# ana-kuznetsova/Policy-Gradient-ASR

Hardware: AMD Instinct MI355X
Metric: utterances/sec (B=32,T=1000,F=80) policy-grad step, 1/2/4/8 MI355X (higher is better)
Workload: dtype f32 (fp32-faithful: fp32 storage and accumulate; every big product -- recurrent sweeps, W_ih projections, input and weight gradients -- on the bf16 MFMA as SIX terms of a 3-plane split hi/mid/lo, every term down to 2^-24 of the product; the small products on the exact fp32 MFMA; the faster bf16x3 mo

## Files before the change

include/pgasr_hip.h:

```cpp
#ifndef PGASR_HIP_H
#define PGASR_HIP_H

#include <stddef.h>
#include <stdint.h>

#ifdef __cplusplus
extern "C" {
#endif

typedef enum pgasr_status {
    PGASR_OK = 0,
    PGASR_ERR_INVALID_ARG = 1,
    PGASR_ERR_LAUNCH = 2,
    PGASR_ERR_WORKSPACE = 3,
    PGASR_ERR_UNSUPPORTED = 4,
    PGASR_ERR_TIMEOUT = 5
} pgasr_status;

#define PGASR_ABI_VERSION 7

int pgasr_abi_version(void);
const char* pgasr_status_string(int status);

size_t pgasr_ctc_workspace_bytes(int T, int B, int V, int Lmax);
int pgasr_ctc_loss_grad(const float* log_probs, const int32_t* targets,
                        const int32_t* input_lengths, const int32_t* target_lengths,
                        int T, int B, int V, int Lmax, int blank,
                        const float* utt_scale, const float* pg_coef, const int32_t* pg_path,
                        float* nll, float* grad_logits,
                        void* workspace, size_t workspace_bytes, void* stream);

int pgasr_ctc_grad_from_lattice(const float* log_probs, const int32_t* input_lengths,
                                const int32_t* target_lengths, int T, int B, int V, int Lmax, int blank,
                                const float* utt_scale, const float* pg_coef, const int32_t* pg_path,
                                int pg_coef_per_frame, float* grad_logits, void* workspace, size_t workspace_bytes,
                                void* stream);

int pgasr_pg_rewards(const int32_t* dist, const int32_t* target_lengths, int B, float lam,
                     float inv_global_batch, float* R_greedy, float* R_sample, float* pg_coef,
                     float* utt_scale, void* stream);
int pgasr_pg_loss_value(const float* log_probs, const int32_t* path, const int32_t* input_lengths,
                        const float* nll, const float* utt_scale, const float* pg_coef,
                        int T, int B, int V, int pg_coef_per_frame, float* terms, void* stream);
int pgasr_pg_step_coefs(const int32_t* paths, const int32_t* input_lengths, const int32_t* prefix_dist, int prefix_stride,
                        const int32_t* token_lengths, const int32_t* target_lengths, int T, int B, int blank,
                        float lam, float inv_global_batch, float* coef, void* stream);

#define PGASR_MAX_SAMPLES 16
#define PGASR_BASELINE_HYPOTHESIS 0
#define PGASR_BASELINE_LEAVE_ONE_OUT 1
int pgasr_frame_sample_multi(const float* scores, int T, int B, int V, int K,
                             uint64_t seed, uint32_t offset, int ctr_stride, int ctr_base,
                             int32_t* greedy_path, int32_t* sample_paths, void* stream);
int pgasr_ctc_grad_from_lattice_multi(const float* log_probs, const int32_t* input_lengths,
                                      const int32_t* target_lengths, int T, int B, int V, int Lmax, int blank,
                                      const float* utt_scale, int K, const float* pg_coef, const int32_t* pg_paths,
                                      float* grad_logits, void* workspace, size_t workspace_bytes, void* stream);
int pgasr_pg_rewards_multi(const int32_t* dist, const int32_t* target_lengths, int B, int K, int baseline,
                           float lam, float inv_global_batch, float* R_baseline, float* R_sample, float* pg_coef,
                           float* utt_scale, void* stream);
int pgasr_pg_loss_value_multi(const float* log_probs, const int32_t* paths, int K, const int32_t* input_lengths,
                              const float* nll, const float* utt_scale, const float* pg_coef,
                              int T, int B, int V, float* terms, void* stream);

size_t pgasr_ctc_hyp_workspace_bytes(int T, int B, int V, int K, int Lh);
int pgasr_ctc_hyp_lattice(const float* log_probs, const int32_t* hyp_tokens, int hyp_stride, const int32_t* hyp_len,
                          const int32_t* input_lengths, int T, int B, int V, int K, int Lh, int blank,
                          float* hyp_nll, void* hyp_workspace, size_t hyp_workspace_bytes, void* stream);
int pgasr_ctc_grad_from_lattices_seq(const float* log_probs, const int32_t* input_lengths, const int32_t* target_lengths,
                                     int T, int B, int V, int Lmax, int blank, const float* utt_scale,
                                     int K, const float* pg_coef, const int32_t* pg_paths, const int32_t* hyp_len, int Lh,
                                     float* grad_logits, void* workspace, size_t workspace_bytes,
                                     void* hyp_workspace, size_t hyp_workspace_bytes, void* stream);
int pgasr_pg_loss_value_seq(const float* log_probs, const int32_t* paths, int K, const int32_t* input_lengths,
                            const float* nll, const float* utt_scale, const float* pg_coef,
                            const float* hyp_nll, const int32_t* hyp_len, int Lh,
                            int T, int B, int V, float* terms, void* stream);

int pgasr_frame_entropy(const float* log_probs, const int32_t* input_lengths, int T, int B, int V,
                        float beta, float inv_global_batch, float* ent_mean, float* ent_scale, void* stream);
int pgasr_ctc_grad_from_lattice_ent(const float* log_probs, const int32_t* input_lengths,
                                    const int32_t* target_lengths, int T, int B, int V, int Lmax, int blank,
                                    const float* utt_scale, const float* pg_coef, const int32_t* pg_path,
                                    int pg_coef_per_frame, const float* ent_scale, float* grad_logits,
                                    void* workspace, size_t workspace_bytes, void* stream);
int pgasr_ctc_grad_from_lattice_multi_ent(const float* log_probs, const int32_t* input_lengths,
                                          const int32_t* target_lengths, int T, int B, int V, int Lmax, int blank,
                                          const float* utt_scale, int K, const float* pg_coef, const int32_t* pg_paths,
                                          const float* ent_scale, float* grad_logits, void* workspace, size_t workspace_bytes,
                                          void* stream);
int pgasr_ctc_grad_from_lattices_seq_ent(const float* log_probs, const int32_t* input_lengths, const int32_t* target_lengths,
                                         int T, int B, int V, int Lmax, int blank, const float* utt_scale,
                                         int K, const float* pg_coef, const int32_t* pg_paths, const int32_t* hyp_len, int Lh,
                                         const float* ent_scale, float* grad_logits, void* workspace, size_t workspace_bytes,
                                         void* hyp_workspace, size_t hyp_workspace_bytes, void* stream);

size_t pgasr_ctc_align_workspace_bytes(int T, int B, int Lmax);
int pgasr_ctc_forced_align(const float* log_probs, const int32_t* tokens, const int32_t* input_lengths,
                           const int32_t* token_lengths, int T, int B, int V, int Lmax, int blank,
                           double* score, int32_t* frame_label, int32_t* frame_token,
                           int32_t* token_start, int32_t* token_end, double* token_logp,
                           void* workspace, size_t workspace_bytes, void* stream);

#define PGASR_WORD_MAX_STRIDE 4094
int pgasr_word_ids(const int32_t* ref, const int32_t* ref_len, int ref_stride,
                   const int32_t* hyp, const int32_t* hyp_len, int hyp_stride, int N, int delimiter,
                   int32_t* ref_ids, int32_t* ref_words, int32_t* hyp_ids, int32_t* hyp_words, void* stream);
int pgasr_pg_rewards_multi_ex(const int32_t* dist, const int32_t* reward_lengths, const int32_t* target_lengths, int B, int K,
                              int baseline, float lam, float inv_global_batch, float* R_baseline, float* R_sample,
                              float* pg_coef, float* utt_scale, void* stream);

int pgasr_head_logsoftmax(const float* x, long long rows, int K, int ldx, const float* W, const float* bias, int V,
                          float* logits, float* log_probs, void* stream);

int pgasr_frame_argmax_sample(const float* scores, int T, int B, int V,
                              uint64_t seed, uint32_t offset, int ctr_stride, int ctr_base,
                              int32_t* greedy_path, int32_t* sample_path, void* stream);

int pgasr_frame_argmax_sample_ids(const float* scores, int T, int B, int V, uint64_t seed, uint32_t offset,
                                  int ctr_stride, const int32_t* utt_ids,
                                  int32_t* greedy_path, int32_t* sample_path, void* stream);
int pgasr_frame_sample_multi_ids(const float* scores, int T, int B, int V, int K, uint64_t seed, uint32_t offset,
                                 int ctr_stride, const int32_t* utt_ids,
                                 int32_t* greedy_path, int32_t* sample_paths, void* stream);

int pgasr_batch_prep(const float* fmask, int B, int T, const long long* tmask, const long long* targets, int L,
                     int32_t* in_len, int32_t* tg_len, int32_t* targets32, void* stream);
int pgasr_ctc_collapse(const int32_t* paths, const int32_t* lengths, int P, int T, int B,
                       int blank, int32_t* tokens, int32_t* token_lengths, void* stream);

int pgasr_edit_distance(const int32_t* ref, const int32_t* ref_len, int ref_stride,
                        const int32_t* hyp, const int32_t* hyp_len, int hyp_stride,
                        int N, int32_t* dist, int32_t* prefix_dist, void* stream);

int pgasr_reinforce_grad(const float* scores, const int32_t* path, const float* coef,
                         const int32_t* lengths, int T, int B, int V, int accumulate,
                         float* grad, void* stream);

size_t pgasr_gemm_workspace_bytes(int M, int N, int batch, int splitk, int sum_batches);
int pgasr_gemm_f32(int transA, int transB, int M, int N, int K, float alpha,
                   const float* A, int lda, long long strideA,
                   const float* B, int ldb, long long strideB,
                   float* C, int ldc, long long strideC,
                   int batch, int sum_batches, int splitk,
                   const float* bias, const float* bias2, int act, float slope, int accumulate,
                   const float* dact_y, int norm_operand, const float* shift, const float* scale,
                   int precision, const unsigned* xcc_busy, void* workspace, size_t workspace_bytes, void* stream);

int pgasr_split_bf16_planes(const float* src, int rows, int cols, int ld, int transpose,
                            unsigned short* hi, unsigned short* lo, void* stream);
int pgasr_gemm_x3w_f32(int M, int N, int K, const float* A, int lda, const unsigned short* Whi,
                       const unsigned short* Wlo, float* C, int ldc, const float* bias,
                       const float* dact_y, float slope, void* stream);
size_t pgasr_gemm_x3w_feed_workspace_bytes(void);
int pgasr_gemm_x3w_feed_col_tiles(int N);
int pgasr_gemm_x3w_feed_head_items(int N, int K, int groups);
int pgasr_gemm_x3w_feed_f32(int M, int N, int K, const float* A, int lda, const unsigned short* Whi,
                            const unsigned short* Wlo, float* C, int ldc, const float* bias,
                            const unsigned* xcc_busy, unsigned* tiles_done, int order, int phase, int head_groups,
                            void* workspace, size_t workspace_bytes, void* stream);

size_t pgasr_lstm_wgrads_workspace_bytes(int T, int in_dim);
int pgasr_lstm_wgrads_streamed(const float* dgates, const float* x, const float* out, int T, int B, int in_dim,
                               float* dwih_perm, float* dwhh_perm, const unsigned* xcc_busy,
                               const unsigned* slab_done, int* err_word, int planes,
                               void* workspace, size_t workspace_bytes, void* stream);

int pgasr_pack_x6w_planes(const float* src, int rows, int cols, int ld, int transpose, void* pack, void* stream);
int pgasr_split_bf16_planes3(const float* src, int rows, int cols, int ld, int transpose,
                             unsigned short* hi, unsigned short* mid, unsigned short* lo, void* stream);
int pgasr_gemm_x6w_f32(int M, int N, int K, const float* A, int lda, const unsigned short* Whi,
                       const unsigned short* Wmid, const unsigned short* Wlo, float* C, int ldc, const float* bias,
                       const float* dact_y, float slope, void* stream);
size_t pgasr_gemm_x6w_feed_workspace_bytes(void);
int pgasr_gemm_x6w_feed_col_tiles(int N);
int pgasr_gemm_x6w_feed_f32(int M, int N, int K, const float* A, int lda, const unsigned short* Whi,
                            const unsigned short* Wmid, const unsigned short* Wlo, float* C, int ldc, const float* bias,
                            const unsigned* xcc_busy, unsigned* tiles_done, int order,
                            void* workspace, size_t workspace_bytes, void* stream);
int pgasr_gemm_x6w_feed_head_items(int M, int N, int K);
int pgasr_gemm_x6w_feed_phase_f32(int M, int N, int K, const float* A, int lda, const unsigned short* Whi,
                                  const unsigned short* Wmid, const unsigned short* Wlo, float* C, int ldc, const float* bias,
                                  const unsigned* xcc_busy, unsigned* tiles_done, int order, int phase, unsigned* ctrl,
                                  void* workspace, size_t workspace_bytes, void* stream);

int pgasr_attention_ctx(const float* dec, const float* enc, int NQ, int B, int T, int H, float* ctx, void* stream);

int pgasr_lstm_cell_f32(const float* gh, const float* xp, float* c, float* h, float* h_out, int B, int H, void* stream);

size_t pgasr_colsum_workspace_bytes(int rows, int cols);
int pgasr_colsum_f32(const float* X, int rows, int cols, int ld, float* out, float* out2, int accumulate,
                     void* workspace, size_t workspace_bytes, void* stream);

int pgasr_instnorm_stats(const float* x, int B, int F, int T, float eps, float* mean, float* rstd,
                         void* stream);

int pgasr_log_softmax_rows(const float* logits, long long rows, int V, float* log_probs, void* stream);

size_t pgasr_lstm_pack_bytes(int which, int planes);
int pgasr_lstm_pack_weights(const float* w_ih_f, const float* w_hh_f, const float* b_ih_f, const float* b_hh_f,
                            const float* w_ih_r, const float* w_hh_r, const float* b_ih_r, const float* b_hh_r,
                            int in_dim, float* wih_perm, float* bias_perm,
                            void* whh_pack_fwd, void* whh_pack_bwd, int planes, void* stream);
int pgasr_lstm_unpack_grads(const float* dwih_perm, const float* dbias_perm, const float* dwhh_perm, int in_dim,
                            float* dw_ih_f, float* dw_hh_f, float* db_ih_f, float* db_hh_f,
                            float* dw_ih_r, float* dw_hh_r, float* db_ih_r, float* db_hh_r,
                            int accumulate, void* stream);
size_t pgasr_lstm_workspace_bytes(int T, int B, int backward);
int pgasr_lstm_error_offset(int B, int backward, size_t* offset);
int pgasr_lstm_status(const void* workspace, size_t workspace_bytes, int B, int backward, void* stream);
int pgasr_error_flag(const int32_t* word0, const int32_t* word1, float* out, void* stream);
int pgasr_lstm_busy_offset(int B, int backward, size_t* offset);
int pgasr_stream_gate(const unsigned* words, int count, int timeout_us, void* stream);
int pgasr_stream_gate_sum(const unsigned* words, int count, int need, const unsigned* running, int timeout_us, void* stream);
int pgasr_stream_gate_report(const unsigned* words, int count, int need, const unsigned* running, int timeout_us,
                             unsigned* report, void* stream);
int pgasr_stream_probe(unsigned* words, int timeout_us, void* stream);
int pgasr_lstm_layer_fwd(float* gates, float* out, float* cbuf, const void* whh_pack_fwd,
                         const int32_t* lengths, int T, int B, int flags,
                         float* out_drop, float drop_p, uint64_t drop_seed, uint32_t drop_offset,
                         void* workspace, size_t workspace_bytes, void* stream);
int pgasr_lstm_layer_fwd_fed(float* gates, float* out, float* cbuf, const void* whh_pack_fwd,
                             const int32_t* lengths, int T, int B, int flags, const unsigned* fed, int fed_need,
                             float* out_drop, float drop_p, uint64_t drop_seed, uint32_t drop_offset,
                             void* workspace, size_t workspace_bytes, void* stream);
int pgasr_lstm_fed_ok(int T, int B, int flags);
int pgasr_lstm_layer_bwd_fed(float* gates, const float* out, const float* cbuf, const float* dout,
                             const void* whh_pack_bwd, const int32_t* lengths, int T, int B, int flags,
                             float* dbias_part, const unsigned* fed, int fed_need, float drop_p, uint64_t drop_seed,
                             uint32_t drop_offset, void* workspace, size_t workspace_bytes, void* stream);
int pgasr_lstm_layer_bwd(float* gates, const float* out, const float* cbuf, const float* dout,
                         const void* whh_pack_bwd, const int32_t* lengths, int T, int B, int flags,
                         float* dbias_part, void* workspace, size_t workspace_bytes, void* stream);
int pgasr_lstm_wgrad_slabs(int T, int* edges, int max_edges);
int pgasr_lstm_layer_bwd_streamed(float* gates, const float* out, const float* cbuf, const float* dout,
                                  const void* whh_pack_bwd, const int32_t* lengths, int T, int B, int flags,
                                  float* dbias_part, const unsigned* fed, int fed_need, float drop_p, uint64_t drop_seed,
                                  uint32_t drop_offset, unsigned* slab_done,
                                  void* workspace, size_t workspace_bytes, void* stream);

size_t pgasr_beam_workspace_bytes(int T, int B, int V, int beam);
int pgasr_ctc_beam_search(const void* log_probs, int is_f64, long long stride_t, long long stride_b,
                          const int32_t* lengths, int T, int B, int V, int beam, int blank, int flags,
                          int32_t* out_tokens, int32_t* out_len, double* out_score,
                          void* workspace, size_t workspace_bytes, void* stream);

int pgasr_ctc_beam_search_lm(const void* log_probs, int is_f64, long long stride_t, long long stride_b,
                             const int32_t* lengths, int T, int B, int V, int beam, int blank, int flags,
                             int32_t* out_tokens, int32_t* out_len, double* out_score,
                             void* workspace, size_t workspace_bytes, void* stream,
                             const float* lm_table, int lm_order, double lm_alpha, double lm_beta);

#define PGASR_SPECAUG_FILL_ROW_MEAN 0
#define PGASR_SPECAUG_FILL_ZERO 1
int pgasr_spec_augment(const float* x, const int32_t* lengths, const int32_t* utt_ids ,
                       int batch_offset, int B, int F, int T, int n_freq, int freq_width, int n_time, int time_width,
                       float time_ratio, int fill_mode, unsigned long long seed, unsigned offset,
                       float* out , int32_t* masks ,
                       void* stream);

int pgasr_dropout(const float* x, float* y, unsigned long long n, float p, uint64_t seed, uint32_t offset,
                  const float* dact_y, float slope, void* stream);
int pgasr_stream_copy(const void* src, void* dst, unsigned long long bytes, int workgroups, void* stream);
int pgasr_adam_step(float* param, const float* grad, float* exp_avg, float* exp_avg_sq, unsigned long long n,
                    int step, float lr, float beta1, float beta2, float eps, float weight_decay,
                    const int32_t* guard0, const int32_t* guard1, int32_t* applied, void* stream);
#define PGASR_CLIP_STATE_BYTES 32
size_t pgasr_grad_norm_ws_bytes(unsigned long long n);
int pgasr_grad_norm_clip(const float* grad, unsigned long long n, float max_norm, void* ws, size_t ws_bytes,
                         void* state, void* stream);
int pgasr_adam_step_clipped(float* param, const float* grad, float* exp_avg, float* exp_avg_sq, unsigned long long n,
                            int step, float lr, float beta1, float beta2, float eps, float weight_decay,
                            const int32_t* guard0, const int32_t* guard1, int32_t* applied, const void* clip_state,
                            void* stream);

int pgasr_feat_frames(const float* wave, const int32_t* n_samples, const int32_t* n_frames, int B,
                      long long wave_stride, int Tmax, float* frames, void* stream);
int pgasr_feat_power(const float* spec, long long rows, float* power, void* stream);
int pgasr_feat_db(float* mel, const int32_t* n_frames, int B, int Tmax, int n_mels, float top_db, void* stream);
int pgasr_feat_deltas_stack(const float* mfcc, const int32_t* n_frames, int B, int Tmax, int n_mfcc,
                            float* feat, float* fmask, void* stream);
int pgasr_feat_stack(const float* x, const int32_t* n_frames, int B, int Tmax, int C, float* feat, float* fmask, void* stream);

#ifdef __cplusplus
}
#endif
#endif
```

policy_gradient_asr_amd/_lib.py:

```python
import ctypes as C
import os

import torch

_HERE = os.path.dirname(os.path.abspath(__file__))
LIB_PATH = os.environ.get("PGASR_HIP_LIB", os.path.join(_HERE, "libpgasr_hip.so"))

c_f32p = C.c_void_p
c_i32p = C.c_void_p
c_ptr = C.c_void_p

SIGNATURES = {
    "pgasr_abi_version": (C.c_int, []),
    "pgasr_status_string": (C.c_char_p, [C.c_int]),
    "pgasr_ctc_workspace_bytes": (C.c_size_t, [C.c_int, C.c_int, C.c_int, C.c_int]),
    "pgasr_ctc_loss_grad": (C.c_int, [c_f32p, c_i32p, c_i32p, c_i32p, C.c_int, C.c_int, C.c_int, C.c_int,
                                      C.c_int, c_f32p, c_f32p, c_i32p, c_f32p, c_f32p, c_ptr, C.c_size_t, c_ptr]),
    "pgasr_ctc_grad_from_lattice": (C.c_int, [c_f32p, c_i32p, c_i32p, C.c_int, C.c_int, C.c_int, C.c_int, C.c_int,
                                              c_f32p, c_f32p, c_i32p, C.c_int, c_f32p, c_ptr, C.c_size_t, c_ptr]),
    "pgasr_pg_rewards": (C.c_int, [c_i32p, c_i32p, C.c_int, C.c_float, C.c_float, c_f32p, c_f32p, c_f32p, c_f32p, c_ptr]),
    "pgasr_pg_loss_value": (C.c_int, [c_f32p, c_i32p, c_i32p, c_f32p, c_f32p, c_f32p, C.c_int, C.c_int, C.c_int, C.c_int,
                                      c_f32p, c_ptr]),
    "pgasr_head_logsoftmax": (C.c_int, [c_f32p, C.c_longlong, C.c_int, C.c_int, c_f32p, c_f32p, C.c_int, c_f32p, c_f32p, c_ptr]),
    "pgasr_pg_step_coefs": (C.c_int, [c_i32p, c_i32p, c_i32p, C.c_int, c_i32p, c_i32p, C.c_int, C.c_int, C.c_int,
                                      C.c_float, C.c_float, c_f32p, c_ptr]),
    "pgasr_frame_argmax_sample": (C.c_int, [c_f32p, C.c_int, C.c_int, C.c_int, C.c_uint64, C.c_uint32, C.c_int, C.c_int,
                                            c_i32p, c_i32p, c_ptr]),
    "pgasr_frame_sample_multi": (C.c_int, [c_f32p, C.c_int, C.c_int, C.c_int, C.c_int, C.c_uint64, C.c_uint32, C.c_int, C.c_int,
                                           c_i32p, c_i32p, c_ptr]),
    "pgasr_frame_argmax_sample_ids": (C.c_int, [c_f32p, C.c_int, C.c_int, C.c_int, C.c_uint64, C.c_uint32, C.c_int, c_i32p,
                                                c_i32p, c_i32p, c_ptr]),
    "pgasr_frame_sample_multi_ids": (C.c_int, [c_f32p, C.c_int, C.c_int, C.c_int, C.c_int, C.c_uint64, C.c_uint32, C.c_int, c_i32p,
                                               c_i32p, c_i32p, c_ptr]),
    "pgasr_ctc_grad_from_lattice_multi": (C.c_int, [c_f32p, c_i32p, c_i32p, C.c_int, C.c_int, C.c_int, C.c_int, C.c_int,
                                                    c_f32p, C.c_int, c_f32p, c_i32p, c_f32p, c_ptr, C.c_size_t, c_ptr]),
    "pgasr_pg_rewards_multi": (C.c_int, [c_i32p, c_i32p, C.c_int, C.c_int, C.c_int, C.c_float, C.c_float, c_f32p, c_f32p, c_f32p,
                                         c_f32p, c_ptr]),
    "pgasr_pg_loss_value_multi": (C.c_int, [c_f32p, c_i32p, C.c_int, c_i32p, c_f32p, c_f32p, c_f32p, C.c_int, C.c_int, C.c_int,
                                            c_f32p, c_ptr]),
    "pgasr_ctc_hyp_workspace_bytes": (C.c_size_t, [C.c_int] * 5),
    "pgasr_ctc_hyp_lattice": (C.c_int, [c_f32p, c_i32p, C.c_int, c_i32p, c_i32p, C.c_int, C.c_int, C.c_int, C.c_int, C.c_int, C.c_int,
                                        c_f32p, c_ptr, C.c_size_t, c_ptr]),
    "pgasr_ctc_grad_from_lattices_seq": (C.c_int, [c_f32p, c_i32p, c_i32p, C.c_int, C.c_int, C.c_int, C.c_int, C.c_int, c_f32p,
                                                   C.c_int, c_f32p, c_i32p, c_i32p, C.c_int, c_f32p, c_ptr, C.c_size_t,
                                                   c_ptr, C.c_size_t, c_ptr]),
    "pgasr_pg_loss_value_seq": (C.c_int, [c_f32p, c_i32p, C.c_int, c_i32p, c_f32p, c_f32p, c_f32p, c_f32p, c_i32p, C.c_int,
                                          C.c_int, C.c_int, C.c_int, c_f32p, c_ptr]),
    "pgasr_frame_entropy": (C.c_int, [c_f32p, c_i32p, C.c_int, C.c_int, C.c_int, C.c_float, C.c_float, c_f32p, c_f32p, c_ptr]),
    "pgasr_ctc_grad_from_lattice_ent": (C.c_int, [c_f32p, c_i32p, c_i32p, C.c_int, C.c_int, C.c_int, C.c_int, C.c_int,
                                                  c_f32p, c_f32p, c_i32p, C.c_int, c_f32p, c_f32p, c_ptr, C.c_size_t, c_ptr]),
    "pgasr_ctc_grad_from_lattice_multi_ent": (C.c_int, [c_f32p, c_i32p, c_i32p, C.c_int, C.c_int, C.c_int, C.c_int, C.c_int,
                                                        c_f32p, C.c_int, c_f32p, c_i32p, c_f32p, c_f32p, c_ptr, C.c_size_t, c_ptr]),
    "pgasr_ctc_grad_from_lattices_seq_ent": (C.c_int, [c_f32p, c_i32p, c_i32p, C.c_int, C.c_int, C.c_int, C.c_int, C.c_int, c_f32p,
                                                       C.c_int, c_f32p, c_i32p, c_i32p, C.c_int, c_f32p, c_f32p, c_ptr, C.c_size_t,
                                                       c_ptr, C.c_size_t, c_ptr]),
    "pgasr_ctc_align_workspace_bytes": (C.c_size_t, [C.c_int] * 3),
    "pgasr_ctc_forced_align": (C.c_int, [c_f32p, c_i32p, c_i32p, c_i32p, C.c_int, C.c_int, C.c_int, C.c_int, C.c_int,
                                         c_ptr, c_i32p, c_i32p, c_i32p, c_i32p, c_ptr, c_ptr, C.c_size_t, c_ptr]),
    "pgasr_word_ids": (C.c_int, [c_i32p, c_i32p, C.c_int, c_i32p, c_i32p, C.c_int, C.c_int, C.c_int, c_i32p, c_i32p, c_i32p, c_i32p,
                                 c_ptr]),
    "pgasr_pg_rewards_multi_ex": (C.c_int, [c_i32p, c_i32p, c_i32p, C.c_int, C.c_int, C.c_int, C.c_float, C.c_float, c_f32p, c_f32p,
                                            c_f32p, c_f32p, c_ptr]),
    "pgasr_batch_prep": (C.c_int, [c_f32p, C.c_int, C.c_int, c_ptr, c_ptr, C.c_int, c_i32p, c_i32p, c_i32p, c_ptr]),
    "pgasr_ctc_collapse": (C.c_int, [c_i32p, c_i32p, C.c_int, C.c_int, C.c_int, C.c_int, c_i32p, c_i32p, c_ptr]),
    "pgasr_edit_distance": (C.c_int, [c_i32p, c_i32p, C.c_int, c_i32p, c_i32p, C.c_int, C.c_int,
                                      c_i32p, c_i32p, c_ptr]),
    "pgasr_reinforce_grad": (C.c_int, [c_f32p, c_i32p, c_f32p, c_i32p, C.c_int, C.c_int, C.c_int, C.c_int,
                                       c_f32p, c_ptr]),
    "pgasr_beam_workspace_bytes": (C.c_size_t, [C.c_int] * 4),
    "pgasr_ctc_beam_search": (C.c_int, [c_ptr, C.c_int, C.c_longlong, C.c_longlong, c_i32p, C.c_int, C.c_int, C.c_int,
                                        C.c_int, C.c_int, C.c_int, c_i32p, c_i32p, c_ptr, c_ptr, C.c_size_t, c_ptr]),
    "pgasr_ctc_beam_search_lm": (C.c_int, [c_ptr, C.c_int, C.c_longlong, C.c_longlong, c_i32p, C.c_int, C.c_int, C.c_int,
                                           C.c_int, C.c_int, C.c_int, c_i32p, c_i32p, c_ptr, c_ptr, C.c_size_t, c_ptr,
                                           c_f32p, C.c_int, C.c_double, C.c_double]),
    "pgasr_dropout": (C.c_int, [c_f32p, c_f32p, C.c_ulonglong, C.c_float, C.c_uint64, C.c_uint32, c_f32p, C.c_float, c_ptr]),
    "pgasr_spec_augment": (C.c_int, [c_f32p, c_i32p, c_i32p, C.c_int, C.c_int, C.c_int, C.c_int, C.c_int, C.c_int, C.c_int, C.c_int,
                                     C.c_float, C.c_int, C.c_ulonglong, C.c_uint, c_f32p, c_i32p, c_ptr]),
    "pgasr_stream_copy": (C.c_int, [c_ptr, c_ptr, C.c_ulonglong, C.c_int, c_ptr]),
    "pgasr_adam_step": (C.c_int, [c_f32p, c_f32p, c_f32p, c_f32p, C.c_ulonglong, C.c_int, C.c_float, C.c_float,
                                  C.c_float, C.c_float, C.c_float, c_i32p, c_i32p, c_i32p, c_ptr]),
    "pgasr_adam_step_clipped": (C.c_int, [c_f32p, c_f32p, c_f32p, c_f32p, C.c_ulonglong, C.c_int, C.c_float, C.c_float,
                                          C.c_float, C.c_float, C.c_float, c_i32p, c_i32p, c_i32p, c_ptr, c_ptr]),
    "pgasr_grad_norm_ws_bytes": (C.c_size_t, [C.c_ulonglong]),
    "pgasr_grad_norm_clip": (C.c_int, [c_f32p, C.c_ulonglong, C.c_float, c_ptr, C.c_size_t, c_ptr, c_ptr]),
    "pgasr_gemm_workspace_bytes": (C.c_size_t, [C.c_int] * 5),
    "pgasr_gemm_f32": (C.c_int, [C.c_int, C.c_int, C.c_int, C.c_int, C.c_int, C.c_float,
                                 c_f32p, C.c_int, C.c_longlong, c_f32p, C.c_int, C.c_longlong,
                                 c_f32p, C.c_int, C.c_longlong, C.c_int, C.c_int, C.c_int,
                                 c_f32p, c_f32p, C.c_int, C.c_float, C.c_int,
                                 c_f32p, C.c_int, c_f32p, c_f32p, C.c_int, c_ptr, c_ptr, C.c_size_t, c_ptr]),
    "pgasr_split_bf16_planes": (C.c_int, [c_f32p, C.c_int, C.c_int, C.c_int, C.c_int, c_ptr, c_ptr, c_ptr]),
    "pgasr_gemm_x3w_f32": (C.c_int, [C.c_int, C.c_int, C.c_int, c_f32p, C.c_int, c_ptr, c_ptr, c_f32p, C.c_int,
                                     c_f32p, c_f32p, C.c_float, c_ptr]),
    "pgasr_gemm_x3w_feed_workspace_bytes": (C.c_size_t, []),
    "pgasr_gemm_x3w_feed_col_tiles": (C.c_int, [C.c_int]),
    "pgasr_gemm_x3w_feed_head_items": (C.c_int, [C.c_int, C.c_int, C.c_int]),
    "pgasr_gemm_x3w_feed_f32": (C.c_int, [C.c_int, C.c_int, C.c_int, c_f32p, C.c_int, c_ptr, c_ptr, c_f32p, C.c_int,
                                          c_f32p, c_ptr, c_ptr, C.c_int, C.c_int, C.c_int, c_ptr, C.c_size_t, c_ptr]),
    "pgasr_feat_frames": (C.c_int, [c_f32p, c_i32p, c_i32p, C.c_int, C.c_longlong, C.c_int, c_f32p, c_ptr]),
    "pgasr_feat_power": (C.c_int, [c_f32p, C.c_longlong, c_f32p, c_ptr]),
    "pgasr_feat_db": (C.c_int, [c_f32p, c_i32p, C.c_int, C.c_int, C.c_int, C.c_float, c_ptr]),
    "pgasr_feat_deltas_stack": (C.c_int, [c_f32p, c_i32p, C.c_int, C.c_int, C.c_int, c_f32p, c_f32p, c_ptr]),
    "pgasr_feat_stack": (C.c_int, [c_f32p, c_i32p, C.c_int, C.c_int, C.c_int, c_f32p, c_f32p, c_ptr]),
    "pgasr_colsum_workspace_bytes": (C.c_size_t, [C.c_int, C.c_int]),
    "pgasr_colsum_f32": (C.c_int, [c_f32p, C.c_int, C.c_int, C.c_int, c_f32p, c_f32p, C.c_int,
                                   c_ptr, C.c_size_t, c_ptr]),
    "pgasr_instnorm_stats": (C.c_int, [c_f32p, C.c_int, C.c_int, C.c_int, C.c_float, c_f32p, c_f32p, c_ptr]),
    "pgasr_log_softmax_rows": (C.c_int, [c_f32p, C.c_longlong, C.c_int, c_f32p, c_ptr]),
    "pgasr_lstm_pack_bytes": (C.c_size_t, [C.c_int, C.c_int]),
    "pgasr_lstm_pack_weights": (C.c_int, [c_f32p] * 8 + [C.c_int, c_f32p, c_f32p, c_ptr, c_ptr, C.c_int, c_ptr]),
    "pgasr_lstm_unpack_grads": (C.c_int, [c_f32p, c_f32p, c_f32p, C.c_int] + [c_f32p] * 8 + [C.c_int, c_ptr]),
    "pgasr_lstm_workspace_bytes": (C.c_size_t, [C.c_int, C.c_int, C.c_int]),
    "pgasr_lstm_error_offset": (C.c_int, [C.c_int, C.c_int, C.POINTER(C.c_size_t)]),
    "pgasr_lstm_busy_offset": (C.c_int, [C.c_int, C.c_int, C.POINTER(C.c_size_t)]),
    "pgasr_lstm_status": (C.c_int, [c_ptr, C.c_size_t, C.c_int, C.c_int, c_ptr]),
    "pgasr_stream_gate": (C.c_int, [c_ptr, C.c_int, C.c_int, c_ptr]),
    "pgasr_stream_gate_sum": (C.c_int, [c_ptr, C.c_int, C.c_int, c_ptr, C.c_int, c_ptr]),
    "pgasr_stream_gate_report": (C.c_int, [c_ptr, C.c_int, C.c_int, c_ptr, C.c_int, c_ptr, c_ptr]),
    "pgasr_stream_probe": (C.c_int, [c_ptr, C.c_int, c_ptr]),
    "pgasr_lstm_layer_fwd": (C.c_int, [c_f32p, c_f32p, c_f32p, c_ptr, c_i32p, C.c_int, C.c_int, C.c_int,
                                       c_f32p, C.c_float, C.c_uint64, C.c_uint32, c_ptr, C.c_size_t, c_ptr]),
    "pgasr_lstm_layer_fwd_fed": (C.c_int, [c_f32p, c_f32p, c_f32p, c_ptr, c_i32p, C.c_int, C.c_int, C.c_int, c_ptr, C.c_int,
                                           c_f32p, C.c_float, C.c_uint64, C.c_uint32, c_ptr, C.c_size_t, c_ptr]),
    "pgasr_lstm_fed_ok": (C.c_int, [C.c_int, C.c_int, C.c_int]),
    "pgasr_lstm_layer_bwd_fed": (C.c_int, [c_f32p, c_f32p, c_f32p, c_f32p, c_ptr, c_i32p, C.c_int, C.c_int, C.c_int,
                                           c_f32p, c_ptr, C.c_int, C.c_float, C.c_uint64, C.c_uint32, c_ptr, C.c_size_t, c_ptr]),
    "pgasr_lstm_layer_bwd": (C.c_int, [c_f32p, c_f32p, c_f32p, c_f32p, c_ptr, c_i32p, C.c_int, C.c_int, C.c_int,
                                       c_f32p, c_ptr, C.c_size_t, c_ptr]),
    "pgasr_lstm_wgrad_slabs": (C.c_int, [C.c_int, c_i32p, C.c_int]),
    "pgasr_lstm_layer_bwd_streamed": (C.c_int, [c_f32p, c_f32p, c_f32p, c_f32p, c_ptr, c_i32p, C.c_int, C.c_int, C.c_int,
                                                c_f32p, c_ptr, C.c_int, C.c_float, C.c_uint64, C.c_uint32, c_ptr,
                                                c_ptr, C.c_size_t, c_ptr]),
    "pgasr_lstm_wgrads_workspace_bytes": (C.c_size_t, [C.c_int, C.c_int]),
    "pgasr_lstm_wgrads_streamed": (C.c_int, [c_f32p, c_f32p, c_f32p, C.c_int, C.c_int, C.c_int, c_f32p, c_f32p, c_ptr,
                                             c_ptr, c_ptr, C.c_int, c_ptr, C.c_size_t, c_ptr]),
    "pgasr_error_flag": (C.c_int, [c_i32p, c_i32p, c_f32p, c_ptr]),
    "pgasr_attention_ctx": (C.c_int, [c_f32p, c_f32p, C.c_int, C.c_int, C.c_int, C.c_int, c_f32p, c_ptr]),
    "pgasr_lstm_cell_f32": (C.c_int, [c_f32p, c_f32p, c_f32p, c_f32p, c_f32p, C.c_int, C.c_int, c_ptr]),
    "pgasr_pack_x6w_planes": (C.c_int, [c_f32p, C.c_int, C.c_int, C.c_int, C.c_int, c_ptr, c_ptr]),
    "pgasr_split_bf16_planes3": (C.c_int, [c_f32p, C.c_int, C.c_int, C.c_int, C.c_int, c_ptr, c_ptr, c_ptr, c_ptr]),
    "pgasr_gemm_x6w_f32": (C.c_int, [C.c_int, C.c_int, C.c_int, c_f32p, C.c_int, c_ptr, c_ptr, c_ptr, c_f32p, C.c_int,
                                     c_f32p, c_f32p, C.c_float, c_ptr]),
    "pgasr_gemm_x6w_feed_workspace_bytes": (C.c_size_t, []),
    "pgasr_gemm_x6w_feed_col_tiles": (C.c_int, [C.c_int]),
    "pgasr_gemm_x6w_feed_f32": (C.c_int, [C.c_int, C.c_int, C.c_int, c_f32p, C.c_int, c_ptr, c_ptr, c_ptr, c_f32p, C.c_int,
                                          c_f32p, c_ptr, c_ptr, C.c_int, c_ptr, C.c_size_t, c_ptr]),
    "pgasr_gemm_x6w_feed_head_items": (C.c_int, [C.c_int, C.c_int, C.c_int]),
    "pgasr_gemm_x6w_feed_phase_f32": (C.c_int, [C.c_int, C.c_int, C.c_int, c_f32p, C.c_int, c_ptr, c_ptr, c_ptr, c_f32p, C.c_int,
                                                c_f32p, c_ptr, c_ptr, C.c_int, C.c_int, c_ptr, c_ptr, C.c_size_t, c_ptr]),
}


class PgasrError(RuntimeError):
    pass


TIMEOUT = 5


_lib = None


def load():
    global _lib
    if _lib is not None:
        return _lib
    if not os.path.exists(LIB_PATH):
        raise PgasrError(
            f"{LIB_PATH} is missing: build it with `python -c 'import __graft_entry__ as g; g.build()'` "
            "or `make -C policy_gradient_asr_amd/csrc`.  There is no CPU fallback.")
    lib = C.CDLL(LIB_PATH)
    for name, (res, args) in SIGNATURES.items():
        fn = getattr(lib, name)
        fn.restype = res
        fn.argtypes = args
    if lib.pgasr_abi_version() != 7:
        raise PgasrError("libpgasr_hip.so ABI version mismatch")
    _lib = lib
    return lib


def check(status, what):
    if status != 0:
        msg = load().pgasr_status_string(status).decode()
        raise PgasrError(f"{what} failed: status {status} ({msg})")
```

policy_gradient_asr_amd/csrc/common.h:

```cpp
#pragma once
#include <hip/hip_runtime.h>
#include <stdint.h>
#include <math.h>
#include <stdio.h>
#include <stdlib.h>
#include "pgasr_hip.h"

#define PGASR_WAVE 64

#define PGASR_LAUNCH_KERNEL(...)                               \
    do {                                                       \
        (void)hipGetLastError();                               \
        hipLaunchKernelGGL(__VA_ARGS__);                       \
    } while (0)

#define PGASR_CHECK_LAUNCH()                                                                  \
    do {                                                                                      \
        hipError_t e__ = hipGetLastError();                                                   \
        if (e__ != hipSuccess) {                                                              \
            if (getenv("PGASR_DEBUG"))                                                        \
                fprintf(stderr, "[pgasr] %s:%d launch failed: %s\n", __FILE__, __LINE__,      \
                        hipGetErrorString(e__));                                              \
            return PGASR_ERR_LAUNCH;                                                          \
        }                                                                                     \
    } while (0)

static inline size_t pgasr_align_up(size_t x, size_t a) { return (x + a - 1) / a * a; }

#define PGASR_NEG_INF (-INFINITY)

__device__ __forceinline__ float wave_sum(float v) {
#pragma unroll
    for (int o = 32; o > 0; o >>= 1) v += __shfl_xor(v, o, 64);
    return v;
}
__device__ __forceinline__ float wave_max(float v) {
#pragma unroll
    for (int o = 32; o > 0; o >>= 1) v = fmaxf(v, __shfl_xor(v, o, 64));
    return v;
}

__device__ __forceinline__ float block_path_logprob_sum(const float* __restrict__ lp, const int32_t* __restrict__ path,
                                                        const float* __restrict__ frame_coef, int Tb, int b, int B, int V, float* red) {
    float s = 0.f;
    for (int t = threadIdx.x; t < Tb; t += 256) {
        const float v = lp[((size_t)t * B + b) * V + path[(size_t)t * B + b]];
        s += frame_coef ? frame_coef[(size_t)t * B + b] * v : v;
    }
    red[threadIdx.x] = s;
    __syncthreads();
    for (int o = 128; o > 0; o >>= 1) {
        if (threadIdx.x < o) red[threadIdx.x] += red[threadIdx.x + o];
        __syncthreads();
    }
    const float r = red[0];
    __syncthreads();
    return r;
}

__device__ __forceinline__ void philox4x32_10(uint32_t c0, uint32_t c1, uint32_t c2, uint32_t c3,
                                              uint32_t k0, uint32_t k1, uint32_t out[4]) {
#pragma unroll
    for (int r = 0; r < 10; ++r) {
        const uint64_t p0 = (uint64_t)0xD2511F53u * c0;
        const uint64_t p1 = (uint64_t)0xCD9E8D57u * c2;
        const uint32_t n0 = (uint32_t)(p1 >> 32) ^ c1 ^ k0;
        const uint32_t n1 = (uint32_t)p1;
        const uint32_t n2 = (uint32_t)(p0 >> 32) ^ c3 ^ k1;
        const uint32_t n3 = (uint32_t)p0;
        c0 = n0; c1 = n1; c2 = n2; c3 = n3;
        k0 += 0x9E3779B9u; k1 += 0xBB67AE85u;
    }
    out[0] = c0; out[1] = c1; out[2] = c2; out[3] = c3;
}

#ifndef PGASR_WSLAB_NUM
#define PGASR_WSLAB_NUM 5
#define PGASR_WSLAB_DEN 4
#define PGASR_WSLAB_CAP 128
#endif
__host__ __device__ inline int pgasr_wslab_next(int s) { const int n = ((s * PGASR_WSLAB_NUM) / PGASR_WSLAB_DEN + 4) & ~7; return n > PGASR_WSLAB_CAP ? PGASR_WSLAB_CAP : n; }
__host__ __device__ inline int pgasr_wslab_count(int T) {
    int h = 0, s = 16, n = 1;
    while (T - h > s + s / 2) { h += s; s = pgasr_wslab_next(s); ++n; }
    return n;
}
__host__ __device__ inline int pgasr_wslab_edge(int T, int i) {
    int h = 0, s = 16;
    for (int j = 0; j < i; ++j) {
        if (T - h <= s + s / 2) return T;
        h += s; s = pgasr_wslab_next(s);
    }
    return h;
}

struct PgasrTn256Args {
    const float* A; const float* B; float* partial;
    int M, N, K, lda, ldb;
    long long sA, sB;
    int batch, splitk, kper;
    float alpha;
    unsigned* queue;
    const unsigned* xcc_busy;
    int diag;
    const unsigned* gate;
    const float* gate_base;
    int gate_T, gate_B, gate_nbg;
    int tslabs;
    int* gate_err;
};
bool pgasr_internal_tn256_ok(const PgasrTn256Args& a, int tk = 32);
int pgasr_internal_tn256_launch(PgasrTn256Args a, int masked_then_unmasked, hipStream_t st, const PgasrTn256Args* second = nullptr);
int pgasr_internal_tn6_launch(PgasrTn256Args a, int masked_then_unmasked, hipStream_t st, const PgasrTn256Args* second = nullptr);

struct PgasrX3cArgs {
    const float* A; const unsigned short* Whi; const unsigned short* Wlo; float* C;
    int M, N, K, lda, ldc;
    const float* bias; const float* dact_y; float slope;
    int feed;
    unsigned* queue; const unsigned* xcc_busy; unsigned* tiles_done;
    int mt_count, nt_count, order, quarters, split_tiles;
    float* slabs; unsigned* arrive;
};
size_t pgasr_internal_x3c_slab_bytes();
int pgasr_internal_x3c_launch(const PgasrX3cArgs& a, hipStream_t st);
```

policy_gradient_asr_amd/csrc/gemm.hip:

```cpp
#include "common.h"

namespace {

constexpr int BM = 128, BN = 128, BK = 16, PADF = 4;
constexpr int GEMM_THREADS = 256;

typedef __attribute__((ext_vector_type(16))) float f32x16;

struct GemmArgs {
    const float* A; const float* B; float* C;
    int M, N, K, lda, ldb, ldc;
    long long sA, sB, sC;
    int batch, splitk, kper;
    float alpha;
    const float* bias; const float* bias2;
    int act; float slope;
    int accumulate;
    const float* dact_y;
    int norm_operand;
    const float* shift; const float* scale;
    float* partial;
    unsigned* queue;
    const unsigned* xcc_busy;
    int tx, ty, tz;
// ... 388 lines not shown
                    ah[i] = tr_frag(&S[cur][0][0][ro]);
                    al[i] = tr_frag(&S[cur][0][1][ro]);
                } else {
                    const int ro = (wm * 64 + i * 32 + fr) * XPITCH + kk + fk;
                    ah[i] = __builtin_bit_cast(bf16x8_t, *reinterpret_cast<const u32x4_t*>(&S[cur][0][0][ro]));
                    al[i] = __builtin_bit_cast(bf16x8_t, *reinterpret_cast<const u32x4_t*>(&S[cur][0][1][ro]));
                }
                if constexpr (TRB) {
                    const int co = kk * TPITCH + wn * 64 + i * 32 + tro;
                    bh[i] = tr_frag(&S[cur][1][0][co]);
                    bl[i] = tr_frag(&S[cur][1][1][co]);
                } else {
                    const int co = (wn * 64 + i * 32 + fr) * XPITCH + kk + fk;
                    bh[i] = __builtin_bit_cast(bf16x8_t, *reinterpret_cast<const u32x4_t*>(&S[cur][1][0][co]));
                    bl[i] = __builtin_bit_cast(bf16x8_t, *reinterpret_cast<const u32x4_t*>(&S[cur][1][1][co]));
                }
            }
#pragma unroll
            for (int i = 0; i < 2; ++i)
#pragma unroll
                for (int j = 0; j < 2; ++j) {
                    acc[i][j] = __builtin_amdgcn_mfma_f32_32x32x16_bf16(ah[i], bh[j], acc[i][j], 0, 0, 0);
                    acc[i][j] = __builtin_amdgcn_mfma_f32_32x32x16_bf16(ah[i], bl[j], acc[i][j], 0, 0, 0);
                    acc[i][j] = __builtin_amdgcn_mfma_f32_32x32x16_bf16(al[i], bh[j], acc[i][j], 0, 0, 0);
                }
        }
    };
    const int nrm = g.norm_operand;
    const float nsh = nrm ? g.shift[bidx] : 0.f, nsc = nrm ? g.scale[bidx] : 1.f;
    auto norm_strip = [&](float (&v)[16], bool tr, int mn_base, int mn_lim, int kb) {
#pragma unroll
        for (int i = 0; i < 16; ++i) {
            const int mn = tr ? mn_base + (tid & 31) * 4 + (i & 3) : mn_base + (tid >> 1);
            const int k = tr ? kb + (tid >> 5) + 8 * (i >> 2) : kb + (tid & 1) * 16 + i;
            v[i] = (mn < mn_lim && k < kend) ? (v[i] - nsh) * nsc : 0.f;
        }
    };
#define XLOAD(RA, RB, KB) do { if constexpr (TRA) tload_strip(A, g.lda, m0, g.M, (KB), kend, tid, vecA, RA); \
                               else xload_strip(A, g.lda, m0, g.M, (KB), kend, tid, vecA, RA); \
                               if constexpr (TRB) tload_strip(B, g.ldb, n0, g.N, (KB), kend, tid, vecB, RB); \
                               else xload_strip(B, g.ldb, n0, g.N, (KB), kend, tid, vecB, RB); \
                               if (nrm == 1) norm_strip(RA, TRA, m0, g.M, (KB)); \
                               else if (nrm == 2) norm_strip(RB, TRB, n0, g.N, (KB)); } while (0)
#define XSTORE(RA, RB, BUF) do { if constexpr (TRA) tstore_strip(S[BUF][0][0], S[BUF][0][1], tid, RA); \
                                 else xstore_strip(S[BUF][0][0], S[BUF][0][1], tid, RA); \
                                 if constexpr (TRB) tstore_strip(S[BUF][1][0], S[BUF][1][1], tid, RB); \
                                 else xstore_strip(S[BUF][1][0], S[BUF][1][1], tid, RB); } while (0)
    if (kbeg < kend) {
        XLOAD(ra0, rb0, kbeg);
        XSTORE(ra0, rb0, 0);
        if (kbeg + XBK < kend) XLOAD(ra0, rb0, kbeg + XBK);
    }
    __syncthreads();
    for (int kb = kbeg; kb < kend; kb += 2 * XBK) {
        if (kb + 2 * XBK < kend) XLOAD(ra1, rb1, kb + 2 * XBK);
        compute(0);
        if (kb + XBK < kend) XSTORE(ra0, rb0, 1);
        __syncthreads();
        if (kb + XBK >= kend) break;
        if (kb + 3 * XBK < kend) XLOAD(ra0, rb0, kb + 3 * XBK);
        compute(1);
        if (kb + 2 * XBK < kend) XSTORE(ra1, rb1, 0);
        __syncthreads();
    }
#undef XLOAD
#undef XSTORE

    if (!g.wide) { store_tiles_fast(g, acc, m0, n0, wm, wn, lane, z, bidx, live); return; }
    const int cl = lane & 31, rq = lane >> 5;
#pragma unroll
    for (int i = 0; i < 2; ++i)
#pragma unroll
        for (int j = 0; j < 2; ++j) {
            const int n = n0 + wn * 64 + j * 32 + cl;
            if (n >= g.N || !live) continue;
            float bsum = 0.f;
            if (!g.partial) {
                if (g.bias) bsum += g.bias[n];
                if (g.bias2) bsum += g.bias2[n];
            }
#pragma unroll
            for (int r = 0; r < 16; ++r) {
                const int m = m0 + wm * 64 + i * 32 + (r & 3) + 8 * (r >> 2) + 4 * rq;
                if (m >= g.M) continue;
                float v = g.alpha * acc[i][j][r];
                if (g.partial) {
                    g.partial[((size_t)z * g.M + m) * g.N + n] = v;
                } else {
                    float* c = g.C + (size_t)bidx * g.sC + (size_t)m * g.ldc + n;
                    v += bsum;
                    if (g.act == 1) v = v > 0.f ? v : v * g.slope;
                    if (g.dact_y) v *= (g.dact_y[(size_t)bidx * g.sC + (size_t)m * g.ldc + n] > 0.f ? 1.f : g.slope);
                    if (g.accumulate) v += *c;
                    *c = v;
                }
            }
        }
}

__global__ __launch_bounds__(256) void gemm_reduce_kernel(const float* __restrict__ partial, int Z, int M, int N,
                                                          float* __restrict__ C, int ldc, long long sC,
                                                          const float* bias,
                                                          const float* bias2, int act, float slope, int accumulate) {
    const size_t idx = (size_t)blockIdx.x * 256 + threadIdx.x;
    if (idx >= (size_t)M * N) return;
    const int m = (int)(idx / N), n = (int)(idx % N);
    partial += (size_t)blockIdx.y * Z * M * N;
    C += (size_t)blockIdx.y * sC;
    float v = 0.f;
    for (int zz = 0; zz < Z; ++zz) v += partial[(size_t)zz * M * N + idx];
    if (bias) v += bias[n];
    if (bias2) v += bias2[n];
    if (act == 1) v = v > 0.f ? v : v * slope;
    float* c = C + (size_t)m * ldc + n;
    if (accumulate) v += *c;
    *c = v;
}

__global__ __launch_bounds__(256) void colsum_partial_kernel(const float* __restrict__ X, int rows, int cols, int ld,
                                                             int rows_per_block, float* __restrict__ partial) {
    __shared__ float red[4][64];
    const int c = blockIdx.x * 64 + (threadIdx.x & 63);
    const int rl = threadIdx.x >> 6;
    const int r0 = blockIdx.y * rows_per_block, r1 = min(rows, r0 + rows_per_block);
    float s = 0.f;
    if (c < cols)
        for (int r = r0 + rl; r < r1; r += 4) s += X[(size_t)r * ld + c];
    red[rl][threadIdx.x & 63] = s;
    __syncthreads();
    if (rl == 0 && c < cols)
        partial[(size_t)blockIdx.y * cols + c] = (red[0][threadIdx.x] + red[1][threadIdx.x]) + (red[2][threadIdx.x] + red[3][threadIdx.x]);
}
__global__ __launch_bounds__(256) void colsum_final_kernel(const float* __restrict__ partial, int nparts, int cols,
                                                           float* __restrict__ out, float* __restrict__ out2, int accumulate) {
    const int c = blockIdx.x * 256 + threadIdx.x;
    if (c >= cols) return;
    float s = 0.f;
    for (int p = 0; p < nparts; ++p) s += partial[(size_t)p * cols + c];
    if (accumulate) { out[c] += s; if (out2) out2[c] += s; }
    else { out[c] = s; if (out2) out2[c] = s; }
}

__global__ __launch_bounds__(1024) void instnorm_stats_kernel(const float* __restrict__ x, long long n_per, float eps,
                                                              float* __restrict__ mean, float* __restrict__ rstd) {
    __shared__ double s1[16], s2[16];
    const float* p = x + (size_t)blockIdx.x * n_per;
    double a = 0.0, b = 0.0;
    long long done = 0;
    if (((n_per & 3) == 0) && ((((size_t)x) & 15) == 0)) {
        const float4* p4 = reinterpret_cast<const float4*>(p);
        const long long n4 = n_per >> 2;
        double a1 = 0.0, b1 = 0.0;
        long long i = threadIdx.x;
        for (; i + 3 * 1024 < n4; i += 4 * 1024) {
            const float4 u0 = p4[i], u1 = p4[i + 1024], u2 = p4[i + 2 * 1024], u3 = p4[i + 3 * 1024];
            a += ((double)u0.x + (double)u0.y) + ((double)u0.z + (double)u0.w);
            b += ((double)u0.x * u0.x + (double)u0.y * u0.y) + ((double)u0.z * u0.z + (double)u0.w * u0.w);
            a1 += ((double)u1.x + (double)u1.y) + ((double)u1.z + (double)u1.w);
            b1 += ((double)u1.x * u1.x + (double)u1.y * u1.y) + ((double)u1.z * u1.z + (double)u1.w * u1.w);
            a += ((double)u2.x + (double)u2.y) + ((double)u2.z + (double)u2.w);
            b += ((double)u2.x * u2.x + (double)u2.y * u2.y) + ((double)u2.z * u2.z + (double)u2.w * u2.w);
            a1 += ((double)u3.x + (double)u3.y) + ((double)u3.z + (double)u3.w);
            b1 += ((double)u3.x * u3.x + (double)u3.y * u3.y) + ((double)u3.z * u3.z + (double)u3.w * u3.w);
        }
        for (; i < n4; i += 1024) {
            const float4 u = p4[i];
            a += ((double)u.x + (double)u.y) + ((double)u.z + (double)u.w);
            b += ((double)u.x * u.x + (double)u.y * u.y) + ((double)u.z * u.z + (double)u.w * u.w);
        }
        a += a1; b += b1;
        done = n_per;
    }
    for (long long i = done + threadIdx.x; i < n_per; i += 1024) { const double v = p[i]; a += v; b += v * v; }
#pragma unroll
    for (int o = 32; o > 0; o >>= 1) { a += __shfl_xor(a, o, 64); b += __shfl_xor(b, o, 64); }
    if ((threadIdx.x & 63) == 0) { s1[threadIdx.x >> 6] = a; s2[threadIdx.x >> 6] = b; }
    __syncthreads();
    if (threadIdx.x == 0) {
        double ta = 0.0, tb = 0.0;
        for (int i = 0; i < 16; ++i) { ta += s1[i]; tb += s2[i]; }
        const double mu = ta / (double)n_per;
        double var = tb / (double)n_per - mu * mu;
        if (var < 0.0) var = 0.0;
        mean[blockIdx.x] = (float)mu;
        rstd[blockIdx.x] = (float)(1.0 / sqrt(var + (double)eps));
    }
}

}

static int gemm_launch(GemmArgs& g, int transA, int transB, int sum_batches, int precision, const unsigned* xcc_busy, void* workspace,
                       size_t workspace_bytes, hipStream_t st) {
    const int Z = g.batch * g.splitk;
    const bool use_partial = (g.splitk > 1) || sum_batches;
    const bool queue_mode = precision >= 1 && xcc_busy != nullptr;
    const size_t head = 256;
    if (use_partial || queue_mode) {
        const size_t need = head + (use_partial ? (size_t)Z * g.M * g.N * sizeof(float) : 0);
        if (!workspace || workspace_bytes < need) return PGASR_ERR_WORKSPACE;
    }
    g.partial = use_partial ? (float*)((char*)workspace + head) : nullptr;
    g.queue = nullptr; g.xcc_busy = nullptr;
    dim3 grid((g.N + BN - 1) / BN, (g.M + BM - 1) / BM, Z);
    if (grid.y > 65535 || grid.z > 65535) return PGASR_ERR_UNSUPPORTED;
    g.tx = (int)grid.x; g.ty = (int)grid.y; g.tz = (int)grid.z;
    if (queue_mode) {
        g.queue = (unsigned*)workspace; g.xcc_busy = xcc_busy;
        if (hipMemsetAsync(workspace, 0, head, st) != hipSuccess) return PGASR_ERR_LAUNCH;
    }
    const unsigned ntiles_q = grid.x * grid.y * grid.z;

    bool done_tn256 = false;
    if (precision >= 1 && transA && !transB && use_partial && g.norm_operand == 0) {
        PgasrTn256Args t{g.A, g.B, g.partial, g.M, g.N, g.K, g.lda, g.ldb, g.sA, g.sB, g.batch, g.splitk, g.kper, g.alpha,
                         queue_mode ? g.queue : nullptr, queue_mode ? g.xcc_busy : nullptr, getenv("PGASR_TN_DIAG") ? atoi(getenv("PGASR_TN_DIAG")) : 0,
                         nullptr, nullptr, 0, 0, 0, 0, nullptr};
        if (pgasr_internal_tn256_ok(t)) {
            const int st_ = precision == 2 ? pgasr_internal_tn6_launch(t, queue_mode ? 1 : 0, st) : pgasr_internal_tn256_launch(t, queue_mode ? 1 : 0, st);
            if (st_ != PGASR_OK) return st_;
            done_tn256 = true;
        }
    }
    if (done_tn256) {
    }
    else if (precision == 2) return PGASR_ERR_UNSUPPORTED;
    else if (precision == 1) {
        if (queue_mode) {
            for (int pass = 0; pass < 2; ++pass) {
                dim3 qgrid(pass == 0 ? 2u * ntiles_q + 8u : ntiles_q);
                if (pass == 1) g.xcc_busy = nullptr;
                if (!transA && !transB) PGASR_LAUNCH_KERNEL((gemm_bf16x3_kernel<false, false, true>), qgrid, dim3(GEMM_THREADS), 0, st, g);
                else if (!transA && transB) PGASR_LAUNCH_KERNEL((gemm_bf16x3_kernel<false, true, true>), qgrid, dim3(GEMM_THREADS), 0, st, g);
                else if (transA && !transB) PGASR_LAUNCH_KERNEL((gemm_bf16x3_kernel<true, false, true>), qgrid, dim3(GEMM_THREADS), 0, st, g);
                else PGASR_LAUNCH_KERNEL((gemm_bf16x3_kernel<true, true, true>), qgrid, dim3(GEMM_THREADS), 0, st, g);
                PGASR_CHECK_LAUNCH();
            }
        }
        else if (!transA && !transB) PGASR_LAUNCH_KERNEL((gemm_bf16x3_kernel<false, false, false>), grid, dim3(GEMM_THREADS), 0, st, g);
        else if (!transA && transB) PGASR_LAUNCH_KERNEL((gemm_bf16x3_kernel<false, true, false>), grid, dim3(GEMM_THREADS), 0, st, g);
        else if (transA && !transB) PGASR_LAUNCH_KERNEL((gemm_bf16x3_kernel<true, false, false>), grid, dim3(GEMM_THREADS), 0, st, g);
        else PGASR_LAUNCH_KERNEL((gemm_bf16x3_kernel<true, true, false>), grid, dim3(GEMM_THREADS), 0, st, g);
    }
    else if (!transA && !transB) PGASR_LAUNCH_KERNEL((gemm_f32_kernel<false, false>), grid, dim3(GEMM_THREADS), 0, st, g);
    else if (!transA && transB) PGASR_LAUNCH_KERNEL((gemm_f32_kernel<false, true>), grid, dim3(GEMM_THREADS), 0, st, g);
    else if (transA && !transB) PGASR_LAUNCH_KERNEL((gemm_f32_kernel<true, false>), grid, dim3(GEMM_THREADS), 0, st, g);
    else PGASR_LAUNCH_KERNEL((gemm_f32_kernel<true, true>), grid, dim3(GEMM_THREADS), 0, st, g);
    PGASR_CHECK_LAUNCH();
    if (use_partial) {
        const size_t total = (size_t)g.M * g.N;
        const int nout = sum_batches ? 1 : g.batch;
        PGASR_LAUNCH_KERNEL(gemm_reduce_kernel, dim3((unsigned)((total + 255) / 256), nout), dim3(256), 0, st,
                           g.partial, Z / nout, g.M, g.N, g.C, g.ldc, g.sC, g.bias, g.bias2, g.act, g.slope,
                           g.accumulate);
        PGASR_CHECK_LAUNCH();
    }
    return PGASR_OK;
}

extern "C" size_t pgasr_gemm_workspace_bytes(int M, int N, int batch, int splitk, int sum_batches) {
    if (M <= 0 || N <= 0 || batch <= 0 || splitk <= 0) return 0;
    if (splitk <= 1 && !sum_batches) return 256;
    return 256 + (size_t)batch * splitk * M * N * sizeof(float);
}

extern "C" int pgasr_gemm_f32(int transA, int transB, int M, int N, int K, float alpha,
                              const float* A, int lda, long long strideA,
                              const float* B, int ldb, long long strideB,
                              float* C, int ldc, long long strideC,
                              int batch, int sum_batches, int splitk,
                              const float* bias, const float* bias2, int act, float slope, int accumulate,
                              const float* dact_y, int norm_operand, const float* shift, const float* scale,
                              int precision, const unsigned* xcc_busy, void* workspace, size_t workspace_bytes, void* stream) {
    if (!A || !B || !C || M <= 0 || N <= 0 || K <= 0 || batch <= 0 || splitk <= 0) return PGASR_ERR_INVALID_ARG;
    if (norm_operand < 0 || norm_operand > 2 || (norm_operand && (!shift || !scale))) return PGASR_ERR_INVALID_ARG;
    if (act < 0 || act > 1 || precision < 0 || precision > 2) return PGASR_ERR_INVALID_ARG;
    if ((splitk > 1 || sum_batches) && dact_y) return PGASR_ERR_INVALID_ARG;
    GemmArgs g;
    g.A = A; g.B = B; g.C = C; g.M = M; g.N = N; g.K = K; g.lda = lda; g.ldb = ldb; g.ldc = ldc;
    g.sA = strideA; g.sB = strideB; g.sC = strideC; g.batch = batch; g.splitk = splitk;
    int kper = (K + splitk - 1) / splitk;
    const int kq = precision >= 1 ? XBK : BK;
    kper = (kper + kq - 1) / kq * kq;
    g.kper = kper;
    g.alpha = alpha; g.bias = bias; g.bias2 = bias2; g.act = act; g.slope = slope; g.accumulate = accumulate;
    g.dact_y = dact_y; g.norm_operand = norm_operand; g.shift = shift; g.scale = scale; g.partial = nullptr;
    g.wide = (((size_t)(M - 1) * ldc + N) * 4 >= ((size_t)1 << 32) || (size_t)M * N * 4 >= ((size_t)1 << 32)) ? 1 : 0;
    return gemm_launch(g, transA, transB, sum_batches, precision, xcc_busy, workspace, workspace_bytes, (hipStream_t)stream);
}

extern "C" int pgasr_lstm_wgrad_slabs(int T, int* edges, int max_edges) {
    if (T <= 0) return 0;
    const int n = pgasr_wslab_count(T);
    for (int i = 0; edges && i <= n && i < max_edges; ++i) edges[i] = pgasr_wslab_edge(T, i);
    return n;
}
extern "C" size_t pgasr_lstm_wgrads_workspace_bytes(int T, int in_dim) {
    if (in_dim <= 0 || T <= 0) return 0;
    return 256 + (size_t)pgasr_wslab_count(T) * ((size_t)2048 * in_dim + (size_t)2 * 1024 * 256) * sizeof(float);
}
extern "C" int pgasr_lstm_wgrads_streamed(const float* dgates, const float* x, const float* out, int T, int B, int in_dim,
                                          float* dwih_perm, float* dwhh_perm, const unsigned* xcc_busy,
                                          const unsigned* slab_done, int* err_word, int planes,
                                          void* workspace, size_t workspace_bytes, void* stream) {
    constexpr int H = 256, G = 2 * 4 * H;
    if (!dgates || !x || !out || !dwih_perm || !dwhh_perm || T <= 1 || B <= 0 || in_dim <= 0) return PGASR_ERR_INVALID_ARG;
    if (planes != 2 && planes != 3) return PGASR_ERR_INVALID_ARG;
    const size_t need = pgasr_lstm_wgrads_workspace_bytes(T, in_dim);
    if (!workspace || workspace_bytes < need) return PGASR_ERR_WORKSPACE;
    hipStream_t st = (hipStream_t)stream;
    const int nslab = pgasr_wslab_count(T);
    float* part_ih = (float*)((char*)workspace + 256);
    float* part_hh = part_ih + (size_t)nslab * G * in_dim;
    const long long K_ih = (long long)T * B, K_hh = (long long)(T - 1) * B;
    if (K_ih >= ((long long)1 << 31)) return PGASR_ERR_UNSUPPORTED;
    PgasrTn256Args ih{dgates, x, part_ih, G, in_dim, (int)K_ih, G, in_dim, 0, 0, 1, nslab, 0, 1.f,
                      (unsigned*)workspace, xcc_busy, 0, slab_done, dgates, T, B, (B + 15) / 16, 1, err_word};
    PgasrTn256Args hh{dgates + (size_t)B * G, out, part_hh, 4 * H, H, (int)K_hh, G, 2 * H, (long long)4 * H - (long long)B * G,
                      (long long)B * 2 * H + H, 2, nslab, 0, 1.f,
                      (unsigned*)workspace, xcc_busy, 0, slab_done, dgates, T, B, (B + 15) / 16, 1, err_word};
    const int tk = planes == 3 ? 16 : 32;
    if (!pgasr_internal_tn256_ok(ih, tk) || !pgasr_internal_tn256_ok(hh, tk)) return PGASR_ERR_UNSUPPORTED;
    if (hipMemsetAsync(workspace, 0, 256, st) != hipSuccess) return PGASR_ERR_LAUNCH;
    const int rc = planes == 3 ? pgasr_internal_tn6_launch(ih, 1, st, &hh) : pgasr_internal_tn256_launch(ih, 1, st, &hh);
    if (rc != PGASR_OK) return rc;
    PGASR_LAUNCH_KERNEL(gemm_reduce_kernel, dim3((unsigned)(((size_t)G * in_dim + 255) / 256), 1), dim3(256), 0, st,
                       part_ih, nslab, G, in_dim, dwih_perm, in_dim, (long long)0, (const float*)nullptr, (const float*)nullptr, 0, 0.f, 0);
    PGASR_CHECK_LAUNCH();
    PGASR_LAUNCH_KERNEL(gemm_reduce_kernel, dim3((unsigned)(((size_t)4 * H * H + 255) / 256), 2), dim3(256), 0, st,
                       part_hh, nslab, 4 * H, H, dwhh_perm, H, (long long)4 * H * H, (const float*)nullptr, (const float*)nullptr, 0, 0.f, 0);
    PGASR_CHECK_LAUNCH();
    return PGASR_OK;
}

extern "C" size_t pgasr_colsum_workspace_bytes(int rows, int cols) {
    if (rows <= 0 || cols <= 0) return 0;
    const int rpb = 512;
    return (size_t)((rows + rpb - 1) / rpb) * cols * sizeof(float);
}

extern "C" int pgasr_colsum_f32(const float* X, int rows, int cols, int ld, float* out, float* out2, int accumulate,
                                void* workspace, size_t workspace_bytes, void* stream) {
    if (!X || !out || rows <= 0 || cols <= 0 || ld < cols) return PGASR_ERR_INVALID_ARG;
    const int rpb = 512;
    const int nparts = (rows + rpb - 1) / rpb;
    if (!workspace || workspace_bytes < (size_t)nparts * cols * sizeof(float)) return PGASR_ERR_WORKSPACE;
    hipStream_t st = (hipStream_t)stream;
    PGASR_LAUNCH_KERNEL(colsum_partial_kernel, dim3((cols + 63) / 64, nparts), dim3(256), 0, st, X, rows, cols, ld, rpb,
                       (float*)workspace);
    PGASR_CHECK_LAUNCH();
    PGASR_LAUNCH_KERNEL(colsum_final_kernel, dim3((cols + 255) / 256), dim3(256), 0, st, (const float*)workspace, nparts,
                       cols, out, out2, accumulate);
    PGASR_CHECK_LAUNCH();
    return PGASR_OK;
}

extern "C" int pgasr_instnorm_stats(const float* x, int B, int F, int T, float eps, float* mean, float* rstd,
                                    void* stream) {
    if (!x || !mean || !rstd || B <= 0 || F <= 0 || T <= 0) return PGASR_ERR_INVALID_ARG;
    PGASR_LAUNCH_KERNEL(instnorm_stats_kernel, dim3(B), dim3(1024), 0, (hipStream_t)stream, x, (long long)F * T, eps,
                       mean, rstd);
    PGASR_CHECK_LAUNCH();
    return PGASR_OK;
}
```

policy_gradient_asr_amd/csrc/gemm_x6.hip:

```cpp
#include "common.h"
#include "x3w_common.h"
#include <type_traits>

#ifdef PGASR_X6_DIAG
#define X6D(bit) (!FEED && (g.single & (bit)))
__device__ long long x6_stamp_out[8][16];
#define X6STAMP_DECL long long st_last_ = clock64(); long long st_acc_[12] = {0, 0, 0, 0, 0, 0, 0, 0, 0, 0, 0, 0}; const long long st_c0_ = clock64(), st_r0_ = wall_clock64()
#define X6STAMP(slot) do { const long long now_ = clock64(); st_acc_[slot] += now_ - st_last_; st_last_ = now_; } while (0)
#define X6STAMP_FLUSH() do { if (blockIdx.x == 0 && blockIdx.y == 0 && lane == 0) { for (int i_ = 0; i_ < 12; ++i_) x6_stamp_out[w][i_] = st_acc_[i_]; \
                             x6_stamp_out[w][12] = clock64() - st_c0_; x6_stamp_out[w][13] = wall_clock64() - st_r0_; } } while (0)
#else
#define X6D(bit) false
#define X6STAMP_DECL
#define X6STAMP(slot) do { } while (0)
#define X6STAMP_FLUSH() do { } while (0)
#endif

namespace {
#ifdef PGASR_LSTM_DIAG
__device__ unsigned x6_feed_diag[4096];
#endif
namespace x6c {
constexpr int TM = 256, TN = 256, TK = 16, THREADS = 512;
constexpr int NW = 4;
constexpr int NA = 3;
constexpr int AP_BYTES = TM * TK * 2;
constexpr int ABUF_BYTES = 3 * AP_BYTES;
constexpr int WP_BYTES = TN * TK * 2;
constexpr int WSTAGE_BYTES = 3 * WP_BYTES;
constexpr int LDS_W = 2 * ABUF_BYTES;
constexpr int LDS_BYTES = LDS_W + NW * WSTAGE_BYTES;
constexpr int SLAB_FLOATS = 128 * THREADS;

typedef u32x4_t Planes2[2][3];

__device__ __forceinline__ void read_pair(Planes2& o, unsigned p0, unsigned p1) {
    static_assert(AP_BYTES == 8192 && WP_BYTES == 8192, "plane offsets are spelled in the asm below");
    asm volatile("ds_read_b128 %0, %6\n\t"
                 "ds_read_b128 %1, %6 offset:8192\n\t"
                 "ds_read_b128 %2, %6 offset:16384\n\t"
                 "ds_read_b128 %3, %7\n\t"
                 "ds_read_b128 %4, %7 offset:8192\n\t"
                 "ds_read_b128 %5, %7 offset:16384"
                 : "=&v"(o[0][0]), "=&v"(o[0][1]), "=&v"(o[0][2]), "=&v"(o[1][0]), "=&v"(o[1][1]), "=&v"(o[1][2])
                 : "v"(p0), "v"(p1)
                 : "memory");
}
__device__ __forceinline__ void wait_pair(Planes2& o) {
    asm volatile("s_waitcnt lgkmcnt(0)"
                 : "+v"(o[0][0]), "+v"(o[0][1]), "+v"(o[0][2]), "+v"(o[1][0]), "+v"(o[1][1]), "+v"(o[1][2])
                 :: "memory");
}
__device__ __forceinline__ void wait_pairs(Planes2& a, Planes2& b) {
    asm volatile("s_waitcnt lgkmcnt(0)"
                 : "+v"(a[0][0]), "+v"(a[0][1]), "+v"(a[0][2]), "+v"(a[1][0]), "+v"(a[1][1]), "+v"(a[1][2]),
                   "+v"(b[0][0]), "+v"(b[0][1]), "+v"(b[0][2]), "+v"(b[1][0]), "+v"(b[1][1]), "+v"(b[1][2])
                 :: "memory");
}
__device__ __forceinline__ void read_row(u32x4_t (&o)[3], unsigned p) {
    asm volatile("ds_read_b128 %0, %3\n\t"
                 "ds_read_b128 %1, %3 offset:8192\n\t"
                 "ds_read_b128 %2, %3 offset:16384"
                 : "=&v"(o[0]), "=&v"(o[1]), "=&v"(o[2]) : "v"(p) : "memory");
}
__device__ __forceinline__ void wait_row(u32x4_t (&o)[3]) {
    asm volatile("s_waitcnt lgkmcnt(0)" : "+v"(o[0]), "+v"(o[1]), "+v"(o[2]) :: "memory");
}
__device__ __forceinline__ void wait_row_pair(u32x4_t (&a)[3], Planes2& b) {
    asm volatile("s_waitcnt lgkmcnt(0)"
                 : "+v"(a[0]), "+v"(a[1]), "+v"(a[2]), "+v"(b[0][0]), "+v"(b[0][1]), "+v"(b[0][2]), "+v"(b[1][0]), "+v"(b[1][1]), "+v"(b[1][2])
                 :: "memory");
}
__device__ __forceinline__ void write_planes3(unsigned addr, unsigned h0, unsigned h1, unsigned m0, unsigned m1, unsigned l0, unsigned l1) {
    typedef __attribute__((ext_vector_type(2))) unsigned u2;
    const u2 h = {h0, h1}, m = {m0, m1}, l = {l0, l1};
    asm volatile("ds_write_b64 %0, %1\n\t"
                 "ds_write_b64 %0, %2 offset:8192\n\t"
                 "ds_write_b64 %0, %3 offset:16384" :: "v"(addr), "v"(h), "v"(m), "v"(l) : "memory");
}
template <int J>
__device__ __forceinline__ void load_a_one(u32x4_t (&r)[2], const unsigned (&aoff)[2], unsigned kb, const float* A) {
    asm volatile("global_load_dwordx4 %0, %1, %2" : "=&v"(r[J]) : "v"(aoff[J] + kb), "s"(A) : "memory");
}
template <int CNT>
__device__ __forceinline__ void wait_a_regs(u32x4_t (&r)[2]) {
    asm volatile("s_waitcnt vmcnt(%2)" : "+v"(r[0]), "+v"(r[1]) : "n"(CNT) : "memory");
}

__device__ __forceinline__ void mfma6(f32x16 (&acc)[2], const u32x4_t (&a)[3], const Planes2& b) {
    constexpr int PA[6] = {0, 0, 1, 0, 2, 1}, PB[6] = {0, 1, 0, 2, 0, 1};
#pragma unroll
    for (int p = 0; p < 6; ++p)
#pragma unroll
        for (int j = 0; j < 2; ++j)
            acc[j] = __builtin_amdgcn_mfma_f32_32x32x16_bf16(__builtin_bit_cast(bf16x8_t, a[PA[p]]), __builtin_bit_cast(bf16x8_t, b[j][PB[p]]), acc[j], 0, 0, 0);
}

template <bool FEED, int VAR>
__global__ __launch_bounds__(THREADS) void gemm_x6c_kernel(DmaGemmArgs g) {
    extern __shared__ __attribute__((aligned(128))) unsigned char smem[];
#ifdef PGASR_LSTM_DIAG
    if (FEED && threadIdx.x == 0 && blockIdx.x == 0) x6_feed_diag[0] = (unsigned)wall_clock64();
#endif
    const int tid = threadIdx.x, lane = tid & 63, w = tid >> 6;
    const int wm = w >> 2, wn = w & 3;
    const int nk = g.K / TK;
    bool head_only = false;
    if (FEED && g.xcc_busy) {
        const unsigned xcc = __builtin_amdgcn_s_getreg(((4 - 1) << 11) | (0 << 6) | 20) & 7u;
        if (__hip_atomic_load(g.xcc_busy + xcc, __ATOMIC_RELAXED, __HIP_MEMORY_SCOPE_AGENT) != 0u) {
            if (!g.head_help) return;
            head_only = true;
        }
    }
    const unsigned lds0 = (unsigned)(size_t)(__attribute__((address_space(3))) unsigned char*)smem;
  for (;;) {
    int tbx, tby;
    int kt0 = 0, kt1 = nk, qpart = -1;
    unsigned tile = 0, parts = 1u, slab0 = 0u;
#ifdef PGASR_LSTM_DIAG
    unsigned diag_t_ = 0xFFFFFFFFu;
#endif
    if (FEED) {
        unsigned* mailbox = reinterpret_cast<unsigned*>(smem + LDS_BYTES);
        const unsigned S8 = (unsigned)g.split8_tiles, S = (unsigned)g.split_tiles, S2 = (unsigned)g.split2_tiles, ntot = (unsigned)g.mt_count * (unsigned)g.nt_count;
        const unsigned n8 = 8u * S8, n4 = 4u * S, n2 = 2u * S2;
        if (tid == 0) {
            if (head_only && __hip_atomic_load(g.queue, __ATOMIC_RELAXED, __HIP_MEMORY_SCOPE_AGENT) >= n8 + n4) *mailbox = 0xFFFFFFFFu;
            else *mailbox = __hip_atomic_fetch_add(g.queue, 1u, __ATOMIC_RELAXED, __HIP_MEMORY_SCOPE_AGENT);
        }
        __syncthreads();
        const unsigned t = *mailbox;
        __syncthreads();
        if (t >= ntot + 7u * S8 + 3u * S + S2) return;
#ifdef PGASR_LSTM_DIAG
        if (tid == 0 && t < 4u) x6_feed_diag[4 + t] = (unsigned)wall_clock64();
        if (tid == 0 && t >= n8 + n4 + n2 && t < n8 + n4 + n2 + 4u) x6_feed_diag[1024 + (t - n8 - n4 - n2)] = (unsigned)wall_clock64();
        diag_t_ = t;
#endif
        if (t < n8) { tile = t >> 3; qpart = (int)(t & 7u); parts = 8u; slab0 = 8u * tile; }
        else if (t < n8 + n4) { const unsigned u = t - n8; tile = S8 + (u >> 2); qpart = (int)(u & 3u); parts = 4u; slab0 = n8 + 4u * (u >> 2); }
        else if (t < n8 + n4 + n2) { const unsigned u = t - n8 - n4; tile = S8 + S + (u >> 1); qpart = (int)(u & 1u); parts = 2u; slab0 = n8 + n4 + 2u * (u >> 1); }
        else tile = t - 7u * S8 - 3u * S - S2;
        if (qpart >= 0) { kt0 = qpart * (nk / (int)parts); kt1 = kt0 + nk / (int)parts; }
        const int half = g.nt_count >> 1, grp = (int)(tile / (unsigned)g.nt_count), j = (int)(tile % (unsigned)g.nt_count);
        tbx = j;
        tby = ((j < half) != (g.order != 0)) ? grp : g.mt_count - 1 - grp;
    } else {
        swizzled_tile(tbx, tby);
    }
    const int m0 = tby * TM, n0 = tbx * TN;

    const int rsub = lane >> 2, ac = lane & 3;
    unsigned aoff[2];
    unsigned apw[2];
#pragma unroll
    for (int j = 0; j < 2; ++j) {
        const int r = w * 32 + j * 16 + rsub;
        int gm = m0 + r; gm = gm < g.M ? gm : g.M - 1;
        aoff[j] = (unsigned)(((size_t)gm * g.lda + ac * 4) * 4);
        apw[j] = (unsigned)(r * 32 + (((ac >> 1) ^ ((r >> 3) & 1)) * 16) + (ac & 1) * 8);
    }
    const bool packed = g.Wmid == nullptr;
    const unsigned short* pw[3];
    {
        const int row = 32 * w + (lane >> 1), cp = lane & 1, c = cp ^ ((row >> 3) & 1);
        const size_t o = (size_t)(n0 + row) * g.K + c * 8;
        pw[0] = g.Whi + o; pw[1] = packed ? g.Whi : g.Wmid + o; pw[2] = g.Wlo + o;
    }
    const unsigned char* wpk = reinterpret_cast<const unsigned char*>(g.Whi) + (size_t)tbx * nk * WSTAGE_BYTES + w * 1024 + lane * 16;
    auto issue_w1 = [&](int kt, int stage, int plane) {
        if (X6D(1) && kt >= kt0 + NW - 1) return;
        const int kc = kt < nk ? kt : nk - 1;
        unsigned char* dst = smem + LDS_W + stage * WSTAGE_BYTES + plane * WP_BYTES + w * 1024;
        if (packed) dma16(wpk + ((size_t)kc * 3 + plane) * WP_BYTES, dst);
        else dma16(pw[plane] + kc * TK, dst);
    };
    auto issue_w = [&](int kt, int stage) { issue_w1(kt, stage, 0); issue_w1(kt, stage, 1); issue_w1(kt, stage, 2); };
    u32x4_t araw[NA][2];
    typedef std::integral_constant<int, 0> I0;
    typedef std::integral_constant<int, 1> I1;
    typedef std::integral_constant<int, 2> I2;
    auto load_a1 = [&](int kt, auto setc, int j) {
        const unsigned kb = (unsigned)((kt < nk ? kt : nk - 1) * TK * 4);
        if (X6D(4) && kt >= kt0 + NA + 1) return;
        if (j == 0) load_a_one<0>(araw[decltype(setc)::value], aoff, kb, g.A);
        else load_a_one<1>(araw[decltype(setc)::value], aoff, kb, g.A);
    };
    auto load_a = [&](int kt, auto setc) { load_a1(kt, setc, 0); load_a1(kt, setc, 1); };
    auto convert_a1 = [&](int buf, auto setc, int j) {
        constexpr int S = decltype(setc)::value;
        const unsigned base = lds0 + (unsigned)buf * ABUF_BYTES;
        if (X6D(8)) return;
        unsigned h0, m0_, l0, h1, m1_, l1;
        if (X6D(128)) { h0 = araw[S][j].x; h1 = araw[S][j].y; m0_ = araw[S][j].z; m1_ = araw[S][j].w; l0 = h0; l1 = h1; }
        else {
            split3(__uint_as_float(araw[S][j].x), __uint_as_float(araw[S][j].y), h0, m0_, l0);
            split3(__uint_as_float(araw[S][j].z), __uint_as_float(araw[S][j].w), h1, m1_, l1);
        }
        if (X6D(64)) { asm volatile("" :: "v"(h0), "v"(h1), "v"(m0_), "v"(m1_), "v"(l0), "v"(l1)); return; }
        write_planes3(base + apw[j], h0, h1, m0_, m1_, l0, l1);
    };
    auto convert_a = [&](int buf, auto setc) { convert_a1(buf, setc, 0); convert_a1(buf, setc, 1); };

    const int fr = lane & 31, fh = lane >> 5;
    unsigned offA[4], offB[2];
#pragma unroll
    for (int i = 0; i < 4; ++i) {
        const int row = wm * 128 + i * 32 + fr;
        offA[i] = (unsigned)(row * 32 + ((fh ^ ((row >> 3) & 1)) * 16));
    }
#pragma unroll
    for (int j = 0; j < 2; ++j) {
        const int n = wn * 64 + j * 32 + fr;
        offB[j] = (unsigned)(LDS_W + n * 32 + ((fh ^ ((n >> 3) & 1)) * 16));
    }

    f32x16 acc[4][2];
#pragma unroll
    for (int i = 0; i < 4; ++i)
#pragma unroll
        for (int j = 0; j < 2; ++j)
#pragma unroll
            for (int r = 0; r < 16; ++r) acc[i][j][r] = 0.f;
    X6STAMP_DECL;

    auto half_step = [&](int cur, int wst, auto halfc, Planes2& fb, auto&& mem) {
        constexpr int HALF = decltype(halfc)::value;
        const unsigned ab = lds0 + (unsigned)cur * ABUF_BYTES, wb = lds0 + (unsigned)wst * WSTAGE_BYTES;
        Planes2 fa;
        if (!X6D(16)) {
            if (HALF == 0) read_pair(fb, wb + offB[0], wb + offB[1]);
            read_pair(fa, ab + offA[2 * HALF], ab + offA[2 * HALF + 1]);
        }
        if (HALF == 0) wait_pairs(fa, fb); else wait_pair(fa);
#pragma unroll
        for (int i = 0; i < 2; ++i) {
            if (!X6D(2)) mfma6(acc[2 * HALF + i], fa[i], fb);
            __builtin_amdgcn_sched_barrier(0);
            mem(i);
            __builtin_amdgcn_sched_barrier(0);
        }
    };

    load_a(kt0, I0{});
    issue_w(kt0, 0);
    wait_a_regs<3>(araw[0]);
    convert_a(0, I0{});
    load_a(kt0 + 1, I1{});
    issue_w(kt0 + 1, 1);
    load_a(kt0 + 2, I2{});
    issue_w(kt0 + 2, 2);
    load_a(kt0 + 3, I0{});
    asm volatile("s_waitcnt vmcnt(12)\n\ts_waitcnt lgkmcnt(0)" ::: "memory");
    __builtin_amdgcn_s_barrier();
    asm volatile("" ::: "memory");

    typedef std::integral_constant<int, 1> H1;
    auto step = [&](const int kt, auto setc) {
        const int rel = kt - kt0, cur = rel & 1, wst = rel & (NW - 1);
        const int kw = kt + NW - 1, sw = (rel + NW - 1) & (NW - 1);
        auto mem_w = [&](int s) { if (s == 0) { issue_w1(kw, sw, 0); issue_w1(kw, sw, 1); } else issue_w1(kw, sw, 2); };
        auto mem_a = [&](int s) { load_a1(kt + 1 + NA, setc, s); };
        Planes2 fb;
        __builtin_amdgcn_sched_barrier(0);
        X6STAMP(0);
        if constexpr (VAR == 7) {
            const unsigned ab = lds0 + (unsigned)cur * ABUF_BYTES, wb = lds0 + (unsigned)wst * WSTAGE_BYTES;
            const unsigned cb = lds0 + (unsigned)(cur ^ 1) * ABUF_BYTES;
            constexpr int S = decltype(setc)::value;
            u32x4_t f0[3], f1[3];
            unsigned hh[2], mm[2], ll[2];
            float r0[2], r1[2];
            auto split_a = [&](int j, int q) {
                const float x0 = __uint_as_float(q ? araw[S][j].z : araw[S][j].x), x1 = __uint_as_float(q ? araw[S][j].w : araw[S][j].y);
                typedef __attribute__((ext_vector_type(2))) __bf16 bf2;
                typedef __attribute__((ext_vector_type(2))) float f2;
                hh[q] = __builtin_bit_cast(unsigned, __builtin_convertvector((f2){x0, x1}, bf2));
                r0[q] = x0 - __uint_as_float(hh[q] << 16); r1[q] = x1 - __uint_as_float(hh[q] & 0xFFFF0000u);
            };
            auto split_b = [&](int q) {
                typedef __attribute__((ext_vector_type(2))) __bf16 bf2;
                typedef __attribute__((ext_vector_type(2))) float f2;
                mm[q] = __builtin_bit_cast(unsigned, __builtin_convertvector((f2){r0[q], r1[q]}, bf2));
                const float s0 = r0[q] - __uint_as_float(mm[q] << 16), s1 = r1[q] - __uint_as_float(mm[q] & 0xFFFF0000u);
                ll[q] = __builtin_bit_cast(unsigned, __builtin_convertvector((f2){s0, s1}, bf2));
            };
            auto filler = [&](int kind, int gp, int nextrow, u32x4_t (&fnext)[3]) {
                if (gp == 0 && nextrow >= 0) read_row(fnext, ab + offA[nextrow]);
                if (kind == 0) {
                    if (gp == 1) wait_a_regs<10>(araw[S]);
                    else if (gp == 2) split_a(0, 0);
                    else if (gp == 3) split_b(0);
                    else if (gp == 4) split_a(0, 1);
                    else if (gp == 5) split_b(1);
                    else if (gp == 6) { if (!X6D(8)) write_planes3(cb + apw[0], hh[0], hh[1], mm[0], mm[1], ll[0], ll[1]); }
                    else if (gp == 7) issue_w1(kw, sw, 0);
                    else if (gp == 8) issue_w1(kw, sw, 1);
                    else if (gp == 9) issue_w1(kw, sw, 2);
                } else if (kind == 1) {
                    if (gp == 1) split_a(1, 0);
                    else if (gp == 2) split_b(0);
                    else if (gp == 3) split_a(1, 1);
                    else if (gp == 4) split_b(1);
                    else if (gp == 5) { if (!X6D(8)) write_planes3(cb + apw[1], hh[0], hh[1], mm[0], mm[1], ll[0], ll[1]); }
                    else if (gp == 6) load_a1(kt + 1 + NA, setc, 0);
                    else if (gp == 7) load_a1(kt + 1 + NA, setc, 1);
                }
            };
            auto row_mfma = [&](auto rowc, auto kindc, auto nextc, u32x4_t (&fa)[3], u32x4_t (&fnext)[3]) {
                constexpr int ROW = decltype(rowc)::value, KIND = decltype(kindc)::value, NEXT = decltype(nextc)::value;
                constexpr int PA[6] = {0, 0, 1, 0, 2, 1}, PB[6] = {0, 1, 0, 2, 0, 1};
#pragma unroll
                for (int m = 0; m < 12; ++m) {
                    const int pp = m >> 1, j = m & 1;
                    acc[ROW][j] = __builtin_amdgcn_mfma_f32_32x32x16_bf16(__builtin_bit_cast(bf16x8_t, fa[PA[pp]]), __builtin_bit_cast(bf16x8_t, fb[j][PB[pp]]), acc[ROW][j], 0, 0, 0);
                    __builtin_amdgcn_sched_barrier(0);
                    filler(KIND, m, NEXT, fnext);
                    __builtin_amdgcn_sched_barrier(0);
                }
            };
            typedef std::integral_constant<int, 2> R2;
            typedef std::integral_constant<int, 3> R3;
            typedef std::integral_constant<int, -1> RN;
            read_pair(fb, wb + offB[0], wb + offB[1]);
            if (w < 4) {
                read_row(f0, ab + offA[0]);
                wait_row_pair(f0, fb);
                X6STAMP(3);
                row_mfma(I0{}, I0{}, I1{}, f0, f1);
                wait_row(f1);
                X6STAMP(1);
                row_mfma(I1{}, I1{}, R2{}, f1, f0);
                wait_row(f0);
                X6STAMP(4);
                row_mfma(R2{}, R2{}, R3{}, f0, f1);
                wait_row(f1);
                X6STAMP(5);
                row_mfma(R3{}, R2{}, RN{}, f1, f0);
                X6STAMP(6);
            } else {
                read_row(f0, ab + offA[2]);
                wait_row_pair(f0, fb);
                X6STAMP(3);
                row_mfma(R2{}, R2{}, R3{}, f0, f1);
                wait_row(f1);
                X6STAMP(1);
                row_mfma(R3{}, R2{}, I0{}, f1, f0);
                wait_row(f0);
                X6STAMP(4);
                row_mfma(I0{}, I0{}, I1{}, f0, f1);
                wait_row(f1);
                X6STAMP(5);
                row_mfma(I1{}, I1{}, RN{}, f1, f0);
                X6STAMP(6);
            }
        } else if (w < 4) {
            wait_a_regs<10>(araw[decltype(setc)::value]);
            X6STAMP(3);
            convert_a(cur ^ 1, setc);
            __builtin_amdgcn_sched_barrier(0);
            X6STAMP(4);
            half_step(cur, wst, I0{}, fb, mem_w);
            X6STAMP(1);
            half_step(cur, wst, H1{}, fb, mem_a);
            X6STAMP(10);
        } else {
            half_step(cur, wst, I0{}, fb, mem_w);
            __builtin_amdgcn_sched_barrier(0);
            X6STAMP(1);
            wait_a_regs<13>(araw[decltype(setc)::value]);
            X6STAMP(3);
            convert_a(cur ^ 1, setc);
            __builtin_amdgcn_sched_barrier(0);
            X6STAMP(4);
            half_step(cur, wst, H1{}, fb, mem_a);
            X6STAMP(10);
        }
        __builtin_amdgcn_sched_barrier(0);
        X6STAMP(7);
        if (X6D(1 | 4)) asm volatile("s_waitcnt vmcnt(0)" ::: "memory");
        else asm volatile("s_waitcnt vmcnt(12)" ::: "memory");
        asm volatile("s_waitcnt lgkmcnt(0)" ::: "memory");
        X6STAMP(8);
        if (!X6D(32)) __builtin_amdgcn_s_barrier();
        X6STAMP(9);
        asm volatile("" ::: "memory");
    };
    for (int kt = kt0; kt < kt1; kt += 3) {
        step(kt, I1{});
        if (kt + 1 < kt1) step(kt + 1, I2{});
        if (kt + 2 < kt1) step(kt + 2, I0{});
    }
    asm volatile("s_waitcnt vmcnt(0)" ::: "memory");
#pragma unroll
    for (int s = 0; s < NA; ++s) asm volatile("" : "+v"(araw[s][0]), "+v"(araw[s][1]));
    X6STAMP(11);
    X6STAMP_FLUSH();

    if (FEED && qpart >= 0) {
        __amdgpu_buffer_rsrc_t srs = __builtin_amdgcn_make_buffer_rsrc(g.slabs, 0, (int)(unsigned)((size_t)g.slab_count * SLAB_FLOATS * 4), 0x00020000);
        const unsigned sbq = (slab0 + (unsigned)qpart) * 32u;
#pragma unroll
        for (int i = 0; i < 4; ++i)
#pragma unroll
            for (int j = 0; j < 2; ++j)
#pragma unroll
                for (int r4 = 0; r4 < 4; ++r4) {
                    const u32x4_t v4 = {__float_as_uint(acc[i][j][4 * r4]), __float_as_uint(acc[i][j][4 * r4 + 1]),
                                        __float_as_uint(acc[i][j][4 * r4 + 2]), __float_as_uint(acc[i][j][4 * r4 + 3])};
                    __builtin_amdgcn_raw_buffer_store_b128(v4, srs, ((sbq + (unsigned)((i * 2 + j) * 4 + r4)) * 512u + (unsigned)tid) * 16u, 0, 16);
                }
        asm volatile("s_waitcnt vmcnt(0)" ::: "memory");
        __syncthreads();
        unsigned* mailbox = reinterpret_cast<unsigned*>(smem + LDS_BYTES);
        if (tid == 0) *mailbox = __hip_atomic_fetch_add(g.arrive + tile, 1u, __ATOMIC_RELAXED, __HIP_MEMORY_SCOPE_AGENT);
#ifdef PGASR_LSTM_DIAG
        if (tid == 0 && diag_t_ < 4u) x6_feed_diag[8 + diag_t_] = (unsigned)wall_clock64();
#endif
        __syncthreads();
        const unsigned before = *mailbox;
        __syncthreads();
        if (before != parts - 1u) { if (FEED && g.single) return; continue; }
        for (unsigned qq = 0; qq < parts; ++qq) {
#pragma unroll
            for (int i = 0; i < 4; ++i)
#pragma unroll
                for (int j = 0; j < 2; ++j)
#pragma unroll
                    for (int r4 = 0; r4 < 4; ++r4) {
                        const u32x4_t v4 = __builtin_amdgcn_raw_buffer_load_b128(srs, (((slab0 + qq) * 32u + (unsigned)((i * 2 + j) * 4 + r4)) * 512u + (unsigned)tid) * 16u, 0, 16);
                        acc[i][j][4 * r4]     = qq == 0 ? __uint_as_float(v4.x) : acc[i][j][4 * r4]     + __uint_as_float(v4.x);
                        acc[i][j][4 * r4 + 1] = qq == 0 ? __uint_as_float(v4.y) : acc[i][j][4 * r4 + 1] + __uint_as_float(v4.y);
                        acc[i][j][4 * r4 + 2] = qq == 0 ? __uint_as_float(v4.z) : acc[i][j][4 * r4 + 2] + __uint_as_float(v4.z);
                        acc[i][j][4 * r4 + 3] = qq == 0 ? __uint_as_float(v4.w) : acc[i][j][4 * r4 + 3] + __uint_as_float(v4.w);
                    }
        }
    }

    const int cl = lane & 31, rq = lane >> 5;
    __amdgpu_buffer_rsrc_t crs = __builtin_amdgcn_make_buffer_rsrc(g.C, 0, (int)(unsigned)((size_t)g.M * g.ldc * 4), 0x00020000);
    __amdgpu_buffer_rsrc_t yrs = __builtin_amdgcn_make_buffer_rsrc(const_cast<float*>(g.dact_y ? g.dact_y : g.C), 0, (int)(unsigned)((size_t)g.M * g.ldc * 4), 0x00020000);
    float bsum[2];
#pragma unroll
    for (int j = 0; j < 2; ++j) bsum[j] = g.bias ? g.bias[n0 + wn * 64 + j * 32 + cl] : 0.f;
    if (g.dact_y) {
#pragma unroll
        for (int i = 0; i < 4; ++i)
#pragma unroll
            for (int j = 0; j < 2; ++j) {
                const unsigned o0 = (unsigned)(((size_t)(m0 + wm * 128 + i * 32 + 4 * rq) * g.ldc + n0 + wn * 64 + j * 32 + cl) * 4);
                float f[16];
#pragma unroll
                for (int r = 0; r < 16; ++r)
                    f[r] = __uint_as_float(__builtin_amdgcn_raw_buffer_load_b32(yrs, o0 + (unsigned)(((r & 3) + 8 * (r >> 2)) * g.ldc * 4), 0, 0)) > 0.f ? 1.f : g.slope;
#pragma unroll
                for (int r = 0; r < 16; ++r)
                    __builtin_amdgcn_raw_buffer_store_b32(__float_as_uint((acc[i][j][r] + bsum[j]) * f[r]), crs, o0 + (unsigned)(((r & 3) + 8 * (r >> 2)) * g.ldc * 4), 0, FEED ? 16 : 0);
            }
    } else {
#pragma unroll
        for (int i = 0; i < 4; ++i)
#pragma unroll
            for (int j = 0; j < 2; ++j) {
                const unsigned o0 = (unsigned)(((size_t)(m0 + wm * 128 + i * 32 + 4 * rq) * g.ldc + n0 + wn * 64 + j * 32 + cl) * 4);
#pragma unroll
                for (int r = 0; r < 16; ++r)
                    __builtin_amdgcn_raw_buffer_store_b32(__float_as_uint(acc[i][j][r] + bsum[j]), crs, o0 + (unsigned)(((r & 3) + 8 * (r >> 2)) * g.ldc * 4), 0, FEED ? 16 : 0);
            }
    }
    if (!FEED) return;
    asm volatile("s_waitcnt vmcnt(0)" ::: "memory");
    __syncthreads();
    if (tid == 0)
        __hip_atomic_fetch_add(g.tiles_done + (tbx < (g.nt_count >> 1) ? 0 : g.mt_count) + tby, 1u, __ATOMIC_RELAXED, __HIP_MEMORY_SCOPE_AGENT);
    if (g.single) return;
#ifdef PGASR_LSTM_DIAG
    {
        const unsigned nh_ = 8u * (unsigned)g.split8_tiles + 4u * (unsigned)g.split_tiles + 2u * (unsigned)g.split2_tiles;
        if (tid == 0 && diag_t_ >= nh_ && diag_t_ < nh_ + 4u) x6_feed_diag[1028 + (diag_t_ - nh_)] = (unsigned)wall_clock64();
    }
    if (tid == 0) {
        const unsigned slot_ = 16u + (unsigned)((tbx < (g.nt_count >> 1) ? 0 : g.mt_count) + tby);
        if (slot_ < 4096u) x6_feed_diag[slot_] = (unsigned)wall_clock64();
    }
#endif
  }
}
}

// ... 127 lines not shown
            unsigned h0, m0_, l0, h1, m1_, l1;
            split3(ra[s][j].x, ra[s][j].y, h0, m0_, l0); split3(ra[s][j].z, ra[s][j].w, h1, m1_, l1);
            *reinterpret_cast<u32x2_t*>(base + j * PITCH) = (u32x2_t){h0, h1};
            *reinterpret_cast<u32x2_t*>(base + PLANE_HALFS + j * PITCH) = (u32x2_t){m0_, m1_};
            *reinterpret_cast<u32x2_t*>(base + 2 * PLANE_HALFS + j * PITCH) = (u32x2_t){l0, l1};
            split3(rb[s][j].x, rb[s][j].y, h0, m0_, l0); split3(rb[s][j].z, rb[s][j].w, h1, m1_, l1);
            *reinterpret_cast<u32x2_t*>(base + 3 * PLANE_HALFS + j * PITCH) = (u32x2_t){h0, h1};
            *reinterpret_cast<u32x2_t*>(base + 4 * PLANE_HALFS + j * PITCH) = (u32x2_t){m0_, m1_};
            *reinterpret_cast<u32x2_t*>(base + 5 * PLANE_HALFS + j * PITCH) = (u32x2_t){l0, l1};
        }
    };

    f32x16 acc[4][2];
#pragma unroll
    for (int i = 0; i < 4; ++i)
#pragma unroll
        for (int j = 0; j < 2; ++j)
#pragma unroll
            for (int r = 0; r < 16; ++r) acc[i][j][r] = 0.f;

    auto multiply = [&](int buf, auto halfc, bf16x8_t (&bf)[2][3]) {
        constexpr int HALF = decltype(halfc)::value;
        const unsigned short* img = S + buf * BUF_HALFS + tro;
        if (HALF == 0) {
#pragma unroll
            for (int j = 0; j < 2; ++j)
#pragma unroll
                for (int p = 0; p < 3; ++p) bf[j][p] = tr_frag(img + (3 + p) * PLANE_HALFS + wn * 64 + j * 32);
        }
        bf16x8_t af[2][3];
#pragma unroll
        for (int i = 0; i < 2; ++i)
#pragma unroll
            for (int p = 0; p < 3; ++p) af[i][p] = tr_frag(img + p * PLANE_HALFS + wm * 128 + (2 * HALF + i) * 32);
        constexpr int PA[6] = {0, 0, 1, 0, 2, 1}, PB[6] = {0, 1, 0, 2, 0, 1};
#pragma unroll
        for (int i = 0; i < 2; ++i)
#pragma unroll
            for (int p = 0; p < 6; ++p)
#pragma unroll
                for (int j = 0; j < 2; ++j)
                    acc[2 * HALF + i][j] = __builtin_amdgcn_mfma_f32_32x32x16_bf16(af[i][PA[p]], bf[j][PB[p]], acc[2 * HALF + i][j], 0, 0, 0);
    };
#define T6_BARRIER() do { asm volatile("s_waitcnt lgkmcnt(0)" ::: "memory"); __builtin_amdgcn_s_barrier(); asm volatile("" ::: "memory"); } while (0)

    load(0, I0{});
    convert(0, I0{});
    load(1, I1{});
    load(2, I0{});
    T6_BARRIER();
    const bool mem = !(g.diag & 1), mul = !(g.diag & 2);
    auto step = [&](int kt, auto setc) {
        const int cur = kt & 1;
        bf16x8_t bf[2][3];
        if constexpr (PP >= 1) {
            if (w < 4) { if (mul) { multiply(cur, I0{}, bf); multiply(cur, I1{}, bf); } }
            else if (mem) { if (kt + 1 < nk) convert(cur ^ 1, setc); load(kt + 3, setc); }
            if (PP == 1) T6_BARRIER();
            if (w >= 4) { if (mul) { multiply(cur, I0{}, bf); multiply(cur, I1{}, bf); } }
            else if (mem) { if (kt + 1 < nk) convert(cur ^ 1, setc); load(kt + 3, setc); }
        } else if (w < 4) {
            if (mem) { if (kt + 1 < nk) convert(cur ^ 1, setc); load(kt + 3, setc); }
            if (mul) { multiply(cur, I0{}, bf); multiply(cur, I1{}, bf); }
        } else {
            if (mul) multiply(cur, I0{}, bf);
            if (mem) { if (kt + 1 < nk) convert(cur ^ 1, setc); load(kt + 3, setc); }
            if (mul) multiply(cur, I1{}, bf);
        }
        T6_BARRIER();
    };
    for (int kt = 0; kt < nk; kt += 2) {
        step(kt, I1{});
        if (kt + 1 < nk) step(kt + 1, I0{});
    }
#undef T6_BARRIER

    float* slab = g.partial + (size_t)z * g.M * g.N;
    __amdgpu_buffer_rsrc_t prs = __builtin_amdgcn_make_buffer_rsrc(slab, 0, (int)(unsigned)((size_t)g.M * g.N * 4), 0x00020000);
    const int cl = lane & 31, rq = lane >> 5;
#pragma unroll
    for (int i = 0; i < 4; ++i)
#pragma unroll
        for (int j = 0; j < 2; ++j) {
            const unsigned o0 = (unsigned)(((size_t)(m0 + wm * 128 + i * 32 + 4 * rq) * g.N + n0 + wn * 64 + j * 32 + cl) * 4);
#pragma unroll
            for (int r = 0; r < 16; ++r)
                __builtin_amdgcn_raw_buffer_store_b32(__float_as_uint(g.alpha * acc[i][j][r]), prs, o0 + (unsigned)(((r & 3) + 8 * (r >> 2)) * g.N * 4), 0, 0);
        }
    if (!g0.queue) return;
    __syncthreads();
  }
}
}

__global__ __launch_bounds__(256) void split_planes3_kernel(const float* __restrict__ src, int rows, int cols, int ld,
                                                            int transpose, unsigned short* __restrict__ hi,
                                                            unsigned short* __restrict__ mid, unsigned short* __restrict__ lo) {
    const size_t idx = (size_t)blockIdx.x * 256 + threadIdx.x;
    if (idx >= (size_t)rows * cols) return;
    int r, c;
    if (transpose) { c = (int)(idx / rows); r = (int)(idx % rows); }
    else { r = (int)(idx / cols); c = (int)(idx % cols); }
    unsigned h, m, l;
    split3(src[(size_t)r * ld + c], 0.f, h, m, l);
    hi[idx] = (unsigned short)h;
    mid[idx] = (unsigned short)m;
    lo[idx] = (unsigned short)l;
}

static int x6_var() {
    const char* e = getenv("PGASR_X6_VAR");
    return (e && e[0] == '0') ? 0 : 7;
}
__global__ __launch_bounds__(256) void pack_x6w_kernel(const float* __restrict__ src, int N, int K, int ld, int transpose, u32x4_t* __restrict__ dst) {
    const size_t idx = (size_t)blockIdx.x * 256 + threadIdx.x;
    if (idx >= (size_t)N * K / 8) return;
    const int nk = K / 16;
    const int pos = (int)(idx % 512), kt = (int)((idx / 512) % nk), tn = (int)(idx / 512 / nk);
    const int r = pos >> 1, cp = pos & 1, c = cp ^ ((r >> 3) & 1);
    const int n = tn * 256 + r, k0 = kt * 16 + c * 8;
    unsigned h[4], m[4], l[4];
#pragma unroll
    for (int e = 0; e < 4; ++e) {
        const float x0 = transpose ? src[(size_t)(k0 + 2 * e) * ld + n] : src[(size_t)n * ld + k0 + 2 * e];
        const float x1 = transpose ? src[(size_t)(k0 + 2 * e + 1) * ld + n] : src[(size_t)n * ld + k0 + 2 * e + 1];
        split3(x0, x1, h[e], m[e], l[e]);
    }
    u32x4_t* blk = dst + ((size_t)tn * nk + kt) * 3 * 512 + pos;
    blk[0] = (u32x4_t){h[0], h[1], h[2], h[3]};
    blk[512] = (u32x4_t){m[0], m[1], m[2], m[3]};
    blk[1024] = (u32x4_t){l[0], l[1], l[2], l[3]};
}

constexpr int X6_HEAD_HELP_DEFAULT = 1;
constexpr int X6_SPLIT8_GROUPS_DEFAULT = 0, X6_SPLIT4_GROUPS_DEFAULT = 16, X6_SPLIT2_GROUPS_DEFAULT = 16;
constexpr int X6_FWD_SPLIT4_GROUPS_DEFAULT = 2;
constexpr int X6_FEED_SPLIT_MAX = 128;
int x6_split_groups() {
    const char* e = getenv("PGASR_X6_SPLIT_GROUPS");
    const int v = e ? atoi(e) : X6_SPLIT4_GROUPS_DEFAULT;
    return v < 0 ? 0 : v;
}
int x6_split8_groups() {
    const char* e = getenv("PGASR_X6_SPLIT8_GROUPS");
    const int v = e ? atoi(e) : X6_SPLIT8_GROUPS_DEFAULT;
    return v < 0 ? 0 : v;
}
int x6_fwd_split_groups() {
    const char* e = getenv("PGASR_X6_FWD_SPLIT_GROUPS");
    const int v = e ? atoi(e) : X6_FWD_SPLIT4_GROUPS_DEFAULT;
    return v < 0 ? 0 : v;
}
int x6_split2_groups() {
    const char* e = getenv("PGASR_X6_SPLIT2_GROUPS");
    const int v = e ? atoi(e) : X6_SPLIT2_GROUPS_DEFAULT;
    return v < 0 ? 0 : v;
}
int x6_quarters(int K) {
    const char* e = getenv("PGASR_X6_QUARTER_K");
    const int kmin = e ? atoi(e) : 512;
    return (K >= kmin && K >= 16 * x6c::TK && K % (4 * x6c::TK) == 0) ? 4 : 1;
}

}

#ifdef PGASR_X6_DIAG
extern "C" int pgasr_diag_x6_stamps(long long* out) {
    return hipMemcpyFromSymbol(out, HIP_SYMBOL(x6_stamp_out), sizeof(long long) * 8 * 16) == hipSuccess ? 0 : 1;
}
#endif

extern "C" int pgasr_pack_x6w_planes(const float* src, int rows, int cols, int ld, int transpose, void* pack, void* stream) {
    if (!src || !pack || rows <= 0 || cols <= 0 || ld < cols) return PGASR_ERR_INVALID_ARG;
    const int N = transpose ? cols : rows, K = transpose ? rows : cols;
    if ((N % x6c::TN) || (K % x6c::TK) || (((size_t)pack) & 15)) return PGASR_ERR_UNSUPPORTED;
    const size_t chunks = (size_t)N * K / 8;
    PGASR_LAUNCH_KERNEL(pack_x6w_kernel, dim3((unsigned)((chunks + 255) / 256)), dim3(256), 0, (hipStream_t)stream, src, N, K, ld, transpose, (u32x4_t*)pack);
    PGASR_CHECK_LAUNCH();
    return PGASR_OK;
}

extern "C" int pgasr_split_bf16_planes3(const float* src, int rows, int cols, int ld, int transpose,
                                        unsigned short* hi, unsigned short* mid, unsigned short* lo, void* stream) {
    if (!src || !hi || !mid || !lo || rows <= 0 || cols <= 0 || ld < cols) return PGASR_ERR_INVALID_ARG;
    const size_t total = (size_t)rows * cols;
    PGASR_LAUNCH_KERNEL(split_planes3_kernel, dim3((unsigned)((total + 255) / 256)), dim3(256), 0, (hipStream_t)stream,
                        src, rows, cols, ld, transpose, hi, mid, lo);
    PGASR_CHECK_LAUNCH();
    return PGASR_OK;
}

static bool x6w_shape_ok(int M, int N, int K, const float* A, int lda, int ldc, const void* p0, const void* p1, const void* p2) {
    if ((K % x6c::TK) || K < 4 * x6c::TK || (N % x6c::TN) || (lda & 3)) return false;
    if ((((size_t)A) & 15) || (((size_t)p0) & 15) || (((size_t)p1) & 15) || (((size_t)p2) & 15)) return false;
    const size_t Mp = ((size_t)M + x6c::TM - 1) / x6c::TM * x6c::TM;
    if (Mp * ldc * 4 >= ((size_t)1 << 32) || Mp * lda * 4 >= ((size_t)1 << 32)) return false;
    return (M + x6c::TM - 1) / x6c::TM <= 65535;
}

extern "C" int pgasr_gemm_x6w_f32(int M, int N, int K, const float* A, int lda, const unsigned short* Whi,
                                  const unsigned short* Wmid, const unsigned short* Wlo, float* C, int ldc,
                                  const float* bias, const float* dact_y, float slope, void* stream) {
    if (!A || !Whi || (!Wmid != !Wlo) || !C || M <= 0 || N <= 0 || K <= 0 || lda < K || ldc < N) return PGASR_ERR_INVALID_ARG;
    if (!x6w_shape_ok(M, N, K, A, lda, ldc, Whi, Wmid, Wlo)) return PGASR_ERR_UNSUPPORTED;
    const size_t lds = (size_t)x6c::LDS_BYTES;
    const int var = x6_var();
    auto kern = var == 7 ? x6c::gemm_x6c_kernel<false, 7> : x6c::gemm_x6c_kernel<false, 0>;
    if (hipFuncSetAttribute((const void*)kern, hipFuncAttributeMaxDynamicSharedMemorySize, (int)lds) != hipSuccess)
        return PGASR_ERR_LAUNCH;
    DmaGemmArgs g{A, Whi, Wlo, C, M, N, K, lda, ldc, bias, dact_y, slope, nullptr, nullptr, nullptr, 0, 0, 0, 1, 0, nullptr, nullptr, 0, Wmid};
#ifdef PGASR_X6_DIAG
    if (const char* e = getenv("PGASR_X6_DIAG")) g.single = atoi(e);
#endif
    PGASR_LAUNCH_KERNEL(kern, dim3((unsigned)(N / x6c::TN), (unsigned)((M + x6c::TM - 1) / x6c::TM)), dim3(x6c::THREADS), lds,
                        (hipStream_t)stream, g);
    PGASR_CHECK_LAUNCH();
    return PGASR_OK;
}

extern "C" size_t pgasr_gemm_x6w_feed_workspace_bytes(void) { return 1024 + (size_t)X6_FEED_SPLIT_MAX * 4 * x6c::SLAB_FLOATS * 4; }

extern "C" int pgasr_gemm_x6w_feed_col_tiles(int N) { return (N > 0 && N % (2 * x6c::TN) == 0) ? N / (2 * x6c::TN) : 0; }

namespace {
void x6_feed_splits(int mt, int nt, int K, size_t workspace_bytes, int& split8, int& split, int& split2) {
    split8 = split = split2 = 0;
    if (x6_quarters(K) != 4) return;
    const size_t room = (workspace_bytes - 1024) / ((size_t)x6c::SLAB_FLOATS * 4);
    const int total = mt * nt;
    if (K >= 1024) { split8 = x6_split8_groups() * nt; split = x6_split_groups() * nt; split2 = x6_split2_groups() * nt; }
    else split = x6_fwd_split_groups() * nt;
    if (K % (8 * x6c::TK) || K < 32 * x6c::TK) { split += split8; split8 = 0; }
    if (split8 > total) split8 = total;
    if (split8 + split > total) split = total - split8;
    if (split8 + split + split2 > total) split2 = total - split8 - split;
    while (split8 + split + split2 > X6_FEED_SPLIT_MAX || (size_t)(8 * split8 + 4 * split + 2 * split2) > room) {
        if (split2 > 0) --split2; else if (split > 0) --split; else --split8;
    }
}
}

extern "C" int pgasr_gemm_x6w_feed_head_items(int M, int N, int K) {
    if (M <= 0 || N <= 0 || K <= 0 || pgasr_gemm_x6w_feed_col_tiles(N) == 0 || (K % x6c::TK)) return 0;
    int s8, s4, s2;
    x6_feed_splits((M + x6c::TM - 1) / x6c::TM, N / x6c::TN, K, pgasr_gemm_x6w_feed_workspace_bytes(), s8, s4, s2);
    const int items = 8 * s8 + 4 * s4;
    return items <= 256 ? items : 0;
}

extern "C" int pgasr_gemm_x6w_feed_phase_f32(int M, int N, int K, const float* A, int lda, const unsigned short* Whi,
                                             const unsigned short* Wmid, const unsigned short* Wlo, float* C, int ldc, const float* bias,
                                             const unsigned* xcc_busy, unsigned* tiles_done, int order, int phase, unsigned* ctrl,
                                             void* workspace, size_t workspace_bytes, void* stream) {
    if (!A || !Whi || (!Wmid != !Wlo) || !C || !tiles_done || M <= 0 || N <= 0 || K <= 0 || lda < K || ldc < N) return PGASR_ERR_INVALID_ARG;
    if (order < 0 || order > 1 || phase < 0 || phase > 2) return PGASR_ERR_INVALID_ARG;
    if (!workspace || workspace_bytes < 1024) return PGASR_ERR_WORKSPACE;
    if (!x6w_shape_ok(M, N, K, A, lda, ldc, Whi, Wmid, Wlo) || pgasr_gemm_x6w_feed_col_tiles(N) == 0) return PGASR_ERR_UNSUPPORTED;
    if ((size_t)M * ldc * 4 >= ((size_t)1 << 31)) return PGASR_ERR_UNSUPPORTED;
    if (phase != 0 && workspace_bytes < pgasr_gemm_x6w_feed_workspace_bytes()) return PGASR_ERR_WORKSPACE;
    hipStream_t st = (hipStream_t)stream;
    const int mt = (M + x6c::TM - 1) / x6c::TM, nt = N / x6c::TN;
    const size_t lds = (size_t)x6c::LDS_BYTES + 16;
    const int var = x6_var();
    auto kern = var == 7 ? x6c::gemm_x6c_kernel<true, 7> : x6c::gemm_x6c_kernel<true, 0>;
    if (hipFuncSetAttribute((const void*)kern, hipFuncAttributeMaxDynamicSharedMemorySize, (int)lds) != hipSuccess)
        return PGASR_ERR_LAUNCH;
    const int quarters = x6_quarters(K);
    int split8, split, split2;
    x6_feed_splits(mt, nt, K, phase != 0 ? pgasr_gemm_x6w_feed_workspace_bytes() : workspace_bytes, split8, split, split2);
    const int head_items = 8 * split8 + 4 * split;
    if (phase != 0 && (head_items <= 0 || head_items > 256)) return PGASR_ERR_UNSUPPORTED;
    if (!ctrl && phase != 2 && hipMemsetAsync(workspace, 0, 1024, st) != hipSuccess) return PGASR_ERR_LAUNCH;
    unsigned* cw = ctrl ? ctrl : (unsigned*)workspace;
    DmaGemmArgs g{A, Whi, Wlo, C, M, N, K, lda, ldc, bias, nullptr, 0.f, cw, xcc_busy, tiles_done, mt, nt, order,
                  quarters, split, (float*)((char*)workspace + 1024), cw + 64, 0, Wmid};
    g.split8_tiles = split8; g.split2_tiles = split2; g.slab_count = 8 * split8 + 4 * split + 2 * split2;
    if (phase == 1) {
        g.single = 1; g.xcc_busy = nullptr; g.head_help = 0;
        PGASR_LAUNCH_KERNEL(kern, dim3((unsigned)head_items), dim3(x6c::THREADS), lds, st, g);
        PGASR_CHECK_LAUNCH();
        return PGASR_OK;
    }
    {
        const char* eh = getenv("PGASR_X6_HEAD_HELP");
        g.head_help = (eh ? atoi(eh) : X6_HEAD_HELP_DEFAULT) != 0 && split8 + split > 0 && (phase == 0 || ctrl != nullptr);
    }
    int grid0 = 256;
    if (K < 1024 && xcc_busy) { const char* eg = getenv("PGASR_X6_FWD_FEED_GRID"); if (eg && atoi(eg) >= 16 && atoi(eg) <= 256) grid0 = atoi(eg); }
    for (int pass = 0; pass < 2; ++pass) {
        if (pass == 1) g.xcc_busy = nullptr;
        PGASR_LAUNCH_KERNEL(kern, dim3(pass == 0 ? grid0 : 256), dim3(x6c::THREADS), lds, st, g);
        PGASR_CHECK_LAUNCH();
    }
    return PGASR_OK;
}

extern "C" int pgasr_gemm_x6w_feed_f32(int M, int N, int K, const float* A, int lda, const unsigned short* Whi,
                                       const unsigned short* Wmid, const unsigned short* Wlo, float* C, int ldc, const float* bias,
                                       const unsigned* xcc_busy, unsigned* tiles_done, int order,
                                       void* workspace, size_t workspace_bytes, void* stream) {
    return pgasr_gemm_x6w_feed_phase_f32(M, N, K, A, lda, Whi, Wmid, Wlo, C, ldc, bias, xcc_busy, tiles_done, order, 0, nullptr, workspace, workspace_bytes, stream);
}

int pgasr_internal_tn6_launch(PgasrTn256Args a, int masked_then_unmasked, hipStream_t st, const PgasrTn256Args* second) {
    PgasrTn256Args b{};
    const int tk = a.tslabs ? t6::TK : 32;
    if (!pgasr_internal_tn256_ok(a, tk)) return PGASR_ERR_UNSUPPORTED;
    if (second) {
        if (!a.queue || second->splitk != a.splitk || !pgasr_internal_tn256_ok(*second, tk)) return PGASR_ERR_UNSUPPORTED;
        b = *second;
    }
    const size_t lds = (size_t)t6::LDS_BYTES;
    const char* ev = getenv("PGASR_T6_VAR");
    const int pp = (ev && ev[0] >= '0' && ev[0] <= '2') ? ev[0] - '0' : 0;
    auto kplain = pp == 2 ? t6::gemm_t6_kernel<false, 2> : pp == 1 ? t6::gemm_t6_kernel<false, 1> : t6::gemm_t6_kernel<false, 0>;
    auto kgated = pp == 2 ? t6::gemm_t6_kernel<true, 2> : pp == 1 ? t6::gemm_t6_kernel<true, 1> : t6::gemm_t6_kernel<true, 0>;
    if (hipFuncSetAttribute((const void*)kplain, hipFuncAttributeMaxDynamicSharedMemorySize, (int)lds) != hipSuccess)
        return PGASR_ERR_LAUNCH;
    const unsigned nitems = (unsigned)((a.N / t6::TN) * (a.M / t6::TM)) * (unsigned)(a.batch * a.splitk);
    if (!a.queue) {
        PGASR_LAUNCH_KERNEL(kplain, dim3(nitems), dim3(t6::THREADS), lds, st, a, b);
        PGASR_CHECK_LAUNCH();
        return PGASR_OK;
    }
    if (a.gate && hipFuncSetAttribute((const void*)kgated, hipFuncAttributeMaxDynamicSharedMemorySize, (int)lds) != hipSuccess)
        return PGASR_ERR_LAUNCH;
    const unsigned* busy = a.xcc_busy;
    const char* eg = getenv("PGASR_T6_GRID");
    const int grid0 = (eg && atoi(eg) >= 8 && atoi(eg) <= 256) ? atoi(eg) : 256;
    for (int pass = 0; pass < ((masked_then_unmasked && busy) ? 2 : 1); ++pass) {
        a.xcc_busy = (pass == 0) ? busy : nullptr;
        b.xcc_busy = a.xcc_busy;
        const int grid = (pass == 0 && busy) ? grid0 : 256;
        if (a.gate) PGASR_LAUNCH_KERNEL(kgated, dim3(grid), dim3(t6::THREADS), lds, st, a, b);
        else        PGASR_LAUNCH_KERNEL(kplain, dim3(grid), dim3(t6::THREADS), lds, st, a, b);
        PGASR_CHECK_LAUNCH();
    }
    return PGASR_OK;
}

#ifdef PGASR_LSTM_DIAG
extern "C" int pgasr_diag_x6_feed(unsigned* out, int reset) {
    if (hipMemcpyFromSymbol(out, HIP_SYMBOL(x6_feed_diag), sizeof(unsigned) * 4096) != hipSuccess) return 1;
    if (reset) { static unsigned z[4096]; if (hipMemcpyToSymbol(HIP_SYMBOL(x6_feed_diag), z, sizeof(z)) != hipSuccess) return 1; }
    return 0;
}
#endif
```

policy_gradient_asr_amd/csrc/x3w_common.h:

```cpp
#pragma once
#include "common.h"

namespace {

typedef __attribute__((ext_vector_type(16))) float f32x16;
typedef __attribute__((ext_vector_type(8))) __bf16 bf16x8_t;
typedef __attribute__((ext_vector_type(4))) unsigned u32x4_t;

struct DmaGemmArgs {
    const float* A; const unsigned short* Whi; const unsigned short* Wlo; float* C;
    int M, N, K, lda, ldc;
    const float* bias; const float* dact_y; float slope;
    unsigned* queue;
    const unsigned* xcc_busy;
    unsigned* tiles_done;
    int mt_count, nt_count, order;
    int quarters;
    int split_tiles;
    float* slabs;
    unsigned* arrive;
    int single;
    const unsigned short* Wmid;
    int head_help;
    int split8_tiles, split2_tiles;
    int slab_count;
};

__device__ __forceinline__ void dma16(const void* gsrc, void* lds_base) {
    __builtin_amdgcn_global_load_lds((const void __attribute__((address_space(1)))*)gsrc,
                                     (void __attribute__((address_space(3)))*)lds_base, 16, 0, 0);
}

__device__ __forceinline__ void split2(float x0, float x1, unsigned& hi_pk, unsigned& lo_pk) {
    typedef __attribute__((ext_vector_type(2))) __bf16 bf2;
    typedef __attribute__((ext_vector_type(2))) float f2;
    const bf2 h = __builtin_convertvector((f2){x0, x1}, bf2);
    hi_pk = __builtin_bit_cast(unsigned, h);
    const float h0 = __uint_as_float(hi_pk << 16), h1 = __uint_as_float(hi_pk & 0xFFFF0000u);
    const bf2 l = __builtin_convertvector((f2){x0 - h0, x1 - h1}, bf2);
    lo_pk = __builtin_bit_cast(unsigned, l);
}

__device__ __forceinline__ void split3(float x0, float x1, unsigned& hi_pk, unsigned& mid_pk, unsigned& lo_pk) {
    typedef __attribute__((ext_vector_type(2))) __bf16 bf2;
    typedef __attribute__((ext_vector_type(2))) float f2;
    hi_pk = __builtin_bit_cast(unsigned, __builtin_convertvector((f2){x0, x1}, bf2));
    float r0 = x0 - __uint_as_float(hi_pk << 16), r1 = x1 - __uint_as_float(hi_pk & 0xFFFF0000u);
    mid_pk = __builtin_bit_cast(unsigned, __builtin_convertvector((f2){r0, r1}, bf2));
    r0 -= __uint_as_float(mid_pk << 16); r1 -= __uint_as_float(mid_pk & 0xFFFF0000u);
    lo_pk = __builtin_bit_cast(unsigned, __builtin_convertvector((f2){r0, r1}, bf2));
}

__device__ __forceinline__ void swizzled_tile(int& bx, int& by) {
    const unsigned gx = gridDim.x, gy = gridDim.y;
    const unsigned nwg = gx * gy;
    const unsigned L = blockIdx.x + gx * blockIdx.y;
    const unsigned q = nwg / 8, r = nwg % 8;
    const unsigned xcd = L % 8, i = L / 8;
    const unsigned t = (xcd < r ? xcd * (q + 1) : r * (q + 1) + (xcd - r) * q) + i;
    bx = (int)(t % gx); by = (int)(t / gx);
}


}
```

policy_gradient_asr_amd/functional.py:

```python
import os

import torch

from . import hipops
from . import streams

HID = hipops.HID
FEED_AHEAD = os.environ.get("PGASR_FEED_AHEAD", "1") != "0"
JOIN_FEED = os.environ.get("PGASR_JOIN_FEED", "0") == "1"
FEED_BWD = os.environ.get("PGASR_FEED_BWD", "1") != "0"
STREAM_DW = os.environ.get("PGASR_STREAM_DW", "1") != "0"
LEAKY_SLOPE = 0.01


def _pick_splitk(M, N, K, target_wgs=512, batch=1, beside_sweep=False):
    if M % 256 == 0 and N % 256 == 0 and K % 32 == 0 and K >= 64:
        tiles = (M // 256) * (N // 256) * batch
        sk = max(1, min((128 if beside_sweep else 256) // tiles, K // 256))
        while sk > 1 and (sk - 1) * (-(-K // sk // 32) * 32) >= K:
            sk -= 1
        return sk
    tiles = ((M + 127) // 128) * ((N + 127) // 128)
    sk = max(1, min(64, target_wgs // max(tiles, 1)))
    while sk > 1 and K // sk < 256:
        sk //= 2
    return max(sk, 1)


class grad_overlap:
    enabled = False
    confine = os.environ.get("PGASR_CONFINE", "1") != "0"
    confine_feed = os.environ.get("PGASR_CONFINE_FEED", "1") != "0"
    _sides = {}
    _pendings = {}

    @classmethod
    def _key(cls):
        return torch.cuda.current_stream().cuda_stream

    _main_of = {}

    @classmethod
    def side_stream(cls):
        k = cls._key()
        if k not in cls._sides:
            cls._sides[k] = streams.side_stream("weight_gradients")
            cls._main_of[cls._sides[k].cuda_stream] = k
        return cls._sides[k]

    upper_grads_hook = None
    tail_dx_first = os.environ.get("PGASR_TAIL_DX_FIRST", "1") != "0"
    split_tail = True
    _sides2 = {}

    @classmethod
    def second_side_stream(cls):
        k = cls._key()
        if k not in cls._sides2:
            cls._sides2[k] = streams.side_stream("feed")
        return cls._sides2[k]

    _sides3 = {}
    _streamed_unjoined = {}

    @classmethod
    def third_side_stream(cls):
        k = cls._key()
        if k not in cls._sides3:
            cls._sides3[k] = streams.side_stream("streamed_weight_gradients")
        return cls._sides3[k]

    _recent = {}
    _feed_unjoined = {}

    @classmethod
    def note_event(cls, ev):
        cls._recent[cls._key()] = ev

    @classmethod
    def take_event(cls):
        return cls._recent.pop(cls._key(), None)

    @classmethod
    def pending(cls):
        return cls._pendings.setdefault(cls._key(), [])

    _deferred = {}

    @classmethod
    def flush(cls, busy_ptr=0, launched_after=None, first=None):
        pending = cls.pending()
        if not pending and first is None:
            return
        side = cls.side_stream()
        prev = hipops.GEMM_XCC_BUSY_PTR
        hipops.GEMM_XCC_BUSY_PTR = busy_ptr if cls.confine else 0
        try:
            with torch.cuda.stream(side):
                for ready, fn in pending:
                    side.wait_event(ready)
                if launched_after is not None and busy_ptr:
                    side.wait_event(launched_after)
                    hipops.stream_gate(busy_ptr)
                if first is not None:
                    first()
                for ready, fn in pending:
                    fn()
        finally:
            hipops.GEMM_XCC_BUSY_PTR = prev
            del pending[:]

    @classmethod
    def finish(cls):
        if cls._deferred:
            cls._deferred.clear()
            raise RuntimeError("a deferred input gradient was never consumed by a BLSTM layer (grad_overlap/FEED_AHEAD)")
        cls.flush()
        cls._recent.pop(cls._key(), None)
        if cls._key() in cls._sides:
            torch.cuda.current_stream().wait_stream(cls.side_stream())
        if cls._streamed_unjoined.pop(cls._key(), False) and cls._key() in cls._sides3:
            torch.cuda.current_stream().wait_stream(cls._sides3[cls._key()])
        if cls._feed_unjoined.pop(cls._key(), False) and cls._key() in cls._sides2:
            torch.cuda.current_stream().wait_stream(cls.second_side_stream())


AFFINE_DW_SPLITK = 2


class InstNormAffineFn(torch.autograd.Function):

    @staticmethod
    def forward(ctx, x, weight, bias, consumer_applies_dact=False):
        B, F, T = x.shape
        N = weight.shape[0]
        x = x.contiguous(); weight = weight.contiguous(); bias = bias.contiguous()
        ctx.consumer_applies_dact = bool(consumer_applies_dact)
        mean, rstd = hipops.instnorm_stats(x, 1e-5)
        y = torch.empty(T, B, N, dtype=torch.float32, device=x.device)
        hipops.gemm(x, weight, y, M=T, N=N, K=F, transA=True, transB=True, lda=T, ldb=F, ldc=B * N,
                    strideA=F * T, strideB=0, strideC=N, batch=B, bias=bias, act=1, slope=LEAKY_SLOPE,
                    norm_operand=1, shift=mean, scale=rstd, precision=0)
        ctx.save_for_backward(x, weight, mean, rstd, y)
        ctx.bias_ref, ctx.weight_ref = bias, weight
        return y

    @staticmethod
    def backward(ctx, dy):
        x, weight, mean, rstd, y = ctx.saved_tensors
        B, F, T = x.shape
        N = weight.shape[0]
        if ctx.consumer_applies_dact:
            dpre = dy.contiguous()
        else:
            dpre = torch.where(y > 0, dy, dy * LEAKY_SLOPE).contiguous()
        bg = getattr(ctx.bias_ref, "grad", None)
        if grad_overlap.enabled and bg is not None and bg.is_contiguous() and bg.dtype == torch.float32:
            main = torch.cuda.current_stream()
            side = grad_overlap.side_stream()
            ready = torch.cuda.Event()
            ready.record()
            with torch.cuda.stream(side):
                side.wait_event(ready)
                hipops.colsum(dpre, T * B, N, N, bg, accumulate=True)
            streams.hold(dpre, side)
            wg = getattr(ctx.weight_ref, "grad", None)
            direct = wg is not None and wg.is_contiguous() and wg.dtype == torch.float32 and tuple(wg.shape) == (N, F)
            dW = wg if direct else torch.empty(N, F, dtype=torch.float32, device=x.device)
            hipops.gemm(dpre, x, dW, M=N, N=F, K=T, transA=True, transB=True, lda=B * N, ldb=T, ldc=F,
                        strideA=N, strideB=F * T, strideC=0, batch=B, sum_batches=True, norm_operand=2,
                        shift=mean, scale=rstd, accumulate=direct, splitk=AFFINE_DW_SPLITK if T >= 256 else 1)
            return (None, None if direct else dW, None, None)
        return (None, *InstNormAffineFn.param_grads(x, mean, rstd, dpre, N), None)

    @staticmethod
    def param_grads(x, mean, rstd, dpre, N):
        B, F, T = x.shape
        dW = torch.empty(N, F, dtype=torch.float32, device=x.device)
        hipops.gemm(dpre, x, dW, M=N, N=F, K=T, transA=True, transB=True, lda=B * N, ldb=T, ldc=F,
                    strideA=N, strideB=F * T, strideC=0, batch=B, sum_batches=True, norm_operand=2,
                    shift=mean, scale=rstd, splitk=AFFINE_DW_SPLITK if T >= 256 else 1)
        db = torch.empty(N, dtype=torch.float32, device=x.device)
        hipops.colsum(dpre, T * B, N, N, db)
        return dW, db


class DropoutFn(torch.autograd.Function):

    @staticmethod
    def forward(ctx, x, p, seed, offset, *opt):
        ctx.cfg = (float(p), int(seed), int(offset))
        x = x.contiguous()
        ctx.fused = bool(opt[0]) if opt else False
        ctx.nopt = len(opt)
        if ctx.fused:
            ctx.save_for_backward(x)
        return hipops.dropout(x, p, seed, offset)

    @staticmethod
    def backward(ctx, dy):
        p, seed, offset = ctx.cfg
        rec = grad_overlap._deferred.get(dy.data_ptr())
        if rec is not None and not ctx.fused and rec["drop"] is None and dy.shape == rec["dx"].shape:
            rec["drop"] = (p, seed, offset)
            return (dy, None, None, None) + (None,) * ctx.nopt
        dact = ctx.saved_tensors[0] if ctx.fused else None
        return (hipops.dropout(dy.contiguous(), p, seed, offset, dact_y=dact, slope=LEAKY_SLOPE), None, None, None) + (None,) * ctx.nopt


class LinearFn(torch.autograd.Function):

    @staticmethod
    def forward(ctx, x, weight, bias):
        shp = x.shape
        x2 = x.contiguous().view(-1, shp[-1])
        rows, K = x2.shape
        N = weight.shape[0]
        weight = weight.contiguous()
        y = torch.empty(rows, N, dtype=torch.float32, device=x.device)
        hipops.gemm(x2, weight, y, M=rows, N=N, K=K, transB=True, bias=bias.contiguous())
        ctx.save_for_backward(x2, weight)
        ctx.shp = shp
        ctx.param_refs = (weight, bias)
        return y.view(*shp[:-1], N)

    @staticmethod
    def backward(ctx, dy):
        x2, weight = ctx.saved_tensors
        rows, K = x2.shape
        N = weight.shape[0]
        dy2 = dy.contiguous().view(rows, N)
        dx = torch.empty(rows, K, dtype=torch.float32, device=dy.device)
        hipops.gemm(dy2, weight, dx, M=rows, N=K, K=N)
        wg, bg = (p.grad for p in ctx.param_refs)
        if grad_overlap.enabled and wg is not None and bg is not None and wg.is_contiguous() and bg.is_contiguous():
            done = torch.cuda.Event()
            done.record()
            grad_overlap.note_event(done)

            def weight_grads():
                hipops.gemm(dy2, x2, wg, M=N, N=K, K=rows, transA=True, lda=N, splitk=_pick_splitk(N, K, rows), accumulate=True)
                hipops.colsum(dy2, rows, N, N, bg, accumulate=True)
            grad_overlap.pending().append((done, weight_grads))
            side = grad_overlap.side_stream()
            streams.hold(dy2, side); streams.hold(x2, side)
            return dx.view(ctx.shp), None, None
        dW = torch.empty(N, K, dtype=torch.float32, device=dy.device)
        hipops.gemm(dy2, x2, dW, M=N, N=K, K=rows, transA=True, lda=N, splitk=_pick_splitk(N, K, rows))
        db = torch.empty(N, dtype=torch.float32, device=dy.device)
        hipops.colsum(dy2, rows, N, N, db)
        return dx.view(ctx.shp), dW, db


class HeadFn(torch.autograd.Function):

    @staticmethod
    def forward(ctx, x, weight, bias):
        shp = x.shape
        x2 = x.contiguous().view(-1, shp[-1])
        weight = weight.contiguous()
        logits, lp = hipops.head_logsoftmax(x2, weight, bias.contiguous())
        ctx.save_for_backward(x2, weight)
        ctx.shp = shp
        ctx.param_refs = (weight, bias)
        lp = lp.view(*shp[:-1], -1)
        ctx.mark_non_differentiable(lp)
        return logits.view(*shp[:-1], -1), lp

    @staticmethod
    def backward(ctx, dy, _dlp=None):
        return LinearFn.backward(ctx, dy)


class LogSoftmaxFn(torch.autograd.Function):
    @staticmethod
    def forward(ctx, logits):
        lp = hipops.log_softmax_rows(logits.contiguous())
        ctx.save_for_backward(lp)
        return lp

    @staticmethod
    def backward(ctx, g):
        (lp,) = ctx.saved_tensors
        return g - torch.exp(lp) * g.sum(dim=-1, keepdim=True)


class BLSTMLayerFn(torch.autograd.Function):

    @staticmethod
    def forward(ctx, x, lengths, dact_y, sweep_follows, prepacked, out_dropout, w_ih_f, w_hh_f, b_ih_f, b_hh_f, w_ih_r, w_hh_r, b_ih_r, b_hh_r):
        T, B, I = x.shape
        x = x.contiguous()
        if prepacked is None:
            prepacked = prepack_blstm((w_ih_f, w_hh_f, b_ih_f, b_hh_f, w_ih_r, w_hh_r, b_ih_r, b_hh_r), I)
        elif prepacked.ready is not None:
            torch.cuda.current_stream().wait_event(prepacked.ready)
        wih_perm, bias_perm, pack_f, pack_b = prepacked.wih_perm, prepacked.bias_perm, prepacked.pack_f, prepacked.pack_b
        ctx.planes_t = prepacked.planes_t
        npl = len(prepacked.planes) if prepacked.planes is not None else hipops.LSTM_PLANES
        ctx.nplanes = npl
        ctx.fed_bwd = prepacked.fed_bwd
        prepacked.fed_bwd = None
        ctx.slab_words = prepacked.slab
        prepacked.slab = None
        G = 2 * 4 * HID
        gates = torch.empty(T, B, G, dtype=torch.float32, device=x.device)
        out = torch.empty(T, B, 2 * HID, dtype=torch.float32, device=x.device)
        cbuf = torch.empty(T, B, 2 * HID, dtype=torch.float32, device=x.device)
        ctx.out_dropout = tuple(out_dropout) if out_dropout is not None else None
        out_drop = torch.empty_like(out) if out_dropout is not None else None
        dkw = {"out_drop": out_drop, "drop": ctx.out_dropout}
        x3w = prepacked.planes is not None and hipops.gemm_x3w_ok(T * B, G, I, planes=npl)
        if (x3w and FEED_AHEAD and hipops.lstm_fed_ok(T, B) and hipops.x3w_feed_col_tiles(G, npl) > 0
                and hipops.streams_concurrent(grad_overlap.second_side_stream())):
            main = torch.cuda.current_stream()
            side = grad_overlap.second_side_stream()
            need_words = 2 * ((T * B + 255) // 256)
            done = prepacked.fed_fwd if (prepacked.fed_fwd is not None and prepacked.fed_fwd.numel() >= need_words) else None
            prepacked.fed_fwd = None
            if done is None:
                done = torch.zeros(need_words, dtype=torch.int32, device=x.device)
            head = hipops.x3w_feed_head_items(G, I, planes=npl) > 0
            ws_feed = hipops.gemm_x3w_feed(x, prepacked.planes, gates, T * B, G, I, bias_perm, 0, done, phase=1) if head else None
            zeroed = torch.cuda.Event()
            zeroed.record()
            hipops.lstm_layer_fwd(gates, out, cbuf, pack_f, lengths, T, B, fed=done, fed_need=hipops.x3w_feed_col_tiles(G, npl), **dkw)
            side.wait_event(zeroed)
            busy = hipops.lstm_busy_ptr(T, B, False, x.device)
            with torch.cuda.stream(side):
                hipops.stream_gate(busy)
                hipops.gemm_x3w_feed(x, prepacked.planes, gates, T * B, G, I, bias_perm, busy if grad_overlap.confine_feed else 0, done,
                                     phase=2 if head else 0, ws=ws_feed)
            if ws_feed is not None:
                streams.hold(ws_feed, side)
            for t_ in (x, gates, done, bias_perm) + tuple(prepacked.planes):
                streams.hold(t_, side)
            grad_overlap._feed_unjoined[main.cuda_stream] = True
            if JOIN_FEED:
                main.wait_stream(side)
        else:
            if x3w and npl == 3 and hipops.x3w_feed_col_tiles(G, npl) > 0 and T * B * G * 4 < 2 ** 31:
                hipops.gemm_x3w_feed(x, prepacked.planes, gates, T * B, G, I, bias_perm, 0,
                                     torch.zeros(2 * ((T * B + 255) // 256), dtype=torch.int32, device=x.device))
            elif x3w:
                hipops.gemm_x3w(x, prepacked.planes, gates, T * B, G, I, bias=bias_perm)
            else:
                hipops.gemm(x, wih_perm, gates, M=T * B, N=G, K=I, transB=True, bias=bias_perm)
            hipops.lstm_layer_fwd(gates, out, cbuf, pack_f, lengths, T, B, **dkw)
        ctx.save_for_backward(x, lengths, gates, out, cbuf, wih_perm, pack_b, dact_y if dact_y is not None else x.new_empty(0))
        ctx.has_dact = dact_y is not None
        ctx.sweep_follows = bool(sweep_follows)
        ctx.param_refs = (w_ih_f, w_hh_f, b_ih_f, b_hh_f, w_ih_r, w_hh_r, b_ih_r, b_hh_r)
        return out if out_drop is None else out_drop

    @staticmethod
    def backward(ctx, dout):
        x, lengths, gates, out, cbuf, wih_perm, pack_b, dact_y = ctx.saved_tensors
        T, B, I = x.shape
        G = 2 * 4 * HID
        dev = x.device
        npl = ctx.nplanes
        dout = dout.contiguous()
        rec = grad_overlap._deferred.pop(dout.data_ptr(), None) if grad_overlap.enabled else None
        if ctx.out_dropout is not None:
            if rec is not None and rec["drop"] is None and dout.shape == rec["dx"].shape:
                rec["drop"] = ctx.out_dropout
            else:
                dout = hipops.dropout(dout, *ctx.out_dropout)
        if grad_overlap.enabled:
            before = grad_overlap.take_event()
            if before is None:
                before = torch.cuda.Event()
                before.record()
        targets = [p.grad for p in ctx.param_refs]
        stream_own = (grad_overlap.enabled and STREAM_DW and all(t is not None and t.is_contiguous() for t in targets)
                      and hipops.lstm_wgrads_ok(T, B, I, npl) and hipops.lstm_fed_ok(T, B)
                      and hipops.streams_concurrent(grad_overlap.third_side_stream()))
        slab = None
        if stream_own:
            slab = ctx.slab_words if (ctx.slab_words is not None and ctx.slab_words.numel() >= 64) else None
            ctx.slab_words = None
            if slab is None:
                slab = torch.zeros(64, dtype=torch.int32, device=dev)
        if rec is not None:
            if grad_overlap.enabled and rec["head"]():
                before = torch.cuda.Event()
                before.record()
            sweep_ws, dbias_part = hipops.lstm_layer_bwd(gates, out, cbuf, dout, pack_b, lengths, T, B, want_dbias=True,
                                                         fed=rec["done"], fed_need=rec["need"], drop=rec["drop"], slab=slab)
        else:
            sweep_ws, dbias_part = hipops.lstm_layer_bwd(gates, out, cbuf, dout, pack_b, lengths, T, B, want_dbias=True, slab=slab)
        dg = gates
        if grad_overlap.enabled:
            busy = hipops.lstm_busy_ptr(T, B, True, dev)
            grad_overlap.flush(busy, launched_after=before, first=(lambda: rec["launch"](busy)) if rec is not None else None)
            if rec is not None:
                streams.hold(dout, grad_overlap.side_stream())
            fed_done = None
            if stream_own and grad_overlap._key() in grad_overlap._sides:
                fed_done = torch.cuda.Event()
                with torch.cuda.stream(grad_overlap.side_stream()):
                    fed_done.record()
            swept = torch.cuda.Event()
            swept.record()
            grad_overlap.note_event(swept)
            if not ctx.sweep_follows and grad_overlap.upper_grads_hook is not None:
                grad_overlap.upper_grads_hook(swept)
        dx = None
        defer = (ctx.needs_input_grad[0] and grad_overlap.enabled and FEED_AHEAD and FEED_BWD and ctx.sweep_follows and not ctx.has_dact
                 and ctx.planes_t is not None and hipops.gemm_x3w_ok(T * B, I, G, planes=npl) and I % 256 == 0 and I == 2 * HID
                 and hipops.x3w_feed_col_tiles(I, npl) > 0
                 and hipops.lstm_fed_ok(T, B) and hipops.streams_concurrent(grad_overlap.side_stream()))
        if defer:
            dx = torch.empty(T, B, I, dtype=torch.float32, device=dev)
            need_words = 2 * ((T * B + 255) // 256)
            done = ctx.fed_bwd if (ctx.fed_bwd is not None and ctx.fed_bwd.numel() >= need_words) else None
            ctx.fed_bwd = None
            if done is None:
                done = torch.zeros(need_words, dtype=torch.int32, device=dev)
            planes_t = ctx.planes_t

            feed_ws = []

            def head(dg=dg, dx=dx, done=done, planes_t=planes_t):
                if hipops.x3w_feed_head_items(I, G, planes=npl) > 0:
                    feed_ws.append(hipops.gemm_x3w_feed(dg, planes_t, dx, T * B, I, G, None, 0, done, order=1, phase=1))
                    return True
                return False

            def launch(busy_ptr, dg=dg, dx=dx, done=done, planes_t=planes_t):
                hipops.gemm_x3w_feed(dg, planes_t, dx, T * B, I, G, None, busy_ptr if grad_overlap.confine_feed else 0, done, order=1,
                                     phase=2 if feed_ws else 0, ws=feed_ws[0] if feed_ws else None)
                side_ = torch.cuda.current_stream()
                for t_ in (dg, dx, done) + tuple(planes_t) + tuple(feed_ws):
                    streams.hold(t_, side_)
            grad_overlap._deferred[dx.data_ptr()] = {"dx": dx, "done": done, "need": hipops.x3w_feed_col_tiles(I, npl), "drop": None,
                                                     "launch": launch, "head": head}
        elif ctx.needs_input_grad[0]:
            dx = torch.empty(T, B, I, dtype=torch.float32, device=dev)
            if (ctx.sweep_follows and not ctx.has_dact and ctx.planes_t is not None and hipops.gemm_x3w_ok(T * B, I, G, planes=npl)
                    and I == 2 * HID and hipops.x3w_feed_col_tiles(I, npl) > 0 and T * B * I * 4 < 2 ** 31):
                done = torch.zeros(2 * ((T * B + 255) // 256), dtype=torch.int32, device=dev)
                hipops.gemm_x3w_feed(dg, ctx.planes_t, dx, T * B, I, G, None, 0, done, order=1)
            elif ctx.planes_t is not None and hipops.gemm_x3w_ok(T * B, I, G, planes=npl):
                hipops.gemm_x3w(dg, ctx.planes_t, dx, T * B, I, G,
                                dact_y=dact_y if ctx.has_dact else None, slope=LEAKY_SLOPE)
            else:
                hipops.gemm(dg, wih_perm, dx, M=T * B, N=I, K=G, dact_y=dact_y if ctx.has_dact else None,
                            slope=LEAKY_SLOPE)
        def weight_grads(accumulate_into=None, hh_stream=None):
            cur = torch.cuda.current_stream()
            if hipops.lstm_wgrads_ok(T, B, I, npl):
                dwih = torch.empty(G, I, dtype=torch.float32, device=dev)
                dwhh = torch.empty(2, 4 * HID, HID, dtype=torch.float32, device=dev)
                hipops.lstm_wgrads(dg, x, out, T, B, I, dwih, dwhh, busy_ptr=hipops.GEMM_XCC_BUSY_PTR, planes=npl)
                dbias = torch.empty(G, dtype=torch.float32, device=dev)
                hipops.colsum(dbias_part, dbias_part.shape[0], G, G, dbias)
                if accumulate_into is not None:
                    hipops.lstm_unpack_grads(dwih, dbias, dwhh, I, accumulate_into, accumulate=True)
                    return None
                gl_ = [torch.empty(4 * HID, I, device=dev), torch.empty(4 * HID, HID, device=dev),
                       torch.empty(4 * HID, device=dev), torch.empty(4 * HID, device=dev),
                       torch.empty(4 * HID, I, device=dev), torch.empty(4 * HID, HID, device=dev),
                       torch.empty(4 * HID, device=dev), torch.empty(4 * HID, device=dev)]
                hipops.lstm_unpack_grads(dwih, dbias, dwhh, I, gl_)
                return gl_

            def hh():
                dwhh_ = torch.zeros(2, 4 * HID, HID, dtype=torch.float32, device=dev)
                if T > 1:
                    K = (T - 1) * B
                    hipops.gemm(dg, out, dwhh_, M=4 * HID, N=HID, K=K, transA=True, lda=G, ldb=2 * HID, ldc=HID,
                                a_off=B * G, b_off=0, strideA=4 * HID - B * G, strideB=B * 2 * HID + HID,
                                strideC=4 * HID * HID, batch=2, splitk=_pick_splitk(4 * HID, HID, K, 256, batch=2, beside_sweep=ctx.sweep_follows))
                return dwhh_
            if hh_stream is not None:
                hh_stream.wait_stream(cur)
                with torch.cuda.stream(hh_stream):
                    dwhh = hh()
                    for t_ in (dg, out):
                        streams.hold(t_, hh_stream)
                streams.hold(dwhh, cur)
            dwih = torch.empty(G, I, dtype=torch.float32, device=dev)
            hipops.gemm(dg, x, dwih, M=G, N=I, K=T * B, transA=True, lda=G,
                        splitk=_pick_splitk(G, I, T * B, 512 if ctx.sweep_follows else 256, beside_sweep=ctx.sweep_follows))
            dbias = torch.empty(G, dtype=torch.float32, device=dev)
            hipops.colsum(dbias_part, dbias_part.shape[0], G, G, dbias)
            if hh_stream is not None:
                cur.wait_stream(hh_stream)
                if hh_stream is grad_overlap._sides2.get(grad_overlap._main_of.get(cur.cuda_stream)):
                    grad_overlap._feed_unjoined.pop(grad_overlap._main_of[cur.cuda_stream], None)
            else:
                dwhh = hh()
            if accumulate_into is not None:
                hipops.lstm_unpack_grads(dwih, dbias, dwhh, I, accumulate_into, accumulate=True)
                return None
            gl = [torch.empty(4 * HID, I, device=dev), torch.empty(4 * HID, HID, device=dev),
                  torch.empty(4 * HID, device=dev), torch.empty(4 * HID, device=dev),
                  torch.empty(4 * HID, I, device=dev), torch.empty(4 * HID, HID, device=dev),
                  torch.empty(4 * HID, device=dev), torch.empty(4 * HID, device=dev)]
            hipops.lstm_unpack_grads(dwih, dbias, dwhh, I, gl)
            return gl

        if stream_own:
            s3 = grad_overlap.third_side_stream()
            with torch.cuda.stream(s3):
                s3.wait_event(before)
                if fed_done is not None:
                    s3.wait_event(fed_done)
                hipops.stream_gate(busy, need=2 * ((B + 15) // 16), timeout_us=5000, running=slab)
                dwih = torch.empty(G, I, dtype=torch.float32, device=dev)
                dwhh = torch.empty(2, 4 * HID, HID, dtype=torch.float32, device=dev)
                hipops.lstm_wgrads(dg, x, out, T, B, I, dwih, dwhh, busy_ptr=busy if grad_overlap.confine else 0,
                                   slab=slab, err_ws=sweep_ws, planes=npl)
                s3.wait_event(swept)
                dbias = torch.empty(G, dtype=torch.float32, device=dev)
                hipops.colsum(dbias_part, dbias_part.shape[0], G, G, dbias)
                hipops.lstm_unpack_grads(dwih, dbias, dwhh, I, targets, accumulate=True)
            for t_ in (dg, x, out, dbias_part, slab):
                streams.hold(t_, s3)
            grad_overlap._streamed_unjoined[grad_overlap._key()] = True
            return (dx, None, None, None, None, None) + (None,) * 8
        if grad_overlap.enabled and all(t is not None and t.is_contiguous() for t in targets):
            side = grad_overlap.side_stream()
            tail = not ctx.sweep_follows
            hh_stream = grad_overlap.second_side_stream() if (tail and grad_overlap.split_tail) else None
            ready = swept
            if tail and dx is not None and grad_overlap.tail_dx_first:
                ready = torch.cuda.Event()
                ready.record()
            grad_overlap.pending().append((ready, lambda: weight_grads(accumulate_into=targets, hh_stream=hh_stream)))
            if tail:
                grad_overlap.flush()
            for t_ in (dg, x, out, dbias_part):
                streams.hold(t_, side)
            return (dx, None, None, None, None, None) + (None,) * 8
        gl = weight_grads()
        return (dx, None, None, None, None, None, *gl)


class PackedBLSTM:
    __slots__ = ("wih_perm", "bias_perm", "pack_f", "pack_b", "planes", "planes_t", "ready", "fed_fwd", "fed_bwd", "slab")


def prepack_blstm(params, in_dim):
    pk = PackedBLSTM()
    params = [p.contiguous() for p in params]
    pk.wih_perm, pk.bias_perm, pk.pack_f, pk.pack_b = hipops.lstm_pack(params, in_dim)
    G = 2 * 4 * HID
    npl = hipops.LSTM_PLANES
    ok = in_dim % 128 == 0 if npl == 2 else (in_dim % 256 == 0 and in_dim >= 64)
    pk.planes = hipops.split_planes(pk.wih_perm, planes=npl) if ok else None
    pk.planes_t = hipops.split_planes(pk.wih_perm, transpose=True, planes=npl) if ok else None
    pk.ready = None
    pk.fed_fwd = pk.fed_bwd = pk.slab = None
    return pk


def prepack_blstm_layers(layer_params, in_dims, rows=0):
    main = torch.cuda.current_stream()
    side = grad_overlap.side_stream()
    side.wait_stream(main)
    out = []
    with torch.cuda.stream(side):
        nl = len(in_dims)
        words = 2 * ((rows + 255) // 256)
        counters = torch.zeros(3 * nl, max(words, 64), dtype=torch.int32, device=layer_params[0][0].device) if rows > 0 else None
        if counters is not None:
            streams.hold(counters, main)
        for li, (params, in_dim) in enumerate(zip(layer_params, in_dims)):
            pk = prepack_blstm(params, in_dim)
            if counters is not None:
                pk.fed_fwd, pk.fed_bwd, pk.slab = counters[2 * li], counters[2 * li + 1], counters[2 * nl + li]
            for t in (pk.wih_perm, pk.bias_perm, pk.pack_f, pk.pack_b) + tuple(pk.planes or ()) + tuple(pk.planes_t or ()):
                streams.hold(t, main)
            out.append(pk)
        ready = torch.cuda.Event()
        ready.record()
        out[0].ready = ready
    return out


def blstm_layer(x, lengths, params, dact_y=None, sweep_follows=False, prepacked=None, out_dropout=None):
    return BLSTMLayerFn.apply(x, lengths, dact_y, sweep_follows, prepacked, out_dropout, *params)
```

policy_gradient_asr_amd/hipops.py:

```python
import collections
import os

import torch

_os_environ_get = os.environ.get

from . import _lib


def _stream():
    return torch.cuda.current_stream().cuda_stream


def _req(t, dtype, name):
    if t is None:
        return None
    if not t.is_cuda:
        raise _lib.PgasrError(f"{name} must live on the GPU (got {t.device}); there is no CPU path")
    if t.dtype != dtype:
        raise _lib.PgasrError(f"{name} must be {dtype} (got {t.dtype})")
    if not t.is_contiguous():
        raise _lib.PgasrError(f"{name} must be contiguous")
    return t

# ... 519 lines not shown
    _req(scores, torch.float32, "scores"); _req(path, torch.int32, "path")
    _req(coef, torch.float32, "coef"); _req(lengths, torch.int32, "lengths")
    T, B, V = scores.shape
    if out is None:
        if accumulate:
            raise _lib.PgasrError("accumulate=True needs an output tensor")
        out = torch.empty_like(scores)
    _req(out, torch.float32, "out")
    st = lib.pgasr_reinforce_grad(_p(scores), _p(path), _p(coef), _p(lengths), T, B, V, int(bool(accumulate)),
                                  _p(out), _stream())
    _lib.check(st, "pgasr_reinforce_grad")
    return out


GEMM_XCC_BUSY_PTR = 0
GEMM_PRECISION = 0
LSTM_PLANES = 3

PRECISION_MODES = {"bf16x3": (1, 2), "f32": (0, 3)}
_precision = "f32"


def set_precision(mode):
    global GEMM_PRECISION, LSTM_PLANES, _precision
    if mode not in PRECISION_MODES:
        raise ValueError(f"precision mode must be one of {sorted(PRECISION_MODES)}")
    GEMM_PRECISION, LSTM_PLANES = PRECISION_MODES[mode]
    _precision = mode


def get_precision():
    return _precision


class precision:

    def __init__(self, mode):
        self.mode = mode

    def __enter__(self):
        self.prev = _precision
        set_precision(self.mode)
        return self

    def __exit__(self, *a):
        set_precision(self.prev)
        return False


def gemm(A, B, C, M, N, K, transA=False, transB=False, lda=None, ldb=None, ldc=None, alpha=1.0,
         strideA=0, strideB=0, strideC=0, batch=1, sum_batches=False, splitk=1, bias=None, bias2=None,
         act=0, slope=0.01, accumulate=False, dact_y=None, norm_operand=0, shift=None, scale=None,
         a_off=0, b_off=0, c_off=0, precision=None, xcc_busy=None):
    lib = _lib.load()
    if precision is None:
        precision = GEMM_PRECISION
    for t, nm in ((A, "A"), (B, "B"), (C, "C"), (bias, "bias"), (bias2, "bias2"), (dact_y, "dact_y"),
                  (shift, "shift"), (scale, "scale")):
        if t is not None:
            if not t.is_cuda or t.dtype != torch.float32:
                raise _lib.PgasrError(f"gemm operand {nm} must be a float32 GPU tensor")
    lda = lda if lda is not None else (M if transA else K)
    ldb = ldb if ldb is not None else (K if transB else N)
    ldc = ldc if ldc is not None else N
    nbytes = lib.pgasr_gemm_workspace_bytes(M, N, batch, splitk, int(sum_batches))
    ws = _workspace(nbytes, C.device, "gemm")
    with _timed("gemm_f32"):
      st = lib.pgasr_gemm_f32(int(transA), int(transB), M, N, K, float(alpha),
                            A.data_ptr() + 4 * a_off, lda, int(strideA), B.data_ptr() + 4 * b_off, ldb, int(strideB),
                            C.data_ptr() + 4 * c_off, ldc, int(strideC), batch, int(sum_batches), splitk,
                            _p(bias), _p(bias2), act, float(slope), int(accumulate), _p(dact_y),
                            norm_operand, _p(shift), _p(scale), int(precision), int(GEMM_XCC_BUSY_PTR if xcc_busy is None else xcc_busy), _p(ws), ws.numel() if ws is not None else 0, _stream())
    _lib.check(st, "pgasr_gemm_f32")
    return C


X6_PACKED = _os_environ_get("PGASR_X6_PACKED", "1") != "0"


class X6Pack:
    __slots__ = ("pack", "N", "K")

    def __init__(self, pack, N, K):
        self.pack, self.N, self.K = pack, N, K

    def __len__(self):
        return 3

    def __iter__(self):
        return iter((self.pack,))


def split_planes(w, transpose=False, planes=None, packed=None):
    lib = _lib.load()
    _req(w, torch.float32, "w")
    if w.dim() != 2 or w.stride(1) != 1:
        raise _lib.PgasrError("split_planes wants a row-major 2-D tensor")
    planes = LSTM_PLANES if planes is None else int(planes)
    if planes not in (2, 3):
        raise _lib.PgasrError("split_planes: 2 or 3 planes")
    rows, cols = w.shape
    shape = (cols, rows) if transpose else (rows, cols)
    if planes == 3 and (X6_PACKED if packed is None else packed) and shape[0] % 256 == 0 and shape[1] % 16 == 0:
        pack = torch.empty(shape[0] * shape[1] * 6, dtype=torch.uint8, device=w.device)
        _lib.check(lib.pgasr_pack_x6w_planes(w.data_ptr(), rows, cols, w.stride(0), int(transpose), pack.data_ptr(), _stream()), "pgasr_pack_x6w_planes")
        return X6Pack(pack, shape[0], shape[1])
    out = tuple(torch.empty(shape, dtype=torch.int16, device=w.device) for _ in range(planes))
    if planes == 3:
        st = lib.pgasr_split_bf16_planes3(w.data_ptr(), rows, cols, w.stride(0), int(transpose), *[t.data_ptr() for t in out], _stream())
    else:
        st = lib.pgasr_split_bf16_planes(w.data_ptr(), rows, cols, w.stride(0), int(transpose), *[t.data_ptr() for t in out], _stream())
    _lib.check(st, "pgasr_split_bf16_planes")
    return out


def gemm_x3w_ok(M, N, K, lda=None, planes=2):
    lda = K if lda is None else lda
    if planes == 3:
        Mp = (M + 255) // 256 * 256
        return K % 16 == 0 and K >= 64 and N % 256 == 0 and lda % 4 == 0 and M > 0 and Mp * max(N, lda) * 4 < 2 ** 32
    return K % 32 == 0 and N % 128 == 0 and lda % 4 == 0 and M > 0


def _plane_ptrs(planes):
    if isinstance(planes, X6Pack):
        return planes.pack.data_ptr(), None, None
    return tuple(t.data_ptr() for t in planes)


def _check_planes(planes, N, K, what):
    if isinstance(planes, X6Pack):
        if (planes.N, planes.K) != (N, K) or not planes.pack.is_cuda:
            raise _lib.PgasrError(f"{what}: packed planes are for a ({planes.N}, {planes.K}) weight, the product wants ({N}, {K})")
        return
    if len(planes) not in (2, 3):
        raise _lib.PgasrError(f"{what}: planes must be a (hi, lo) or (hi, mid, lo) tuple")
    for t in planes:
        if tuple(t.shape) != (N, K) or t.dtype != torch.int16 or not t.is_contiguous() or not t.is_cuda:
            raise _lib.PgasrError(f"{what} planes must be contiguous int16 (N, K) GPU tensors")


def gemm_x3w(A, planes, C, M, N, K, lda=None, ldc=None, bias=None, dact_y=None, slope=0.01):
    lib = _lib.load()
    for t, nm in ((A, "A"), (C, "C"), (bias, "bias"), (dact_y, "dact_y")):
        if t is not None and (not t.is_cuda or t.dtype != torch.float32):
            raise _lib.PgasrError(f"gemm_x3w operand {nm} must be a float32 GPU tensor")
    _check_planes(planes, N, K, "gemm_x3w")
    with _timed("gemm_x6c" if len(planes) == 3 else "gemm_x3c"):
        if len(planes) == 3:
            st = lib.pgasr_gemm_x6w_f32(M, N, K, A.data_ptr(), K if lda is None else lda, *_plane_ptrs(planes),
                                        C.data_ptr(), N if ldc is None else ldc, _p(bias), _p(dact_y), float(slope), _stream())
        else:
            st = lib.pgasr_gemm_x3w_f32(M, N, K, A.data_ptr(), K if lda is None else lda, planes[0].data_ptr(), planes[1].data_ptr(),
                                        C.data_ptr(), N if ldc is None else ldc, _p(bias), _p(dact_y), float(slope), _stream())
    _lib.check(st, "pgasr_gemm_x6w_f32" if len(planes) == 3 else "pgasr_gemm_x3w_f32")
    return C


def colsum(X, rows, cols, ld, out, out2=None, accumulate=False):
    lib = _lib.load()
    nbytes = lib.pgasr_colsum_workspace_bytes(rows, cols)
    ws = _workspace(nbytes, X.device, "colsum")
    st = lib.pgasr_colsum_f32(_p(X), rows, cols, ld, _p(out), _p(out2), int(accumulate), _p(ws), ws.numel(), _stream())
    _lib.check(st, "pgasr_colsum_f32")
    return out


def instnorm_stats(x, eps=1e-5):
    lib = _lib.load()
    _req(x, torch.float32, "x")
    B, F, T = x.shape
    mean = torch.empty(B, dtype=torch.float32, device=x.device)
    rstd = torch.empty(B, dtype=torch.float32, device=x.device)
    _lib.check(lib.pgasr_instnorm_stats(_p(x), B, F, T, float(eps), _p(mean), _p(rstd), _stream()), "pgasr_instnorm_stats")
    return mean, rstd


def log_softmax_rows(logits):
    lib = _lib.load()
    _req(logits, torch.float32, "logits")
    V = logits.shape[-1]
    out = torch.empty_like(logits)
    _lib.check(lib.pgasr_log_softmax_rows(_p(logits), logits.numel() // V, V, _p(out), _stream()), "pgasr_log_softmax_rows")
    return out


HID = 256


def lstm_pack(params, in_dim):
    lib = _lib.load()
    dev = params[0].device
    for t in params:
        _req(t, torch.float32, "lstm parameter")
    wih_perm = torch.empty(2 * 4 * HID, in_dim, dtype=torch.float32, device=dev)
    bias_perm = torch.empty(2 * 4 * HID, dtype=torch.float32, device=dev)
    nb = lib.pgasr_lstm_pack_bytes(0, LSTM_PLANES)
    pack_f = torch.empty(nb, dtype=torch.uint8, device=dev)
    pack_b = torch.empty(nb, dtype=torch.uint8, device=dev)
    st = lib.pgasr_lstm_pack_weights(*[_p(t) for t in params], in_dim, _p(wih_perm), _p(bias_perm),
                                     _p(pack_f), _p(pack_b), LSTM_PLANES, _stream())
    _lib.check(st, "pgasr_lstm_pack_weights")
    return wih_perm, bias_perm, pack_f, pack_b


def _lstm_flags(pack):
    planes = 3 if pack.numel() == _lib.load().pgasr_lstm_pack_bytes(0, 3) else 2
    return LSTM_FLAGS | (2 if planes == 3 else 0)


def lstm_unpack_grads(dwih_perm, dbias_perm, dwhh_perm, in_dim, grads, accumulate=False):
    lib = _lib.load()
    st = lib.pgasr_lstm_unpack_grads(_p(dwih_perm), _p(dbias_perm), _p(dwhh_perm), in_dim,
                                     *[_p(g) for g in grads], int(accumulate), _stream())
    _lib.check(st, "pgasr_lstm_unpack_grads")


_lstm_err_checks = []


def _lstm_ws(T, B, backward, device):
    lib = _lib.load()
    nbytes = lib.pgasr_lstm_workspace_bytes(T, B, int(backward))
    return _workspace(nbytes, device, "lstm_bwd" if backward else "lstm_fwd")


import os as _os
LSTM_FLAGS = int(_os.environ.get("PGASR_LSTM_FLAGS", "0"), 0)


def lstm_layer_fwd(gates, out, cbuf, pack_f, lengths, T, B, fed=None, fed_need=0, out_drop=None, drop=None):
    lib = _lib.load()
    ws = _lstm_ws(T, B, False, gates.device)
    p, seed, offset = drop if (drop is not None and out_drop is not None) else (0.0, 0, 0)
    if out_drop is not None:
        _req(out_drop, torch.float32, "out_drop")
        if out_drop.numel() != out.numel() or drop is None:
            raise _lib.PgasrError("lstm_layer_fwd: out_drop must have out's size and come with drop = (p, seed, offset)")
    dargs = (_p(out_drop), float(p), int(seed) & (2 ** 64 - 1), int(offset) & 0xFFFFFFFF)
    with _timed("lstm_fwd_kernel"):
        if fed is None:
            st = lib.pgasr_lstm_layer_fwd(_p(gates), _p(out), _p(cbuf), _p(pack_f), _p(lengths), T, B, _lstm_flags(pack_f), *dargs,
                                          _p(ws), ws.numel(), _stream())
        else:
            if fed.dtype != torch.int32 or not fed.is_cuda or fed.numel() < 2 * ((T * B + 255) // 256):
                raise _lib.PgasrError("lstm_layer_fwd: fed must be an int32 GPU tensor of 2 * ceil(T*B/256) words")
            st = lib.pgasr_lstm_layer_fwd_fed(_p(gates), _p(out), _p(cbuf), _p(pack_f), _p(lengths), T, B, _lstm_flags(pack_f),
                                              _p(fed), int(fed_need), *dargs, _p(ws), ws.numel(), _stream())
    _lib.check(st, "pgasr_lstm_layer_fwd_fed" if fed is not None else "pgasr_lstm_layer_fwd")
    return ws


def lstm_fed_ok(T, B):
    return bool(_lib.load().pgasr_lstm_fed_ok(T, B, LSTM_FLAGS))


def x3w_feed_col_tiles(N, planes=2):
    lib = _lib.load()
    return int(lib.pgasr_gemm_x6w_feed_col_tiles(int(N)) if planes == 3 else lib.pgasr_gemm_x3w_feed_col_tiles(int(N)))


FEED_HEAD_GROUPS = int(_os_environ_get("PGASR_FEED_HEAD", "0"))




def x3w_feed_head_items(N, K, groups=None, planes=2):
    groups = FEED_HEAD_GROUPS if groups is None else groups
    if planes == 3:
        return 0
    return int(_lib.load().pgasr_gemm_x3w_feed_head_items(int(N), int(K), int(groups))) if groups > 0 else 0


def gemm_x3w_feed(A, planes, C, M, N, K, bias, busy_ptr, tiles_done, order=0, phase=0, ws=None, ctrl=None):
    lib = _lib.load()
    for t, nm in ((A, "A"), (C, "C"), (bias, "bias")):
        if t is not None and (not t.is_cuda or t.dtype != torch.float32):
            raise _lib.PgasrError(f"gemm_x3w_feed operand {nm} must be a float32 GPU tensor")
    _check_planes(planes, N, K, "gemm_x3w_feed")
    if tiles_done.dtype != torch.int32 or tiles_done.numel() < 2 * ((M + 255) // 256):
        raise _lib.PgasrError("gemm_x3w_feed: tiles_done must hold 2 * ceil(M/256) int32 words")
    if len(planes) == 3:
        if phase == 2 and ws is None:
            raise _lib.PgasrError("gemm_x3w_feed: phase 2 continues the queue of a phase-1 call: pass its workspace")
        if ws is None:
            ws = _workspace(lib.pgasr_gemm_x6w_feed_workspace_bytes(), C.device, "x6w_feed")
        with _timed("gemm_feed_x6c"):
            if ctrl is not None and (ctrl.dtype != torch.int32 or ctrl.numel() < 256 or not ctrl.is_contiguous()):
                raise _lib.PgasrError("gemm_x3w_feed: ctrl = 256 zeroed int32 words")
            st = lib.pgasr_gemm_x6w_feed_phase_f32(M, N, K, A.data_ptr(), K, *_plane_ptrs(planes), C.data_ptr(), N, _p(bias),
                                                   busy_ptr, tiles_done.data_ptr(), int(order), int(phase), _p(ctrl), _p(ws), ws.numel(), _stream())
        _lib.check(st, "pgasr_gemm_x6w_feed_phase_f32")
        return ws if phase == 1 else C
    if ws is None:
        ws = _workspace(lib.pgasr_gemm_x3w_feed_workspace_bytes(), C.device, "x3w_feed")
    with _timed("gemm_feed_x3w"):
        st = lib.pgasr_gemm_x3w_feed_f32(M, N, K, A.data_ptr(), K, planes[0].data_ptr(), planes[1].data_ptr(), C.data_ptr(), N, _p(bias),
                                         busy_ptr, tiles_done.data_ptr(), int(order), int(phase), FEED_HEAD_GROUPS if phase else 0,
                                         _p(ws), ws.numel(), _stream())
    _lib.check(st, "pgasr_gemm_x3w_feed_f32")
    return ws if phase == 1 else C


def lstm_layer_bwd(gates, out, cbuf, dout, pack_b, lengths, T, B, want_dbias=False, fed=None, fed_need=0, drop=None, slab=None):
    lib = _lib.load()
    ws = _lstm_ws(T, B, True, gates.device)
    part = torch.empty((B + 15) // 16, 2 * 4 * HID, dtype=torch.float32, device=gates.device) if want_dbias else None
    with _timed("lstm_bwd_kernel"):
        if slab is not None:
            words = slab
            if words.dtype != torch.int32 or not words.is_cuda or words.numel() < 2 * ((B + 15) // 16):
                raise _lib.PgasrError("lstm_layer_bwd: slab_done must be an int32 GPU tensor of 2 * ceil(B/16) words")
            p, seed, offset = drop if drop is not None else (0.0, 0, 0)
            st = lib.pgasr_lstm_layer_bwd_streamed(_p(gates), _p(out), _p(cbuf), _p(dout), _p(pack_b), _p(lengths), T, B, _lstm_flags(pack_b),
                                                   _p(part), _p(fed), int(fed_need), float(p), int(seed), int(offset),
                                                   _p(words), _p(ws), ws.numel(), _stream())
        elif fed is None:
            st = lib.pgasr_lstm_layer_bwd(_p(gates), _p(out), _p(cbuf), _p(dout), _p(pack_b), _p(lengths), T, B, _lstm_flags(pack_b),
                                          _p(part), _p(ws), ws.numel(), _stream())
        else:
            if fed.dtype != torch.int32 or not fed.is_cuda or fed.numel() < 2 * ((T * B + 255) // 256):
                raise _lib.PgasrError("lstm_layer_bwd: fed must be an int32 GPU tensor of 2 * ceil(T*B/256) words")
            p, seed, offset = drop if drop is not None else (0.0, 0, 0)
            st = lib.pgasr_lstm_layer_bwd_fed(_p(gates), _p(out), _p(cbuf), _p(dout), _p(pack_b), _p(lengths), T, B, _lstm_flags(pack_b),
                                              _p(part), _p(fed), int(fed_need), float(p), int(seed), int(offset),
                                              _p(ws), ws.numel(), _stream())
    _lib.check(st, "pgasr_lstm_layer_bwd")
    return (ws, part) if want_dbias else ws


def lstm_wgrad_slabs(T):
    import ctypes
    lib = _lib.load()
    n = lib.pgasr_lstm_wgrad_slabs(int(T), None, 0)
    edges = (ctypes.c_int * (n + 1))()
    lib.pgasr_lstm_wgrad_slabs(int(T), ctypes.addressof(edges), n + 1)
    return [int(edges[i]) for i in range(n + 1)]


def lstm_wgrads_ok(T, B, in_dim, planes=None):
    planes = LSTM_PLANES if planes is None else int(planes)
    return T >= 2 and in_dim % 256 == 0 and B > 0 and B % (16 if planes == 3 else 32) == 0 and T * B * 2048 * 4 < 2 ** 31


def lstm_wgrads(dgates, x, out, T, B, in_dim, dwih, dwhh, busy_ptr=0, slab=None, err_ws=None, planes=None):
    lib = _lib.load()
    planes = LSTM_PLANES if planes is None else int(planes)
    for t_, nm in ((dgates, "dgates"), (x, "x"), (out, "out"), (dwih, "dwih"), (dwhh, "dwhh")):
        _req(t_, torch.float32, nm)
    nbytes = lib.pgasr_lstm_wgrads_workspace_bytes(T, in_dim)
    ws = _workspace(nbytes, dgates.device, "gemm")
    err_ptr = 0
    if err_ws is not None:
        import ctypes
        off = ctypes.c_size_t(0)
        _lib.check(lib.pgasr_lstm_error_offset(B, 1, ctypes.byref(off)), "pgasr_lstm_error_offset")
        err_ptr = err_ws.data_ptr() + off.value
    with _timed("gemm_t6" if planes == 3 else "gemm_t256"):
        st = lib.pgasr_lstm_wgrads_streamed(_p(dgates), _p(x), _p(out), T, B, in_dim, _p(dwih), _p(dwhh), int(busy_ptr),
                                            _p(slab), err_ptr, planes, _p(ws), ws.numel(), _stream())
    _lib.check(st, "pgasr_lstm_wgrads_streamed")


def lstm_check_error(ws, B, backward):
    import ctypes
    lib = _lib.load()
    off = ctypes.c_size_t(0)
    _lib.check(lib.pgasr_lstm_error_offset(B, int(backward), ctypes.byref(off)), "pgasr_lstm_error_offset")
    flag = int(ws[off.value:off.value + 4].view(torch.int32).item())
    if flag != 0:
        raise _lib.PgasrError("persistent LSTM sweep timed out waiting for its cluster (status 5)")


def lstm_assert_no_timeouts():
    lib = _lib.load()
    for key, ws in list(_ws_cache.items()):
        if not key[0].startswith("lstm"):
            continue
        st = lib.pgasr_lstm_status(ws.data_ptr(), ws.numel(), 1, int(key[0] == "lstm_bwd"), _stream())
        if st == _lib.TIMEOUT:
            raise _lib.PgasrError(f"persistent LSTM sweep timed out (status {st}: {lib.pgasr_status_string(st).decode()}) "
                                  f"in workspace {key[0]!r}; its outputs and every gradient since are invalid")
        _lib.check(st, "pgasr_lstm_status")


def lstm_error_words(device):
    return [w.data_ptr() for w in lstm_error_word_tensors(device)]


def lstm_error_word_tensors(device):
    import ctypes
    lib = _lib.load()
    cur = torch.cuda.current_stream().cuda_stream
    out = []
    for tag, backward in (("lstm_fwd", 0), ("lstm_bwd", 1)):
        ws = _ws_cache.get((tag, device, cur))
        if ws is None:
            continue
        off = ctypes.c_size_t(0)
        _lib.check(lib.pgasr_lstm_error_offset(1, backward, ctypes.byref(off)), "pgasr_lstm_error_offset")
        out.append(ws[off.value:off.value + 4].view(torch.int32))
    return out


def attention_ctx(dec, enc):
    lib = _lib.load()
    _req(dec, torch.float32, "dec"); _req(enc, torch.float32, "enc")
    if enc.dim() != 3 or dec.shape[-1] != enc.shape[2]:
        raise _lib.PgasrError("attention_ctx: enc (B,T,H) and dec (..., H) with the same H (model.py:69: the bmm output is (H,H))")
    B, T, H = enc.shape
    NQ = dec.numel() // H
    if NQ % B:
        raise _lib.PgasrError("attention_ctx: dec must hold a multiple of B rows")
    ctx = torch.empty_like(dec)
    _lib.check(lib.pgasr_attention_ctx(_p(dec), _p(enc), NQ, B, T, H, _p(ctx), _stream()), "pgasr_attention_ctx")
    return ctx


def lstm_cell(gh, xp, c, h, h_out=None):
    lib = _lib.load()
    for n, t in (("gh", gh), ("xp", xp), ("c", c), ("h", h)):
        _req(t, torch.float32, n)
    B, H = c.shape
    if gh.shape != (B, 4 * H) or xp.shape != (B, 4 * H) or h.shape != (B, H) or not (gh.is_contiguous() and xp.is_contiguous() and c.is_contiguous() and h.is_contiguous()):
        raise _lib.PgasrError("lstm_cell: gh, xp (B,4H) and c, h (B,H), all contiguous")
    if h_out is not None:
        _req(h_out, torch.float32, "h_out")
        if h_out.shape != (B, H) or not h_out.is_contiguous():
            raise _lib.PgasrError("lstm_cell: h_out (B,H) contiguous")
    _lib.check(lib.pgasr_lstm_cell_f32(_p(gh), _p(xp), _p(c), _p(h), _p(h_out), B, H, _stream()),
               "pgasr_lstm_cell_f32")


def ctc_beam_search(log_probs, lengths=None, beam=5, blank=0, collapse=False, out=None, generic=False,
                    lm=None, lm_alpha=0.0, lm_beta=0.0):
    lib = _lib.load()
    if not log_probs.is_cuda or log_probs.dtype not in (torch.float32, torch.float64):
        raise _lib.PgasrError("log_probs must be a float32/float64 GPU tensor")
    if log_probs.stride(2) != 1:
        raise _lib.PgasrError("log_probs must be contiguous in its last dimension")
    T, B, V = log_probs.shape
    _req(lengths, torch.int32, "lengths")
    lm_table, lm_order = None, 0
    if lm is not None:
        if lm.vocab != V or lm.blank != int(blank):
            raise ValueError(f"the LM is over {lm.vocab} symbols with blank {lm.blank}; the search has {V} symbols and blank {int(blank)}")
        lm_table, lm_order = lm.device_table(log_probs.device), lm.order
    nbytes = lib.pgasr_beam_workspace_bytes(T, B, V, beam)
    ws = _workspace(nbytes, log_probs.device, "beam")
    if out is not None:
        tokens, tl = out
        _req(tokens, torch.int32, "out tokens"); _req(tl, torch.int32, "out lengths")
        if tokens.numel() != B * T or tl.numel() != B:
            raise _lib.PgasrError("ctc_beam_search: out tensors must hold (B,T) and (B) int32")
    else:
        tokens = torch.zeros(B, T, dtype=torch.int32, device=log_probs.device)
        tl = torch.empty(B, dtype=torch.int32, device=log_probs.device)
    score = torch.empty(B, dtype=torch.float64, device=log_probs.device)
    with _timed("beam_search"):
        st = lib.pgasr_ctc_beam_search_lm(_p(log_probs), int(log_probs.dtype == torch.float64), log_probs.stride(0),
                                          log_probs.stride(1), _p(lengths), T, B, V, int(beam), int(blank), int(bool(collapse)) | (2 if generic else 0),
                                          _p(tokens), _p(tl), _p(score), _p(ws), ws.numel(), _stream(),
                                          _p(lm_table), lm_order, float(lm_alpha), float(lm_beta))
    _lib.check(st, "pgasr_ctc_beam_search_lm")
    return tokens, tl, score


def dropout(x, p, seed, offset, out=None, dact_y=None, slope=0.01):
    lib = _lib.load()
    _req(x, torch.float32, "x"); _req(dact_y, torch.float32, "dact_y")
    if dact_y is not None and dact_y.numel() != x.numel():
        raise _lib.PgasrError("dropout: dact_y must have x's size")
    if out is None:
        out = torch.empty_like(x)
    _lib.check(lib.pgasr_dropout(_p(x), _p(out), x.numel(), float(p), int(seed) & (2 ** 64 - 1),
                                 int(offset) & 0xFFFFFFFF, _p(dact_y), float(slope), _stream()), "pgasr_dropout")
    return out


def stream_copy(dst, src, workgroups=8):
    lib = _lib.load()
    if not dst.is_cuda or not dst.is_contiguous() or not src.is_contiguous() or dst.dtype != src.dtype or dst.numel() != src.numel():
        raise _lib.PgasrError("stream_copy: contiguous tensors of one dtype and size, destination on the GPU")
    if not src.is_cuda and not src.is_pinned():
        raise _lib.PgasrError("stream_copy: a host source must be pinned (device-mapped) memory")
    nbytes = dst.numel() * dst.element_size()
    if nbytes == 0:
        return dst
    _lib.check(lib.pgasr_stream_copy(src.data_ptr(), dst.data_ptr(), nbytes, int(workgroups), _stream()), "pgasr_stream_copy")
    return dst


CLIP_STATE_WORDS = 8


def clip_state(device):
    return torch.zeros(CLIP_STATE_WORDS, dtype=torch.float32, device=device)


def clip_state_counts(state):
    w = state.view(torch.int32).tolist()
    return w[2], w[4], w[5]


def grad_norm_clip(grad, max_norm, state=None):
    lib = _lib.load()
    _req(grad, torch.float32, "grad")
    if state is None:
        state = clip_state(grad.device)
    _req(state, torch.float32, "state")
    if state.numel() != CLIP_STATE_WORDS:
        raise _lib.PgasrError(f"grad_norm_clip: state must hold {CLIP_STATE_WORDS} words (hipops.clip_state)")
    n = grad.numel()
    nbytes = lib.pgasr_grad_norm_ws_bytes(n)
    ws = _workspace(nbytes, grad.device, "grad_norm")
    with _timed("grad_norm_kernel"):
        _lib.check(lib.pgasr_grad_norm_clip(_p(grad), n, float(max_norm), _p(ws), nbytes, _p(state), _stream()), "pgasr_grad_norm_clip")
    return state


def adam_step(param, grad, exp_avg, exp_avg_sq, step, lr=5e-4, betas=(0.9, 0.999), eps=1e-8, weight_decay=0.0, guards=(),
              applied=None, clip_state=None):
    lib = _lib.load()
    for t, nm in ((param, "param"), (grad, "grad"), (exp_avg, "exp_avg"), (exp_avg_sq, "exp_avg_sq")):
        _req(t, torch.float32, nm)
    _req(applied, torch.int32, "applied")
    if applied is not None and applied.numel() != 2:
        raise _lib.PgasrError("adam_step: applied must hold two int32 words")
    g = list(guards)[:2] + [0, 0]
    if clip_state is not None:
        _req(clip_state, torch.float32, "clip_state")
        if clip_state.numel() != CLIP_STATE_WORDS:
            raise _lib.PgasrError(f"adam_step: clip_state must hold {CLIP_STATE_WORDS} words (hipops.clip_state)")
        _lib.check(lib.pgasr_adam_step_clipped(_p(param), _p(grad), _p(exp_avg), _p(exp_avg_sq), param.numel(), int(step),
                                               float(lr), float(betas[0]), float(betas[1]), float(eps), float(weight_decay),
                                               g[0], g[1], _p(applied), _p(clip_state), _stream()), "pgasr_adam_step_clipped")
        return
    _lib.check(lib.pgasr_adam_step(_p(param), _p(grad), _p(exp_avg), _p(exp_avg_sq), param.numel(), int(step),
                                   float(lr), float(betas[0]), float(betas[1]), float(eps), float(weight_decay),
                                   g[0], g[1], _p(applied), _stream()), "pgasr_adam_step")


def lstm_busy_ptr(T, B, backward, device, stream=None):
    import ctypes
    lib = _lib.load()
    off = ctypes.c_size_t(0)
    _lib.check(lib.pgasr_lstm_busy_offset(B, int(backward), ctypes.byref(off)), "pgasr_lstm_busy_offset")
    if stream is None:
        ws = _lstm_ws(T, B, backward, device)
    else:
        with torch.cuda.stream(stream):
            ws = _lstm_ws(T, B, backward, device)
    return ws.data_ptr() + off.value


_concurrent = {}
STRICT_CONCURRENCY = False


def streams_concurrent(other):
    main = torch.cuda.current_stream()
    key = (main.cuda_stream, other.cuda_stream)
    if key not in _concurrent:
        lib = _lib.load()
        words = torch.zeros(2, dtype=torch.int32, device=torch.device("cuda", torch.cuda.current_device()))
        torch.cuda.synchronize()
        _lib.check(lib.pgasr_stream_probe(words.data_ptr(), 200000, _stream()), "pgasr_stream_probe")
        with torch.cuda.stream(other):
            words[0:1].fill_(1)
        torch.cuda.synchronize()
        _concurrent[key] = bool(int(words[1].item()) == 1)
        if not _concurrent[key] and STRICT_CONCURRENCY:
            raise _lib.PgasrError("kernels of different streams do not run concurrently here (serialising profiler / launch-blocking "
                                  "mode / one hardware queue): the feed-ahead GEMMs would fall back to the sequential order; set "
                                  "PGASR_ALLOW_SEQUENTIAL=1 to benchmark that order knowingly")
        if not _concurrent[key]:
            import warnings
            warnings.warn("policy_gradient_asr_amd: kernels of different streams do not run concurrently here "
                          "(serialising profiler / launch-blocking mode / one hardware queue): feed-ahead GEMMs are off")
    return _concurrent[key]


GATE_OPENED_ON_BUSY, GATE_OPENED_ON_PUBLICATION, GATE_TIMED_OUT = 1, 2, 3


def stream_gate(words_ptr, count=8, timeout_us=60, need=0, running=None, report=None):
    lib = _lib.load()
    if need > 0 and report is not None:
        _req(report, torch.int32, "report")
        if report.numel() < 2:
            raise _lib.PgasrError("report needs two int32 words")
        _lib.check(lib.pgasr_stream_gate_report(words_ptr, count, int(need), _p(running), timeout_us, _p(report), _stream()),
                   "pgasr_stream_gate_report")
    elif need > 0:
        _lib.check(lib.pgasr_stream_gate_sum(words_ptr, count, int(need), _p(running), timeout_us, _stream()), "pgasr_stream_gate_sum")
    else:
        _lib.check(lib.pgasr_stream_gate(words_ptr, count, timeout_us, _stream()), "pgasr_stream_gate")
```

Before: 3366.

## Stream LSTM input-gradient GEMM beside the backward sweep, gated on slab progress

Adds a gated persistent x6 feed kernel that computes the LSTM input gradient dx tile by tile as soon as the backward sweep publishes the time slabs each row tile needs. Work items are ordered on the host by required slab count and claimed through atomic control words. The weight-gradient GEMM gets a grid cap so both can share the device with the sweep. This aims to hide the dx GEMM behind the serial recurrent sweep instead of running it afterward, at the cost of spin-waiting blocks, extra sync complexity and timeout risk.

```diff
diff --git a/include/pgasr_hip.h b/include/pgasr_hip.h
--- a/include/pgasr_hip.h
+++ b/include/pgasr_hip.h
@@ -183,6 +183,20 @@
                                   const unsigned short* Wmid, const unsigned short* Wlo, float* C, int ldc, const float* bias,
                                   const unsigned* xcc_busy, unsigned* tiles_done, int order, int phase, unsigned* ctrl,
                                   void* workspace, size_t workspace_bytes, void* stream);
+
+int pgasr_gemm_x6w_gate_need(int T, int B, int row_tile);
+int pgasr_gemm_x6w_gate_items(int T, int B, int N, int K, int order, int whole_k, unsigned* items, int max_items);
+size_t pgasr_gemm_x6w_gate_ctl_words(int n_items);
+int pgasr_gemm_x6w_feed_gated_f32(int T, int B, int N, int K, const float* A, int lda, const unsigned short* Whi,
+                                  const unsigned short* Wmid, const unsigned short* Wlo, float* C, int ldc,
+                                  const float* dact_y, float slope, const unsigned* xcc_busy, unsigned* tiles_done, int order,
+                                  const unsigned* slab_done, int* err_word, const unsigned* items, int n_items,
+                                  int whole_k, unsigned* ctl, size_t ctl_words, int grid,
+                                  void* workspace, size_t workspace_bytes, void* stream);
+int pgasr_lstm_wgrads_streamed_grid(const float* dgates, const float* x, const float* out, int T, int B, int in_dim,
+                                    float* dwih_perm, float* dwhh_perm, const unsigned* xcc_busy,
+                                    const unsigned* slab_done, int* err_word, int planes, int grid,
+                                    void* workspace, size_t workspace_bytes, void* stream);
 
 int pgasr_attention_ctx(const float* dec, const float* enc, int NQ, int B, int T, int H, float* ctx, void* stream);
 
diff --git a/policy_gradient_asr_amd/_lib.py b/policy_gradient_asr_amd/_lib.py
--- a/policy_gradient_asr_amd/_lib.py
+++ b/policy_gradient_asr_amd/_lib.py
@@ -148,6 +148,14 @@
     "pgasr_gemm_x6w_feed_head_items": (C.c_int, [C.c_int, C.c_int, C.c_int]),
     "pgasr_gemm_x6w_feed_phase_f32": (C.c_int, [C.c_int, C.c_int, C.c_int, c_f32p, C.c_int, c_ptr, c_ptr, c_ptr, c_f32p, C.c_int,
                                                 c_f32p, c_ptr, c_ptr, C.c_int, C.c_int, c_ptr, c_ptr, C.c_size_t, c_ptr]),
+    "pgasr_gemm_x6w_gate_need": (C.c_int, [C.c_int, C.c_int, C.c_int]),
+    "pgasr_gemm_x6w_gate_items": (C.c_int, [C.c_int, C.c_int, C.c_int, C.c_int, C.c_int, C.c_int, c_ptr, C.c_int]),
+    "pgasr_gemm_x6w_gate_ctl_words": (C.c_size_t, [C.c_int]),
+    "pgasr_gemm_x6w_feed_gated_f32": (C.c_int, [C.c_int, C.c_int, C.c_int, C.c_int, c_f32p, C.c_int, c_ptr, c_ptr, c_ptr, c_f32p, C.c_int,
+                                                c_f32p, C.c_float, c_ptr, c_ptr, C.c_int, c_ptr, c_ptr, c_ptr, C.c_int,
+                                                C.c_int, c_ptr, C.c_size_t, C.c_int, c_ptr, C.c_size_t, c_ptr]),
+    "pgasr_lstm_wgrads_streamed_grid": (C.c_int, [c_f32p, c_f32p, c_f32p, C.c_int, C.c_int, C.c_int, c_f32p, c_f32p, c_ptr,
+                                                  c_ptr, c_ptr, C.c_int, C.c_int, c_ptr, C.c_size_t, c_ptr]),
 }
 
 
diff --git a/policy_gradient_asr_amd/csrc/common.h b/policy_gradient_asr_amd/csrc/common.h
--- a/policy_gradient_asr_amd/csrc/common.h
+++ b/policy_gradient_asr_amd/csrc/common.h
@@ -93,6 +93,14 @@
     }
     return h;
 }
+__host__ __device__ inline int pgasr_wslab_rows_need(int T, int B, long long row0, long long row1) {
+    const int t_lo = (int)(row0 / B), t_hi = (int)((row1 - 1) / B);
+    const int s_last = t_hi > T - 1 - t_lo ? t_hi : T - 1 - t_lo;
+    const int n = pgasr_wslab_count(T);
+    int need = 1;
+    while (need < n && T - pgasr_wslab_edge(T, n - need) <= s_last) ++need;
+    return need;
+}
 
 struct PgasrTn256Args {
     const float* A; const float* B; float* partial;
@@ -108,6 +116,7 @@
     int gate_T, gate_B, gate_nbg;
     int tslabs;
     int* gate_err;
+    int grid0;
 };
 bool pgasr_internal_tn256_ok(const PgasrTn256Args& a, int tk = 32);
 int pgasr_internal_tn256_launch(PgasrTn256Args a, int masked_then_unmasked, hipStream_t st, const PgasrTn256Args* second = nullptr);
diff --git a/policy_gradient_asr_amd/csrc/gemm.hip b/policy_gradient_asr_amd/csrc/gemm.hip
--- a/policy_gradient_asr_amd/csrc/gemm.hip
+++ b/policy_gradient_asr_amd/csrc/gemm.hip
@@ -714,9 +714,16 @@
                                           float* dwih_perm, float* dwhh_perm, const unsigned* xcc_busy,
                                           const unsigned* slab_done, int* err_word, int planes,
                                           void* workspace, size_t workspace_bytes, void* stream) {
+    return pgasr_lstm_wgrads_streamed_grid(dgates, x, out, T, B, in_dim, dwih_perm, dwhh_perm, xcc_busy, slab_done, err_word, planes, 0,
+                                           workspace, workspace_bytes, stream);
+}
+extern "C" int pgasr_lstm_wgrads_streamed_grid(const float* dgates, const float* x, const float* out, int T, int B, int in_dim,
+                                               float* dwih_perm, float* dwhh_perm, const unsigned* xcc_busy,
+                                               const unsigned* slab_done, int* err_word, int planes, int grid,
+                                               void* workspace, size_t workspace_bytes, void* stream) {
     constexpr int H = 256, G = 2 * 4 * H;
     if (!dgates || !x || !out || !dwih_perm || !dwhh_perm || T <= 1 || B <= 0 || in_dim <= 0) return PGASR_ERR_INVALID_ARG;
-    if (planes != 2 && planes != 3) return PGASR_ERR_INVALID_ARG;
+    if ((planes != 2 && planes != 3) || grid < 0 || grid > 256) return PGASR_ERR_INVALID_ARG;
     const size_t need = pgasr_lstm_wgrads_workspace_bytes(T, in_dim);
     if (!workspace || workspace_bytes < need) return PGASR_ERR_WORKSPACE;
     hipStream_t st = (hipStream_t)stream;
@@ -732,6 +739,7 @@
                       (unsigned*)workspace, xcc_busy, 0, slab_done, dgates, T, B, (B + 15) / 16, 1, err_word};
     const int tk = planes == 3 ? 16 : 32;
     if (!pgasr_internal_tn256_ok(ih, tk) || !pgasr_internal_tn256_ok(hh, tk)) return PGASR_ERR_UNSUPPORTED;
+    ih.grid0 = grid;
     if (hipMemsetAsync(workspace, 0, 256, st) != hipSuccess) return PGASR_ERR_LAUNCH;
     const int rc = planes == 3 ? pgasr_internal_tn6_launch(ih, 1, st, &hh) : pgasr_internal_tn256_launch(ih, 1, st, &hh);
     if (rc != PGASR_OK) return rc;
diff --git a/policy_gradient_asr_amd/csrc/gemm_x6.hip b/policy_gradient_asr_amd/csrc/gemm_x6.hip
--- a/policy_gradient_asr_amd/csrc/gemm_x6.hip
+++ b/policy_gradient_asr_amd/csrc/gemm_x6.hip
@@ -1,6 +1,8 @@
 #include "common.h"
 #include "x3w_common.h"
 #include <type_traits>
+#include <algorithm>
+#include <vector>
 
 #ifdef PGASR_X6_DIAG
 #define X6D(bit) (!FEED && (g.single & (bit)))
@@ -78,9 +80,10 @@
                  "ds_write_b64 %0, %2 offset:8192\n\t"
                  "ds_write_b64 %0, %3 offset:16384" :: "v"(addr), "v"(h), "v"(m), "v"(l) : "memory");
 }
-template <int J>
+template <int J, bool SC1>
 __device__ __forceinline__ void load_a_one(u32x4_t (&r)[2], const unsigned (&aoff)[2], unsigned kb, const float* A) {
-    asm volatile("global_load_dwordx4 %0, %1, %2" : "=&v"(r[J]) : "v"(aoff[J] + kb), "s"(A) : "memory");
+    if constexpr (SC1) asm volatile("global_load_dwordx4 %0, %1, %2 sc1" : "=&v"(r[J]) : "v"(aoff[J] + kb), "s"(A) : "memory");
+    else asm volatile("global_load_dwordx4 %0, %1, %2" : "=&v"(r[J]) : "v"(aoff[J] + kb), "s"(A) : "memory");
 }
 template <int CNT>
 __device__ __forceinline__ void wait_a_regs(u32x4_t (&r)[2]) {
@@ -96,8 +99,9 @@
             acc[j] = __builtin_amdgcn_mfma_f32_32x32x16_bf16(__builtin_bit_cast(bf16x8_t, a[PA[p]]), __builtin_bit_cast(bf16x8_t, b[j][PB[p]]), acc[j], 0, 0, 0);
 }
 
-template <bool FEED, int VAR>
+template <bool FEED, int VAR, bool GATED = false>
 __global__ __launch_bounds__(THREADS) void gemm_x6c_kernel(DmaGemmArgs g) {
+    static_assert(FEED || !GATED, "the gate belongs to the persistent kernel");
     extern __shared__ __attribute__((aligned(128))) unsigned char smem[];
 #ifdef PGASR_LSTM_DIAG
     if (FEED && threadIdx.x == 0 && blockIdx.x == 0) x6_feed_diag[0] = (unsigned)wall_clock64();
@@ -114,6 +118,11 @@
         }
     }
     const unsigned lds0 = (unsigned)(size_t)(__attribute__((address_space(3))) unsigned char*)smem;
+    if constexpr (GATED) {
+        unsigned* mailbox = reinterpret_cast<unsigned*>(smem + LDS_BYTES);
+        if (tid == 0) { mailbox[1] = 0u; mailbox[2] = 0u; }
+        __syncthreads();
+    }
   for (;;) {
     int tbx, tby;
     int kt0 = 0, kt1 = nk, qpart = -1;
@@ -125,7 +134,57 @@
         unsigned* mailbox = reinterpret_cast<unsigned*>(smem + LDS_BYTES);
         const unsigned S8 = (unsigned)g.split8_tiles, S = (unsigned)g.split_tiles, S2 = (unsigned)g.split2_tiles, ntot = (unsigned)g.mt_count * (unsigned)g.nt_count;
         const unsigned n8 = 8u * S8, n4 = 4u * S, n2 = 2u * S2;
-        if (tid == 0) {
+        if constexpr (GATED) {
+            if (w == 0) {
+                const unsigned nitems = (unsigned)g.gate_nitems, npub = (unsigned)g.gate_npub;
+                unsigned sel = 0xFFFFFFFFu, need = 0u, state = mailbox[1], scan = mailbox[2];
+                auto published = [&](unsigned k) {
+                    unsigned v = k;
+                    if (lane < g.gate_words) v = __hip_atomic_load(g.gate + lane, __ATOMIC_RELAXED, __HIP_MEMORY_SCOPE_AGENT);
+                    return !__any(v < k);
+                };
+                if (state == 0u && published(npub)) state = 1u;
+                if (state == 0u) {
+                    for (;;) {
+                        unsigned a = 0u;
+                        if (lane == 0) a = __hip_atomic_fetch_add(g.gate_ctl, 1u, __ATOMIC_RELAXED, __HIP_MEMORY_SCOPE_AGENT);
+                        a = (unsigned)__builtin_amdgcn_readfirstlane((int)a);
+                        if (a >= nitems) break;
+                        const unsigned e = g.gate_items[a];
+                        if ((e & 0xFFFFFFu) >= nitems) continue;
+                        unsigned old = 0u;
+                        if (lane == 0) old = __hip_atomic_exchange(g.gate_ctl + 16 + (e & 0xFFFFFFu), 1u, __ATOMIC_RELAXED, __HIP_MEMORY_SCOPE_AGENT);
+                        old = (unsigned)__builtin_amdgcn_readfirstlane((int)old);
+                        if (old == 0u) { sel = e & 0xFFFFFFu; need = e >> 24; break; }
+                    }
+                    if (sel != 0xFFFFFFFFu) {
+                        unsigned spins = 0; long long t0 = 0;
+                        while (!published(need)) {
+                            if (g.gate_err && __hip_atomic_load(g.gate_err, __ATOMIC_RELAXED, __HIP_MEMORY_SCOPE_AGENT) != 0) { state = 2u; break; }
+                            __builtin_amdgcn_s_sleep(32);
+                            if (((++spins) & 255u) == 0) {
+                                const long long now = wall_clock64();
+                                if (spins == 256u) t0 = now;
+                                else if (now - t0 > 300000000LL) { if (lane == 0 && g.gate_err) *g.gate_err = 1; state = 2u; break; }
+                            }
+                        }
+                    }
+                } else {
+                    while (scan < nitems) {
+                        const unsigned idx = scan + (unsigned)lane;
+                        const unsigned c = idx < nitems ? __hip_atomic_load(g.gate_ctl + 16 + idx, __ATOMIC_RELAXED, __HIP_MEMORY_SCOPE_AGENT) : 1u;
+                        const unsigned long long open = __ballot(c == 0u);
+                        if (!open) { scan += 64u; continue; }
+                        const unsigned first = scan + (unsigned)__builtin_ctzll(open);
+                        unsigned old = 0u;
+                        if (lane == 0) old = __hip_atomic_exchange(g.gate_ctl + 16 + first, 1u, __ATOMIC_RELAXED, __HIP_MEMORY_SCOPE_AGENT);
+                        old = (unsigned)__builtin_amdgcn_readfirstlane((int)old);
+                        if (old == 0u) { sel = first; break; }
+                    }
+                }
+                if (lane == 0) { mailbox[0] = sel; mailbox[1] = state; mailbox[2] = scan; }
+            }
+        } else if (tid == 0) {
             if (head_only && __hip_atomic_load(g.queue, __ATOMIC_RELAXED, __HIP_MEMORY_SCOPE_AGENT) >= n8 + n4) *mailbox = 0xFFFFFFFFu;
             else *mailbox = __hip_atomic_fetch_add(g.queue, 1u, __ATOMIC_RELAXED, __HIP_MEMORY_SCOPE_AGENT);
         }
@@ -133,6 +192,7 @@
         const unsigned t = *mailbox;
         __syncthreads();
         if (t >= ntot + 7u * S8 + 3u * S + S2) return;
+        if constexpr (GATED) __builtin_amdgcn_fence(__ATOMIC_ACQUIRE, "agent");
 #ifdef PGASR_LSTM_DIAG
         if (tid == 0 && t < 4u) x6_feed_diag[4 + t] = (unsigned)wall_clock64();
         if (tid == 0 && t >= n8 + n4 + n2 && t < n8 + n4 + n2 + 4u) x6_feed_diag[1024 + (t - n8 - n4 - n2)] = (unsigned)wall_clock64();
@@ -184,8 +244,8 @@
     auto load_a1 = [&](int kt, auto setc, int j) {
         const unsigned kb = (unsigned)((kt < nk ? kt : nk - 1) * TK * 4);
         if (X6D(4) && kt >= kt0 + NA + 1) return;
-        if (j == 0) load_a_one<0>(araw[decltype(setc)::value], aoff, kb, g.A);
-        else load_a_one<1>(araw[decltype(setc)::value], aoff, kb, g.A);
+        if (j == 0) load_a_one<0, GATED>(araw[decltype(setc)::value], aoff, kb, g.A);
+        else load_a_one<1, GATED>(araw[decltype(setc)::value], aoff, kb, g.A);
     };
     auto load_a = [&](int kt, auto setc) { load_a1(kt, setc, 0); load_a1(kt, setc, 1); };
     auto convert_a1 = [&](int buf, auto setc, int j) {
@@ -919,6 +979,99 @@
     return pgasr_gemm_x6w_feed_phase_f32(M, N, K, A, lda, Whi, Wmid, Wlo, C, ldc, bias, xcc_busy, tiles_done, order, 0, nullptr, workspace, workspace_bytes, stream);
 }
 
+extern "C" int pgasr_gemm_x6w_gate_need(int T, int B, int row_tile) {
+    if (T <= 0 || B <= 0 || row_tile < 0) return 0;
+    const long long M = (long long)T * B, r0 = (long long)row_tile * x6c::TM;
+    if (r0 >= M) return 0;
+    return pgasr_wslab_rows_need(T, B, r0, r0 + x6c::TM < M ? r0 + x6c::TM : M);
+}
+
+namespace {
+unsigned x6_item_tile(unsigned t, unsigned S8, unsigned S, unsigned S2) {
+    const unsigned n8 = 8u * S8, n4 = 4u * S, n2 = 2u * S2;
+    if (t < n8) return t >> 3;
+    if (t < n8 + n4) return S8 + ((t - n8) >> 2);
+    if (t < n8 + n4 + n2) return S8 + S + ((t - n8 - n4) >> 1);
+    return t - 7u * S8 - 3u * S - S2;
+}
+int x6_gate_item_count(int mt, int nt, int K, int whole_k, int& s8, int& s4, int& s2) {
+    s8 = s4 = s2 = 0;
+    if (!whole_k) x6_feed_splits(mt, nt, K, pgasr_gemm_x6w_feed_workspace_bytes(), s8, s4, s2);
+    return mt * nt + 7 * s8 + 3 * s4 + s2;
+}
+}
+
+extern "C" int pgasr_gemm_x6w_gate_items(int T, int B, int N, int K, int order, int whole_k, unsigned* items, int max_items) {
+    if (T <= 0 || B <= 0 || N <= 0 || K <= 0 || order < 0 || order > 1 || pgasr_gemm_x6w_feed_col_tiles(N) == 0 || (K % x6c::TK)) return 0;
+    const long long M = (long long)T * B;
+    if (M * N * 4 >= ((long long)1 << 31)) return 0;
+    const int mt = (int)((M + x6c::TM - 1) / x6c::TM), nt = N / x6c::TN;
+    int s8, s4, s2;
+    const int n = x6_gate_item_count(mt, nt, K, whole_k, s8, s4, s2);
+    if (n >= (1 << 24)) return 0;
+    if (!items) return n;
+    if (max_items < n) return 0;
+    const int npub = pgasr_wslab_count(T), half = nt >> 1;
+    std::vector<int> need((size_t)mt);
+    for (int r = 0; r < mt; ++r) need[(size_t)r] = pgasr_gemm_x6w_gate_need(T, B, r);
+    struct Key { int k, dist, t; };
+    std::vector<Key> keys((size_t)n);
+    for (int t = 0; t < n; ++t) {
+        const unsigned tile = x6_item_tile((unsigned)t, (unsigned)s8, (unsigned)s4, (unsigned)s2);
+        const int grp = (int)(tile / (unsigned)nt), j = (int)(tile % (unsigned)nt);
+        const int tby = ((j < half) != (order != 0)) ? grp : mt - 1 - grp;
+        const int d2 = 2 * tby - (mt - 1), k = need[(size_t)tby];
+        keys[(size_t)t] = Key{k, k < npub ? (d2 < 0 ? -d2 : d2) / 2 : 0, t};
+    }
+    std::sort(keys.begin(), keys.end(), [](const Key& a, const Key& b) { return a.k != b.k ? a.k < b.k : a.dist != b.dist ? a.dist < b.dist : a.t < b.t; });
+    for (int q = 0; q < n; ++q) items[q] = ((unsigned)keys[(size_t)q].k << 24) | (unsigned)keys[(size_t)q].t;
+    return n;
+}
+
+extern "C" size_t pgasr_gemm_x6w_gate_ctl_words(int n_items) { return n_items > 0 ? 16 + (size_t)n_items : 0; }
+
+extern "C" int pgasr_gemm_x6w_feed_gated_f32(int T, int B, int N, int K, const float* A, int lda, const unsigned short* Whi,
+                                             const unsigned short* Wmid, const unsigned short* Wlo, float* C, int ldc,
+                                             const float* dact_y, float slope, const unsigned* xcc_busy, unsigned* tiles_done, int order,
+                                             const unsigned* slab_done, int* err_word, const unsigned* items, int n_items,
+                                             int whole_k, unsigned* ctl, size_t ctl_words, int grid,
+                                             void* workspace, size_t workspace_bytes, void* stream) {
+    whole_k = (whole_k || dact_y) ? 1 : 0;
+    if (!A || !Whi || (!Wmid != !Wlo) || !C || !tiles_done || !slab_done || !items || !ctl || T <= 0 || B <= 0 || N <= 0 || K <= 0 || lda < K || ldc < N)
+        return PGASR_ERR_INVALID_ARG;
+    if (order < 0 || order > 1 || grid < 0 || grid > 256) return PGASR_ERR_INVALID_ARG;
+    if (!workspace || workspace_bytes < pgasr_gemm_x6w_feed_workspace_bytes()) return PGASR_ERR_WORKSPACE;
+    const long long Ml = (long long)T * B;
+    if (Ml >= ((long long)1 << 31) || 2 * ((B + 15) / 16) > 64) return PGASR_ERR_UNSUPPORTED;
+    const int M = (int)Ml;
+    if (!x6w_shape_ok(M, N, K, A, lda, ldc, Whi, Wmid, Wlo) || pgasr_gemm_x6w_feed_col_tiles(N) == 0) return PGASR_ERR_UNSUPPORTED;
+    if ((size_t)M * ldc * 4 >= ((size_t)1 << 31)) return PGASR_ERR_UNSUPPORTED;
+    const int mt = (M + x6c::TM - 1) / x6c::TM, nt = N / x6c::TN;
+    int split8, split, split2;
+    const int n = x6_gate_item_count(mt, nt, K, whole_k, split8, split, split2);
+    if (n != n_items || n >= (1 << 24)) return PGASR_ERR_INVALID_ARG;
+    if (ctl_words < pgasr_gemm_x6w_gate_ctl_words(n)) return PGASR_ERR_WORKSPACE;
+    hipStream_t st = (hipStream_t)stream;
+    const size_t lds = (size_t)x6c::LDS_BYTES + 16;
+    auto kern = x6_var() == 7 ? x6c::gemm_x6c_kernel<true, 7, true> : x6c::gemm_x6c_kernel<true, 0, true>;
+    if (hipFuncSetAttribute((const void*)kern, hipFuncAttributeMaxDynamicSharedMemorySize, (int)lds) != hipSuccess) return PGASR_ERR_LAUNCH;
+    if (hipMemsetAsync(workspace, 0, 1024, st) != hipSuccess) return PGASR_ERR_LAUNCH;
+    if (hipMemsetAsync(ctl, 0, pgasr_gemm_x6w_gate_ctl_words(n) * 4, st) != hipSuccess) return PGASR_ERR_LAUNCH;
+    unsigned* cw = (unsigned*)workspace;
+    DmaGemmArgs g{A, Whi, Wlo, C, M, N, K, lda, ldc, nullptr, dact_y, slope, cw, xcc_busy, tiles_done, mt, nt, order,
+                  whole_k ? 1 : x6_quarters(K), split, (float*)((char*)workspace + 1024), cw + 64, 0, Wmid};
+    g.head_help = 0;
+    g.split8_tiles = split8; g.split2_tiles = split2; g.slab_count = 8 * split8 + 4 * split + 2 * split2;
+    g.gate = slab_done; g.gate_items = items; g.gate_ctl = ctl; g.gate_err = err_word;
+    g.gate_words = 2 * ((B + 15) / 16); g.gate_nitems = n; g.gate_npub = pgasr_wslab_count(T);
+    for (int pass = 0; pass < (xcc_busy ? 2 : 1); ++pass) {
+        if (pass == 1) g.xcc_busy = nullptr;
+        PGASR_LAUNCH_KERNEL(kern, dim3(pass == 0 && grid > 0 ? grid : 256), dim3(x6c::THREADS), lds, st, g);
+        PGASR_CHECK_LAUNCH();
+    }
+    return PGASR_OK;
+}
+
 int pgasr_internal_tn6_launch(PgasrTn256Args a, int masked_then_unmasked, hipStream_t st, const PgasrTn256Args* second) {
     PgasrTn256Args b{};
     const int tk = a.tslabs ? t6::TK : 32;
@@ -944,7 +1097,7 @@
         return PGASR_ERR_LAUNCH;
     const unsigned* busy = a.xcc_busy;
     const char* eg = getenv("PGASR_T6_GRID");
-    const int grid0 = (eg && atoi(eg) >= 8 && atoi(eg) <= 256) ? atoi(eg) : 256;
+    const int grid0 = (eg && atoi(eg) >= 8 && atoi(eg) <= 256) ? atoi(eg) : (a.grid0 >= 8 && a.grid0 <= 256) ? a.grid0 : 256;
     for (int pass = 0; pass < ((masked_then_unmasked && busy) ? 2 : 1); ++pass) {
         a.xcc_busy = (pass == 0) ? busy : nullptr;
         b.xcc_busy = a.xcc_busy;
diff --git a/policy_gradient_asr_amd/csrc/x3w_common.h b/policy_gradient_asr_amd/csrc/x3w_common.h
--- a/policy_gradient_asr_amd/csrc/x3w_common.h
+++ b/policy_gradient_asr_amd/csrc/x3w_common.h
@@ -24,6 +24,11 @@
     int head_help;
     int split8_tiles, split2_tiles;
     int slab_count;
+    const unsigned* gate;
+    const unsigned* gate_items;
+    unsigned* gate_ctl;
+    int* gate_err;
+    int gate_words, gate_nitems, gate_npub;
 };
 
 __device__ __forceinline__ void dma16(const void* gsrc, void* lds_base) {
diff --git a/policy_gradient_asr_amd/functional.py b/policy_gradient_asr_amd/functional.py
--- a/policy_gradient_asr_amd/functional.py
+++ b/policy_gradient_asr_amd/functional.py
@@ -10,6 +10,9 @@
 JOIN_FEED = os.environ.get("PGASR_JOIN_FEED", "0") == "1"
 FEED_BWD = os.environ.get("PGASR_FEED_BWD", "1") != "0"
 STREAM_DW = os.environ.get("PGASR_STREAM_DW", "1") != "0"
+DX_BESIDE = os.environ.get("PGASR_DX_BESIDE", "1") != "0"
+DX_BESIDE_T6_GRID = int(os.environ.get("PGASR_DX_T6_GRID", "128"))
+DX_BESIDE_X6_GRID = int(os.environ.get("PGASR_DX_X6_GRID", "128"))
 LEAKY_SLOPE = 0.01
 
 
@@ -377,11 +380,25 @@
                       and hipops.lstm_wgrads_ok(T, B, I, npl) and hipops.lstm_fed_ok(T, B)
                       and hipops.streams_concurrent(grad_overlap.third_side_stream()))
         slab = None
+        slab_zeroed = None
         if stream_own:
             slab = ctx.slab_words if (ctx.slab_words is not None and ctx.slab_words.numel() >= 64) else None
             ctx.slab_words = None
             if slab is None:
                 slab = torch.zeros(64, dtype=torch.int32, device=dev)
+                slab_zeroed = True
+        defer = (ctx.needs_input_grad[0] and grad_overlap.enabled and FEED_AHEAD and FEED_BWD and ctx.sweep_follows and not ctx.has_dact
+                 and ctx.planes_t is not None and hipops.gemm_x3w_ok(T * B, I, G, planes=npl) and I % 256 == 0 and I == 2 * HID
+                 and hipops.x3w_feed_col_tiles(I, npl) > 0
+                 and hipops.lstm_fed_ok(T, B) and hipops.streams_concurrent(grad_overlap.side_stream()))
+        dx_split = ctx.sweep_follows and not ctx.has_dact and I == 2 * HID
+        beside = (DX_BESIDE and stream_own and ctx.needs_input_grad[0] and npl == 3 and (defer or not ctx.sweep_follows)
+                  and ctx.planes_t is not None and hipops.gemm_x3w_ok(T * B, I, G, planes=npl)
+                  and hipops.x3w_feed_col_tiles(I, npl) > 0 and hipops.x6w_gated_ok(T, B, I, G, whole_k=not dx_split)
+                  and hipops.streams_concurrent(grad_overlap.side_stream()))
+        if beside and slab_zeroed:
+            slab_zeroed = torch.cuda.Event()
+            slab_zeroed.record()
         if rec is not None:
             if grad_overlap.enabled and rec["head"]():
                 before = torch.cuda.Event()
@@ -397,21 +414,51 @@
             if rec is not None:
                 streams.hold(dout, grad_overlap.side_stream())
             fed_done = None
+            if beside:
+                grad_overlap.side_stream()
             if stream_own and grad_overlap._key() in grad_overlap._sides:
                 fed_done = torch.cuda.Event()
                 with torch.cuda.stream(grad_overlap.side_stream()):
                     fed_done.record()
+            dx = None
+            if beside:
+                side = grad_overlap.side_stream()
+                dx = torch.empty(T, B, I, dtype=torch.float32, device=dev)
+                need_words = 2 * ((T * B + 255) // 256)
+                done = ctx.fed_bwd if (ctx.fed_bwd is not None and ctx.fed_bwd.numel() >= need_words) else None
+                ctx.fed_bwd = None
+                if done is None:
+                    done = torch.zeros(need_words, dtype=torch.int32, device=dev)
+                    done_zeroed = torch.cuda.Event()
+                    done_zeroed.record()
+                    side.wait_event(done_zeroed)
+                side.wait_event(before)
+                if slab_zeroed is not None:
+                    side.wait_event(slab_zeroed)
+                with torch.cuda.stream(side):
+                    items_dev = hipops.gemm_x6w_feed_gated(dg, ctx.planes_t, dx, T, B, I, G, busy if grad_overlap.confine_feed else 0, done, slab,
+                                                           sweep_ws, order=1, dact_y=dact_y if ctx.has_dact else None, slope=LEAKY_SLOPE,
+                                                           whole_k=not dx_split, grid=DX_BESIDE_X6_GRID)
+                    dx_ready = torch.cuda.Event() if not ctx.sweep_follows else None
+                    if dx_ready is not None:
+                        dx_ready.record()
+                for t_ in (dg, dx, done, slab, items_dev) + tuple(ctx.planes_t) + ((dact_y,) if ctx.has_dact else ()):
+                    streams.hold(t_, side)
+                if ctx.sweep_follows:
+                    grad_overlap._deferred[dx.data_ptr()] = {"dx": dx, "done": done, "need": hipops.x3w_feed_col_tiles(I, npl), "drop": None,
+                                                             "launch": lambda busy_ptr: None, "head": lambda: False}
             swept = torch.cuda.Event()
             swept.record()
             grad_overlap.note_event(swept)
             if not ctx.sweep_follows and grad_overlap.upper_grads_hook is not None:
                 grad_overlap.upper_grads_hook(swept)
-        dx = None
-        defer = (ctx.needs_input_grad[0] and grad_overlap.enabled and FEED_AHEAD and FEED_BWD and ctx.sweep_follows and not ctx.has_dact
-                 and ctx.planes_t is not None and hipops.gemm_x3w_ok(T * B, I, G, planes=npl) and I % 256 == 0 and I == 2 * HID
-                 and hipops.x3w_feed_col_tiles(I, npl) > 0
-                 and hipops.lstm_fed_ok(T, B) and hipops.streams_concurrent(grad_overlap.side_stream()))
-        if defer:
+            if beside and dx_ready is not None:
+                torch.cuda.current_stream().wait_event(dx_ready)
+        else:
+            dx = None
+        if beside:
+            pass
+        elif defer:
             dx = torch.empty(T, B, I, dtype=torch.float32, device=dev)
             need_words = 2 * ((T * B + 255) // 256)
             done = ctx.fed_bwd if (ctx.fed_bwd is not None and ctx.fed_bwd.numel() >= need_words) else None
@@ -512,7 +559,7 @@
                 dwih = torch.empty(G, I, dtype=torch.float32, device=dev)
                 dwhh = torch.empty(2, 4 * HID, HID, dtype=torch.float32, device=dev)
                 hipops.lstm_wgrads(dg, x, out, T, B, I, dwih, dwhh, busy_ptr=busy if grad_overlap.confine else 0,
-                                   slab=slab, err_ws=sweep_ws, planes=npl)
+                                   slab=slab, err_ws=sweep_ws, planes=npl, grid=DX_BESIDE_T6_GRID if beside else 0)
                 s3.wait_event(swept)
                 dbias = torch.empty(G, dtype=torch.float32, device=dev)
                 hipops.colsum(dbias_part, dbias_part.shape[0], G, G, dbias)
diff --git a/policy_gradient_asr_amd/hipops.py b/policy_gradient_asr_amd/hipops.py
--- a/policy_gradient_asr_amd/hipops.py
+++ b/policy_gradient_asr_amd/hipops.py
@@ -845,6 +845,84 @@
     return ws if phase == 1 else C
 
 
+def x6w_gate_need(T, B, row_tile):
+    return int(_lib.load().pgasr_gemm_x6w_gate_need(int(T), int(B), int(row_tile)))
+
+
+def x6w_gate_items(T, B, N, K, order=1, whole_k=False):
+    import ctypes
+    lib = _lib.load()
+    n = lib.pgasr_gemm_x6w_gate_items(int(T), int(B), int(N), int(K), int(order), int(bool(whole_k)), None, 0)
+    if n <= 0:
+        return []
+    arr = (ctypes.c_uint32 * n)()
+    if lib.pgasr_gemm_x6w_gate_items(int(T), int(B), int(N), int(K), int(order), int(bool(whole_k)), ctypes.addressof(arr), n) != n:
+        raise _lib.PgasrError("pgasr_gemm_x6w_gate_items: inconsistent item count")
+    return list(arr)
+
+
+_gate_items_cache = collections.OrderedDict()
+
+
+def _gate_items_dev(items, device):
+    key = (device, tuple(items))
+    t = _gate_items_cache.get(key)
+    if t is None:
+        t = torch.tensor(items, dtype=torch.int64).to(torch.int32).to(device)
+        _gate_items_cache[key] = t
+        while len(_gate_items_cache) > 64:
+            _gate_items_cache.popitem(last=False)
+    else:
+        _gate_items_cache.move_to_end(key)
+    return t
+
+
+def x6w_gated_ok(T, B, N, K, whole_k=False):
+    return (LSTM_PLANES == 3 and B % 16 == 0 and 0 < B <= 32 and T >= 2 and lstm_fed_ok(T, B)
+            and bool(_lib.load().pgasr_gemm_x6w_gate_items(int(T), int(B), int(N), int(K), 1, int(bool(whole_k)), None, 0) > 0))
+
+
+def gemm_x6w_feed_gated(A, planes, C, T, B, N, K, busy_ptr, tiles_done, slab, err_ws, order=1, dact_y=None, slope=0.01, whole_k=False, grid=0,
+                        gate=True):
+    import ctypes
+    lib = _lib.load()
+    for t, nm in ((A, "A"), (C, "C"), (dact_y, "dact_y")):
+        if t is not None and (not t.is_cuda or t.dtype != torch.float32):
+            raise _lib.PgasrError(f"gemm_x6w_feed_gated operand {nm} must be a float32 GPU tensor")
+    _check_planes(planes, N, K, "gemm_x6w_feed_gated")
+    M = T * B
+    if len(planes) != 3:
+        raise _lib.PgasrError("gemm_x6w_feed_gated: six-product planes only")
+    if tiles_done.dtype != torch.int32 or tiles_done.numel() < 2 * ((M + 255) // 256):
+        raise _lib.PgasrError("gemm_x6w_feed_gated: tiles_done must hold 2 * ceil(M/256) int32 words")
+    nwords = 2 * ((B + 15) // 16)
+    if slab is None or slab.dtype != torch.int32 or not slab.is_cuda or slab.numel() < nwords:
+        raise _lib.PgasrError("gemm_x6w_feed_gated: slab must be the sweep's int32 slab_done words")
+    whole_k = bool(whole_k) or dact_y is not None
+    items = x6w_gate_items(T, B, N, K, order, whole_k)
+    if not items:
+        raise _lib.PgasrError("gemm_x6w_feed_gated: not a shape of the gated feed")
+    items_dev = _gate_items_dev(items, C.device)
+    ctl_words = int(lib.pgasr_gemm_x6w_gate_ctl_words(len(items)))
+    ctl = _workspace(4 * ctl_words, C.device, "x6w_gate_ctl")
+    ws = _workspace(lib.pgasr_gemm_x6w_feed_workspace_bytes(), C.device, "x6w_feed")
+    err_ptr = 0
+    if err_ws is not None:
+        off = ctypes.c_size_t(0)
+        _lib.check(lib.pgasr_lstm_error_offset(B, 1, ctypes.byref(off)), "pgasr_lstm_error_offset")
+        err_ptr = err_ws.data_ptr() + off.value
+    if gate:
+        first = items[0] >> 24
+        stream_gate(slab.data_ptr(), count=nwords, need=first * nwords, timeout_us=5000)
+    with _timed("gemm_feed_x6c_gated"):
+        st = lib.pgasr_gemm_x6w_feed_gated_f32(T, B, N, K, A.data_ptr(), K, *_plane_ptrs(planes), C.data_ptr(), N, _p(dact_y), float(slope),
+                                               busy_ptr, tiles_done.data_ptr(), int(order), slab.data_ptr(), err_ptr,
+                                               items_dev.data_ptr(), len(items), int(whole_k), ctl.data_ptr(), ctl_words, int(grid),
+                                               _p(ws), ws.numel(), _stream())
+    _lib.check(st, "pgasr_gemm_x6w_feed_gated_f32")
+    return items_dev
+
+
 def lstm_layer_bwd(gates, out, cbuf, dout, pack_b, lengths, T, B, want_dbias=False, fed=None, fed_need=0, drop=None, slab=None):
     lib = _lib.load()
     ws = _lstm_ws(T, B, True, gates.device)
@@ -886,7 +964,7 @@
     return T >= 2 and in_dim % 256 == 0 and B > 0 and B % (16 if planes == 3 else 32) == 0 and T * B * 2048 * 4 < 2 ** 31
 
 
-def lstm_wgrads(dgates, x, out, T, B, in_dim, dwih, dwhh, busy_ptr=0, slab=None, err_ws=None, planes=None):
+def lstm_wgrads(dgates, x, out, T, B, in_dim, dwih, dwhh, busy_ptr=0, slab=None, err_ws=None, planes=None, grid=0):
     lib = _lib.load()
     planes = LSTM_PLANES if planes is None else int(planes)
     for t_, nm in ((dgates, "dgates"), (x, "x"), (out, "out"), (dwih, "dwih"), (dwhh, "dwhh")):
@@ -900,8 +978,8 @@
         _lib.check(lib.pgasr_lstm_error_offset(B, 1, ctypes.byref(off)), "pgasr_lstm_error_offset")
         err_ptr = err_ws.data_ptr() + off.value
     with _timed("gemm_t6" if planes == 3 else "gemm_t256"):
-        st = lib.pgasr_lstm_wgrads_streamed(_p(dgates), _p(x), _p(out), T, B, in_dim, _p(dwih), _p(dwhh), int(busy_ptr),
-                                            _p(slab), err_ptr, planes, _p(ws), ws.numel(), _stream())
+        st = lib.pgasr_lstm_wgrads_streamed_grid(_p(dgates), _p(x), _p(out), T, B, in_dim, _p(dwih), _p(dwhh), int(busy_ptr),
+                                                 _p(slab), err_ptr, planes, int(grid) if planes == 3 else 0, _p(ws), ws.numel(), _stream())
     _lib.check(st, "pgasr_lstm_wgrads_streamed")
 
 
```

New measurement: 3253. -3.4%, worse.
